# wkentaro/morefusion

Hardware: AMD Instinct MI355X
Metric: objects/sec (32^3 voxelize+3D-CNN+ICC refine) (higher is better)
Workload: dtype f32; 1 GPU; 1 scene(s) x 8 objects per GPU: singleview_3d Model.predict (ResNet18+PSPNet, 32^3 voxelize, occupancy 3D-CNN, heads; B=8) -> ICC joint refine 100 iters (BASELINE configs[1]+configs[2]); random weights, ICC starts from synthetic perturbed-GT poses; ICC(k) on a second HIP stream, event-ordered after network(k), beside network(k+1); objects_per_gpu=8, icc_iters=100, parallelism=scene-sharded x1, pose all_gather, stream_priority=none, backbone_memory_format=contiguous

## Files before the change

include/mfhip.h:

```cpp
#ifndef MFHIP_H_
#define MFHIP_H_

#include <stdint.h>

#ifdef __cplusplus
extern "C" {
#endif

typedef void *mfStream_t;

int mf_version(void);
const char *mf_last_error_string(void);

int mf_average_voxelization_3d_fwd(const float *values, const float *points,
                                   const int32_t *batch_indices, int64_t n, int C,
                                   int B, int X, int Y, int Z, float ox, float oy,
                                   float oz, float pitch, float *matrix,
                                   int32_t *counts, int32_t *head, int32_t *link,
                                   int32_t *nan_flag, mfStream_t stream);
int mf_average_voxelization_3d_bwd(const float *gmatrix, const float *points,
                                   const int32_t *batch_indices,
                                   const int32_t *counts, int64_t n, int C, int B,
                                   int X, int Y, int Z, float ox, float oy, float oz,
                                   float pitch, float *gvalues, mfStream_t stream);

int mf_max_voxelization_3d_fwd(const float *values, const float *points,
                               const int32_t *batch_indices, const float *intensities,
                               int64_t n, int C, int B, int X, int Y, int Z, float ox,
                               float oy, float oz, float pitch, float *matrix,
                               int32_t *indices, uint64_t *key, int32_t *nan_flag,
                               mfStream_t stream);
int mf_max_voxelization_3d_bwd(const float *gmatrix, const int32_t *indices, int64_t n,
                               int C, int B, int X, int Y, int Z, float *gvalues,
                               mfStream_t stream);

int mf_interpolate_voxel_grid_fwd(const float *vox, const float *points,
                                  const int32_t *batch_indices, const int32_t *batch_start,
                                  int64_t n, int B, int C, int X, int Y, int Z, float *values,
                                  int channels_first, mfStream_t stream);
int mf_interpolate_voxel_grid_bwd(const float *gvalues, const float *points,
                                  const int32_t *batch_indices, const int32_t *batch_start,
                                  int64_t n, int B, int C, int X, int Y, int Z, float *gvox,
                                  int channels_first, mfStream_t stream);

int mf_occupancy_grid_3d_fwd(const float *points, int64_t P, float pitch, float ox,
                             float oy, float oz, int X, int Y, int Z, float threshold,
                             float *grid, float *dmin, mfStream_t stream);
int mf_occupancy_grid_3d_bwd(const float *ggrid, const float *points, int64_t P,
                             float pitch, float ox, float oy, float oz, int X, int Y,
                             int Z, float threshold, const float *dmin, float *gpoints,
                             mfStream_t stream);

int mf_truncated_distance_function_fwd(const float *points, int64_t P, float pitch,
                                       float ox, float oy, float oz, int X, int Y, int Z,
                                       float truncation, float *tdf, int32_t *flat,
                                       mfStream_t stream);
int mf_truncated_distance_function_bwd(const float *gtdf, const float *points,
                                       const int32_t *flat, int64_t P, float pitch,
                                       float ox, float oy, float oz, int X, int Y, int Z,
                                       float truncation, float *gpoints,
                                       mfStream_t stream);
int mf_pseudo_occupancy_weights(const float *tdf, const int32_t *flat, const float *sdf,
                                int X, int Y, int Z, int K, float truncation,
                                float sdf_offset, float *grids, float *wsurf, float *win,
                                float *wmax, mfStream_t stream);

int mf_nn(const float *ref, int64_t R, const float *query, int64_t Q, int64_t *out,
          float *out_dist, mfStream_t stream);

int mf_icp_loss_grad(const float *source, int64_t S, const float *target, int64_t T,
                     const float *Rt, float thresh, float *out, mfStream_t stream);

int mf_icp_refine(const float *source, const int32_t *src_off, const float *target,
                  const int32_t *tgt_off, int32_t L, int32_t max_T, float thresh, float *q, float *t,
                  float *adam_m, float *adam_v, int32_t n_iter, int32_t step0, float alpha_q,
                  float alpha_t, float *losses, float *ws, mfStream_t stream);

typedef struct {
  const void *pts4;
  const int32_t *obj_off;
  const int32_t *scene_off;
  const int32_t *obj_scene;
  const float *pitch;
  const float *origin;
  const float *grid_target;
  const float *grid_ne;
  int32_t n_objects;
  int32_t n_scenes;
  int32_t n_points;
  int32_t dim;
  int32_t max_scene_objects;
  float voxel_threshold;
  float sdf_offset;
  int32_t grid_ne_binary;
  int32_t flags;
} mfIccBatch;

int64_t mf_icc_workspace_bytes(const mfIccBatch *batch);

int mf_icc_prepare(const mfIccBatch *batch, void *ws, mfStream_t stream);

int mf_icc_loss_grad(const mfIccBatch *batch, const float *q, const float *t,
                     float *loss, float *gq, float *gt, void *ws, mfStream_t stream);

int mf_icc_refine(const mfIccBatch *batch, float *q, float *t, float *adam_m,
                  float *adam_v, int32_t n_iter, int32_t step0, float alpha_q,
                  float alpha_t, float *losses, float *traj, void *ws,
                  mfStream_t stream);

int mf_icc_iteration_launches(const mfIccBatch *batch);

int mf_icc_plan(const mfIccBatch *batch, int64_t *out, int32_t n);

int mf_icc_launch_stage(const mfIccBatch *batch, const float *q, const float *t, void *ws,
                        int32_t stage, mfStream_t stream);

int mf_icc_debug_stamps(unsigned long long *host_out, int n);

int64_t mf_sparse_conv3d_workspace_bytes(int32_t B, int32_t Cs, int32_t Cout, int32_t D,
                                         int32_t max_rows, int64_t n_points);
int mf_sparse_conv3d_pack_weights(const float *W, int32_t Cout, int32_t Cs, int32_t w_cin,
                                  int32_t c_off, float *Wp, mfStream_t stream);
int mf_sparse_conv3d_k4s2_fwd(const float *x, const int32_t *counts, const float *Wp,
                              const float *dense, const float *bias, float *out, void *ws,
                              int32_t B, int32_t Cs, int32_t Cout, int32_t D, int32_t max_rows,
                              int32_t relu, mfStream_t stream);

int mf_average_distance_fwd(const float *points, const float *T_true, const float *T_pred,
                            const uint8_t *symmetric, int32_t B, int32_t M, int32_t P,
                            float *out, int32_t *nn_idx, mfStream_t stream);
int mf_average_distance_bwd(const float *points, const float *T_true, const float *T_pred,
                            const uint8_t *symmetric, const float *gout, int32_t B, int32_t M,
                            int32_t P, const int32_t *nn_idx, float *gT_pred, mfStream_t stream);

int mf_sparse_conv3d_k4s2_points_fwd(const float *values, const float *points,
                                     const int32_t *batch_indices, int64_t n, float ox, float oy,
                                     float oz, float pitch, const float *Wp, const float *dense,
                                     const float *bias, float *out, void *ws, int32_t B,
                                     int32_t Cs, int32_t Cout, int32_t D, int32_t max_rows,
                                     int32_t relu, mfStream_t stream);

int mf_conv3d_k4s2_pack_weights(const float *W, int32_t Cout, int32_t Cin, int32_t w_cin, int32_t c_off,
                                float *wt, mfStream_t stream);
int32_t mf_conv3d_k4s2_default_split(int32_t B, int32_t Cin, int32_t Cout, int32_t D);
int64_t mf_conv3d_k4s2_workspace_bytes(int32_t B, int32_t Cout, int32_t D, int32_t split);
int mf_conv3d_k4s2_fwd(const float *x, const float *wt, const float *bias, const float *add, float *out,
                       void *ws, int32_t B, int32_t Cin, int32_t Cout, int32_t D, int32_t split,
                       int32_t relu, mfStream_t stream);
int mf_to_channels_last(const float *src, float *dst, int32_t B, int32_t C, int64_t V, mfStream_t stream);

int mf_sparse_conv3d_k4s2_points_cl_fwd(const float *values, int64_t ldv, const float *points,
                                        const int32_t *batch_indices, int64_t n, float ox, float oy,
                                        float oz, float pitch, const float *Wp, const float *dense,
                                        const float *bias, float *out, void *ws, int32_t B, int32_t Cs,
                                        int32_t Cout, int32_t D, int32_t max_rows, int32_t relu,
                                        mfStream_t stream);
int mf_interpolate_voxel_grid_cl_fwd(const float *vox, const float *points, const int32_t *batch_indices,
                                     int64_t n, int B, int C, int X, int Y, int Z, float *out, int64_t ldo,
                                     mfStream_t stream);
int mf_sparse_conv3d_k4s2_points_cl_split_fwd(const float *values, int64_t ldv, const float *points,
                                              const int32_t *batch_indices, int64_t n, float ox, float oy, float oz,
                                              float pitch, const float *Wp, const float *dense, const float *bias,
                                              float *out, void *out_split, void *ws, int32_t B, int32_t Cs,
                                              int32_t Cout, int32_t D, int32_t max_rows, int32_t relu,
                                              mfStream_t stream);
int mf_interpolate_voxel_grid_cl_split_fwd(const float *vox, const float *points, const int32_t *batch_indices,
                                           int64_t n, int B, int C, int X, int Y, int Z, void *outs, int64_t ldos,
                                           int64_t los, mfStream_t stream);
int mf_occupancy_convs_fwd(const float *grid, const float *w1, const float *b1, const float *w2,
                           const float *b2, float *h1, float *h2, int32_t B, int32_t D, mfStream_t stream);

int mf_linear_fwd(const float *A, int64_t a_group_stride, int32_t lda, const float *W, int64_t w_group_stride,
                  int32_t ldw, const float *bias, int64_t b_group_stride, float *out, int64_t o_group_stride,
                  int32_t ldo, int32_t M, int32_t N, int32_t Npad, int32_t K, int32_t groups, int32_t relu,
                  mfStream_t stream);

int mf_cast_rows_bf16(const float *src, int64_t src_ld, void *dst, int64_t dst_ld, int64_t rows, int32_t cols,
                      mfStream_t stream);
int mf_relu_mask_bf16(const void *y, const void *dy, const float *dy32, void *dz, int64_t n, mfStream_t stream);
int mf_linear_bf16(const void *A, int64_t a_group_stride, int32_t lda, const void *W, int64_t w_group_stride,
                   int32_t ldw, const float *bias, int64_t b_group_stride, void *out, int64_t o_group_stride,
                   int32_t ldo, int32_t M, int32_t N, int32_t K, int32_t groups, int32_t relu, int32_t out_f32,
                   int32_t accumulate, mfStream_t stream);
int mf_linear_wgrad_bf16(const void *dY, int64_t y_group_stride, int32_t ldy, const void *A, int64_t a_group_stride,
                         int32_t lda, float *dW, int64_t w_group_stride, int32_t ldc, void *ws, int32_t M, int32_t N,
                         int32_t K, int32_t groups, int32_t split, mfStream_t stream);
int mf_conv3d_k4s2_pack_bf16(const float *W, int32_t Cout, int32_t Cin, int32_t w_cin, int32_t c_off, void *fwd,
                             void *dgrad, mfStream_t stream);
int mf_conv3d_k4s2_bf16_fwd(const void *x, const void *wt, const float *bias, void *out, int32_t B, int32_t Cin,
                            int32_t Cout, int32_t D, int32_t relu, int32_t out_f32, mfStream_t stream);
int mf_conv3d_k4s2_bf16_dgrad(const void *dy, const void *wd, void *dx, int32_t B, int32_t Cin, int32_t Cout,
                              int32_t D, int32_t out_f32, int32_t accumulate, mfStream_t stream);
int64_t mf_conv3d_k4s2_bf16_wgrad_workspace_bytes(int32_t Cin, int32_t Cout, int32_t split);
int32_t mf_conv3d_k4s2_bf16_wgrad_default_split(int32_t B, int32_t Cin, int32_t Cout, int32_t D);
int mf_conv3d_k4s2_bf16_wgrad(const void *dy, const void *x, float *dW, void *ws, int32_t B, int32_t Cin,
                              int32_t Cout, int32_t D, int32_t w_cin, int32_t c_off, int32_t split,
                              mfStream_t stream);

int mf_conv3d_bf16_pack(const float *W, int32_t Cout, int32_t Cin, int32_t w_cin, int32_t c_off, int32_t ks, void *fwd,
                        void *dgrad_k4s2, void *flipT, mfStream_t stream);
int mf_conv3d_bf16_fwd(const void *x, const void *wt, const float *bias, void *out, int32_t B, int32_t Cin,
                       int32_t Cout, int32_t D, int32_t ks, int32_t stride, int32_t pad, int32_t dil, int32_t relu,
                       int32_t out_f32, int32_t ldo, mfStream_t stream);
int64_t mf_conv3d_bf16_fwd_workspace_bytes(int32_t B, int32_t Cin, int32_t Cout, int32_t D, int32_t ks, int32_t stride,
                                           int32_t pad, int32_t dil);
int mf_conv3d_bf16_fwd_ws(const void *x, const void *wt, const float *bias, void *out, void *ws, int64_t ws_bytes,
                          int32_t B, int32_t Cin, int32_t Cout, int32_t D, int32_t ks, int32_t stride, int32_t pad,
                          int32_t dil, int32_t relu, int32_t out_f32, int32_t ldo, mfStream_t stream);
int mf_conv2d_split_pack(const float *W, int32_t Cout, int32_t Cin, int32_t ks, void *wp, mfStream_t stream);
int64_t mf_conv2d_split_workspace_bytes(int32_t B, int32_t Cin, int32_t Cout, int32_t D, int32_t ks, int32_t stride,
                                        int32_t pad, int32_t dil);
int mf_conv2d_split_fwd(const void *xs, const void *wp, const float *bias, const float *res, int32_t ldr,
                        const float *slope, int32_t act, float *out32, int32_t ldo32, void *outs, int32_t ldos,
                        int32_t los, void *ws, int64_t ws_bytes, int32_t B, int32_t Cin, int32_t Cout, int32_t D,
                        int32_t ks, int32_t stride, int32_t pad, int32_t dil, mfStream_t stream);
int mf_conv3d_k4s2_split_pack(const float *W, int32_t Cout, int32_t Cin, int32_t w_cin, int32_t c_off, void *wp,
                              mfStream_t stream);
int64_t mf_conv3d_k4s2_split_workspace_bytes(int32_t B, int32_t Cin, int32_t Cout, int32_t D);
int mf_conv3d_k4s2_split_fwd(const void *xs, const void *wp, const float *bias, int32_t relu, float *out32,
                             int32_t ldo32, void *outs, int32_t ldos, int32_t los, void *ws, int64_t ws_bytes, int32_t B,
                             int32_t Cin, int32_t Cout, int32_t D, mfStream_t stream);
int mf_linear_split_pack(const float *W, int64_t w_gs, int32_t ldw, int32_t N, int32_t K, int32_t Np, int32_t Kp,
                         int32_t groups, void *wp, mfStream_t stream);
int64_t mf_linear_split_workspace_bytes(int64_t M, int32_t N, int32_t Kp);
int mf_linear_split_fwd(const void *As, int32_t lda, const void *wp, const float *bias, int32_t relu, float *out32,
                        int32_t ldo32, void *outs, int32_t ldos, int32_t los, void *ws, int64_t ws_bytes, int32_t M,
                        int32_t N, int32_t Kp, mfStream_t stream);
int64_t mf_conv3d_k3_narrow_bf16_pack_elems(int32_t CI);
int mf_conv3d_k3_narrow_bf16_pack(const float *W, int32_t Cout, int32_t Cin, int32_t w_cin, int32_t c_off,
                                  int32_t transpose, void *wp, mfStream_t stream);
int mf_conv3d_k3_narrow_bf16(const void *x, const void *wp, const float *bias, void *out, int32_t B, int32_t CI,
                             int32_t CO, int32_t D, int32_t dil, int32_t relu, mfStream_t stream);
int64_t mf_conv3d_bf16_wgrad_workspace_bytes(int32_t Cin, int32_t Cout, int32_t ks, int32_t split);
int32_t mf_wgrad_split(int64_t tiles, int64_t ktiles, int64_t slab_bytes);
int32_t mf_linear_wgrad_bf16_default_split(int64_t M, int32_t N, int32_t K, int32_t groups);
int32_t mf_conv3d_bf16_wgrad_default_split(int32_t B, int32_t Cin, int32_t Cout, int32_t Do, int32_t ks);
int mf_conv3d_bf16_wgrad(const void *dy, const void *x, float *dW, void *ws, int32_t B, int32_t Cin, int32_t Cout,
                         int32_t D, int32_t ks, int32_t stride, int32_t pad, int32_t dil, int32_t w_cin, int32_t c_off,
                         int32_t split, mfStream_t stream);

int64_t mf_sparse_conv3_bf16_max_rows(int64_t n_points);
int64_t mf_sparse_conv3_bf16_workspace_bytes(int64_t n_points, int32_t B, int32_t D);
int mf_sparse_conv3_bf16_tables(void *ws, int64_t n_points, int32_t B, int32_t D, int64_t *out7);
int mf_sparse_conv3_bf16_index(const float *points, const int32_t *batch_indices, int64_t n, int32_t B, int32_t D,
                               void *ws, mfStream_t stream);
int mf_sparse_conv3_bf16_pack(const float *W, int32_t Cout, int32_t Cs, int32_t w_cin, int32_t c_off, void *Wp, void *Wq,
                              mfStream_t stream);
int mf_sparse_conv3_bf16_unpack_dw(const float *dWp, int32_t Cout, int32_t Cs, int32_t w_cin, int32_t c_off, float *dW,
                                   mfStream_t stream);
int mf_sparse_conv3_bf16_reduce(const void *C, const float *dense, const float *bias, void *ws, int64_t n_points,
                                int32_t B, int32_t D, int32_t Cout, int32_t relu, void *out, mfStream_t stream);
int mf_sparse_conv3_bf16_gather_dy(const void *dz, void *ws, int64_t n_points, int32_t B, int32_t D, int32_t Cout,
                                   void *dYg, mfStream_t stream);
int mf_linear_bf16_tiles(const void *A, int32_t lda, const void *W, int64_t w_group_stride, int32_t ldw,
                         const int32_t *tile_group, void *out, int32_t ldo, int32_t M, int32_t N, int32_t K,
                         int32_t out_f32, mfStream_t stream);
int mf_linear_wgrad_bf16_ranges(const void *dY, int32_t ldy, const void *A, int32_t lda, float *dW,
                                int64_t w_group_stride, int32_t ldc, const int32_t *m_range, int32_t groups, int32_t N,
                                int32_t K, mfStream_t stream);
int mf_conv3d_k4s2_bf16_pack_cols(const float *W, int32_t Cout, int32_t Cin, int32_t w_cin, int32_t c_off, void *W2,
                                  mfStream_t stream);
int mf_conv3d_k4s2_bf16_col2im(const void *T, int32_t B, int32_t D, int32_t Cin, void *dx, mfStream_t stream);
int mf_average_voxelization_rows_bf16_fwd(const void *values, int64_t ldv, const float *points,
                                          const int32_t *batch_indices, int64_t n, int32_t C, int32_t B, int32_t D,
                                          const int32_t *counts, const int32_t *head, const int32_t *link,
                                          const int32_t *rowmap, void *A, int64_t lda, mfStream_t stream);
int mf_average_voxelization_rows_bf16_bwd(const void *dA, int64_t lda, const float *points,
                                          const int32_t *batch_indices, const int32_t *counts, const int32_t *rowmap,
                                          int64_t n, int32_t C, int32_t B, int32_t D, void *gvalues, int64_t ldg,
                                          mfStream_t stream);

int mf_average_voxelization_cl_bf16_fwd(const void *values, int64_t ldv, const float *points,
                                        const int32_t *batch_indices, int64_t n, int32_t C, int32_t B, int32_t D,
                                        void *x, int64_t ldx, int32_t *counts, int32_t *head, int32_t *link,
                                        mfStream_t stream);
int mf_average_voxelization_cl_bf16_bwd(const void *gx, int64_t ldx, const float *points, const int32_t *batch_indices,
                                        const int32_t *counts, int64_t n, int32_t C, int32_t B, int32_t D,
                                        void *gvalues, int64_t ldg, mfStream_t stream);
int mf_interpolate_voxel_grid_cl_bf16_fwd(const void *vox, const float *points, const int32_t *batch_indices,
                                          int64_t n, int B, int C, int X, int Y, int Z, void *out, int64_t ldo,
                                          mfStream_t stream);
int mf_interpolate_voxel_grid_cl_bf16_bwd(const void *gout, int64_t ldg, const float *points,
                                          const int32_t *batch_indices, const int32_t *batch_start, int64_t n, int B,
                                          int C, int X, int Y, int Z, void *gvox, int32_t out_bf16, mfStream_t stream);

int mf_upsample_bilinear_cl_fwd(const void *x, void *y, int32_t B, int32_t H, int32_t W, int32_t Ho, int32_t Wo,
                                int32_t C, int32_t bf16, mfStream_t stream);
int mf_upsample_bilinear_cl_split_fwd(const float *x, void *y, int32_t B, int32_t H, int32_t W, int32_t Ho, int32_t Wo,
                                      int32_t C, int32_t ldy, int32_t los, mfStream_t stream);
int mf_split_bf16(const float *x, int64_t sb, int64_t sc, int64_t sh, int64_t sw, int32_t B, int32_t C, int32_t H,
                  int32_t W, void *y, int32_t ldy, int32_t los, mfStream_t stream);
int mf_upsample2x_tapsum_fwd(const float *z, const float *bias, const float *slope, int32_t act, float *y32,
                             int32_t ld32, void *ys, int32_t lds, int32_t los, int32_t B, int32_t H, int32_t W, int32_t C,
                             mfStream_t stream);
int mf_maxpool3s2_split_fwd(const float *x, int64_t sb, int64_t sc, int64_t sh, int64_t sw, int32_t B, int32_t C,
                            int32_t H, int32_t W, float *y32, void *ys, mfStream_t stream);
int mf_upsample_bilinear_cl_bwd(const void *gy, void *gx, int32_t B, int32_t H, int32_t W, int32_t Ho, int32_t Wo,
                                int32_t C, int32_t bf16, mfStream_t stream);
int mf_upsample_bilinear_cf_fwd(const void *x, void *y, int64_t BC, int32_t H, int32_t W, int32_t Ho, int32_t Wo,
                                int32_t bf16, mfStream_t stream);
int mf_upsample_bilinear_cf_bwd(const void *gy, void *gx, int64_t BC, int32_t H, int32_t W, int32_t Ho, int32_t Wo,
                                int32_t bf16, mfStream_t stream);
int mf_prelu_fwd(const void *x, const float *slope, void *y, int64_t n, int32_t bf16, mfStream_t stream);
int mf_rgb_normalize(const void *rgb, int32_t u8, const float *mean3, const float *std3, float *out, int64_t npix,
                     mfStream_t stream);
int mf_bn_act_fwd(const void *x, const void *identity, const float *mean, const float *var, const float *weight,
                  const float *bias, float eps, void *y, int64_t n, int32_t C, int64_t HW, int32_t channels_last,
                  int32_t relu, int32_t bf16, mfStream_t stream);
int mf_backbone2d_last_path(void);
int64_t mf_prelu_bwd_workspace_floats(int64_t n);
int mf_prelu_bwd(const void *x, const void *dy, const float *slope, void *dx, float *dslope, float *ws, int64_t n,
                 int32_t bf16, mfStream_t stream);

int mf_gemm_bf16_last_tile(void);

int mf_gemm_bf16_nt_plan(int32_t mode, int64_t M, int32_t N, int32_t K, int32_t groups, int32_t table,
                         int64_t dgrad_rows, int32_t may_split, int32_t have_ws, int32_t *tile, int32_t *S);
int mf_gemm_bf16_tn_plan(int32_t Ni, int32_t Nj, int32_t ldc, int64_t rows, int32_t groups, int32_t ranges,
                         int32_t conv, int32_t split, int32_t *form, int32_t *default_split, int32_t *finish);

int mf_psp_tail_rows_bf16_fwd(const void *u2, const int64_t *pix, int32_t B, int32_t P, int32_t H, int32_t W, void *rows,
                              mfStream_t stream);
int mf_psp_tail_rows_bf16_bwd(const void *grows, const int64_t *pix, int32_t B, int32_t P, int32_t H, int32_t W,
                              float *acc, void *gu2, mfStream_t stream);

int mf_confidence_loss_fwd(const float *add, const float *conf, int32_t B, int32_t P, float lambda, float *loss,
                           int32_t *cnt, mfStream_t stream);
int mf_confidence_loss_bwd(const float *add, const float *conf, const int32_t *cnt, const float *gloss, int32_t B,
                           int32_t P, float lambda, float *dadd, float *dconf, mfStream_t stream);

int mf_pose_epilogue_train_fwd(const float *orot, const float *otrn, const float *ocnf, const int64_t *class_id,
                               const float *pts, const float *origin, const float *pitch, int32_t B, int32_t P,
                               int32_t n_fg, float *rot, float *trans, float *conf, mfStream_t stream);
int mf_pose_epilogue_train_bwd(const float *orot, const float *ocnf, const int64_t *class_id, const float *pitch,
                               const float *grot, const float *gtrans, const float *gconf, int32_t B, int32_t P,
                               int32_t n_fg, float *drot, float *dtrn, float *dcnf, mfStream_t stream);
int mf_transformation_matrix_fwd(const float *q, const float *t, int64_t n, float *T, mfStream_t stream);
int mf_transformation_matrix_bwd(const float *q, const float *gT, int64_t n, float *gq, float *gt, mfStream_t stream);
int mf_point_prep(const float *points_cam, const float *values, const float *origin, const float *pitch,
                  int32_t B, int32_t P, int32_t Cv, float center, float *pts, float *tc4, float *x_rows,
                  int32_t *batch_indices, mfStream_t stream);
int mf_pose_epilogue(const float *heads_out, int64_t ldo, int32_t np4, const int64_t *class_id,
                     const float *pts, const float *origin, const float *pitch, int32_t B, int32_t P, int32_t n_fg,
                     float *rot, float *trans, float *conf, mfStream_t stream);

#define MF_PCDNET_WS_BUFFERS 12
#define MF_PCDNET_MAX_FG 256
int32_t mf_pcdnet_workspace_offsets(int32_t B, int32_t P, int32_t n_fg, int64_t *offsets);
int64_t mf_pcdnet_workspace_bytes(int32_t B, int32_t P, int32_t n_fg);
int mf_pcdnet_stem(const float *x_rows, const float *pcd, const int64_t *pix, const float *center, const float *w_rgb,
                   const float *b_rgb, const float *w_pcd, const float *b_pcd, int32_t B, int32_t P, int32_t HW,
                   float *pts, void *f1, int32_t ld1, void *xs, int32_t ldx, int32_t losx, mfStream_t stream);
int mf_pcdnet_pool(const float *h, int64_t ldh, int32_t B, int32_t P, int32_t C, float *pooled, mfStream_t stream);
int mf_pcdnet_bias_relu_split(const float *y, int64_t ldy, const float *gbias, int32_t B, int32_t P, int32_t N, int32_t G,
                              void *out, int64_t ldo, mfStream_t stream);

int mf_psp_tail_fwd(const float *u2, int64_t sb, int64_t sc, int64_t sy, int64_t sx, const int64_t *pix,
                    const float *w3t, const float *b3, const float *prelu_slope, const float *w1t,
                    const float *b1, int32_t B, int32_t P, int32_t H, int32_t W, float *out, mfStream_t stream);

int mf_pack_points_sdf(const float *points, const float *sdf, int64_t n, void *pts4,
                       mfStream_t stream);

int mf_instance_stats(const int32_t *label, const float *depth, int H, int W,
                      const int32_t *instance_ids, int n_inst, int32_t *stats,
                      mfStream_t stream);
int mf_instance_crops(const uint8_t *rgb, const float *depth, const int32_t *label, int H,
                      int W, double fx, double fy, double cx, double cy,
                      const int32_t *instance_ids, const int32_t *stats, int n_inst, int S,
                      int min_valid, uint8_t *rgb_out, float *pcd_out, uint8_t *keep,
                      mfStream_t stream);

int mf_valid_pixel_order(const float *pcd, int32_t B, int32_t HW, int32_t *order, int32_t *counts,
                         mfStream_t stream);

typedef struct {
  float *logodds;
  uint32_t *bits;
  int32_t lo[3];
  int32_t dim[3];
  double resolution;
  double res_factor;
} mfOccTree;
int mf_occmap_regrid(const mfOccTree *src, const mfOccTree *dst, mfStream_t stream);
int mf_occmap_bounds(const float *pts, const int32_t *label, int64_t n, const int32_t *slots,
                     int32_t n_slots, const mfOccTree *trees, int32_t n_trees, int32_t *bounds,
                     mfStream_t stream);
int mf_occmap_raycast(const float *pts, const int32_t *label, int64_t n, const int32_t *slots,
                      int32_t n_slots, const mfOccTree *trees, float origin_x, float origin_y,
                      float origin_z, int32_t *overflow, mfStream_t stream);
int mf_occmap_count_hits(const float *pts, int64_t n, const mfOccTree *trees, int32_t tree,
                         int32_t *overflow, mfStream_t stream);
int mf_occmap_apply(const mfOccTree *trees, int32_t n_trees, int64_t max_cells, int32_t mode,
                    mfStream_t stream);
int mf_occmap_extract(const mfOccTree *trees, int32_t n_trees, const int32_t *target_tree,
                      const double *pitch, const double *origin, int32_t B, int32_t D0, int32_t D1,
                      int32_t D2, float *grid_target, float *grid_nontarget, float *grid_empty,
                      uint8_t *net_target, uint8_t *net_nte, mfStream_t stream);

int64_t mf_occtrack_workspace_bytes(int32_t H, int32_t W, int32_t n_ref);
int64_t mf_occtrack_stats_elems(int32_t n_ref, int32_t n_det);
int mf_occtrack_transform(const float *pts, const float *T, int64_t n, float *out, mfStream_t stream);
int mf_occtrack_render(const float *pts, const float *K, const float *T, float origin_x, float origin_y,
                       float origin_z, const mfOccTree *trees, const int32_t *slots, int32_t n_slots,
                       int32_t H, int32_t W, void *workspace, int32_t *label_rendered,
                       float *depth_rendered, mfStream_t stream);
int mf_occtrack_overlap(const int32_t *label_rendered, const int32_t *label_detected, int32_t H, int32_t W,
                        const int32_t *ref_ids, int32_t n_ref, const int32_t *det_ids, int32_t n_det,
                        int32_t *stats, mfStream_t stream);
int mf_occtrack_assign(const int32_t *stats, const int32_t *ref_ids, int32_t n_ref, int32_t n_det, int32_t H,
                       int32_t W, int32_t min_mask, int32_t min_bbox, int32_t min_side, double iou_threshold,
                       double coverage_threshold, int32_t *counter, int32_t *remap, int32_t *suspicious_ref,
                       int32_t *suspicious_det, mfStream_t stream);
int mf_occtrack_relabel(const int32_t *label_rendered, const int32_t *label_detected, int32_t H, int32_t W,
                        const int32_t *ref_ids, int32_t n_ref, const int32_t *det_ids, int32_t n_det,
                        const int32_t *remap, const int32_t *suspicious_ref, int32_t *label_tracked,
                        int32_t *label_reference, mfStream_t stream);
int mf_occtrack_clean(const int32_t *label, int32_t H, int32_t W, int32_t min_area, int32_t band,
                      void *workspace, int32_t *label_out, mfStream_t stream);
int mf_occtrack_merge(const int32_t *label_reference, const int32_t *label_tracked, int32_t H, int32_t W,
                      const int32_t *ref_ids, int32_t n_ref, void *workspace, int32_t *label_merged,
                      mfStream_t stream);

#define MF_ICPREG_MAX_CELLS (1 << 24)
int64_t mf_icpreg_workspace_bytes(int64_t total_cells, int64_t total_grid, int64_t n_points);
int mf_icpreg_bounds(const double *pts, const int64_t *off, int32_t n_sets, double voxel_size,
                     double *vmin, int32_t *ext, mfStream_t stream);
int mf_icpreg_prepare(const double *pts, const int64_t *off, int32_t n_sets, double voxel_size,
                      const double *vmin, const int32_t *ext, const int64_t *box_off,
                      int64_t total_cells, const int64_t *grid_off, const int32_t *grid_dim,
                      int64_t total_grid, double cell, int64_t n_points, void *workspace,
                      double *out, int32_t *out_cnt, double *grid_origin, int32_t *grid_start,
                      int32_t *grid_idx, mfStream_t stream);
typedef struct {
  const double *src;
  const int64_t *src_off;
  const int32_t *src_cnt;
  const double *tgt;
  const int64_t *tgt_off;
  const int32_t *tgt_cnt;
  const int64_t *grid_off;
  const int32_t *grid_dim;
  const double *grid_origin;
  const int32_t *grid_start;
  const int32_t *grid_idx;
  const double *transform_init;
  const uint8_t *active;
  double *cur;
  int32_t *corr;
  double *transform;
  double *transformation;
  double *fitness;
  double *inlier_rmse;
  int32_t *n_iter;
  double *hist_transform;
  double *hist_fitness;
  double *hist_rmse;
  double max_corr_dist;
  double cell;
  int32_t n_objects;
  int32_t max_iter;
  int32_t mode;
  int32_t reserved;
} mfIcpRegBatch;
int mf_icpreg_run(const mfIcpRegBatch *batch, mfStream_t stream);

#define MF_MESHSDF_MAX_MESHES 65535
#define MF_MESHSDF_MAX_FACES (1LL << 26)
#define MF_MESHSDF_MAX_GRID_DIM 1024
typedef struct {
  const double *vertices;
  const int64_t *v_off;
  const int32_t *faces;
  const int64_t *f_off;
  double *face_rec;
  const double *points;
  const int64_t *q_off;
  const int32_t *blk_off;
  const double *grid_origin;
  const double *grid_h;
  double *dist;
  int32_t *face;
  double *winding;
  double *sdf;
  uint8_t *occupancy;
  int32_t n_meshes;
  int32_t n_blocks;
  int32_t grid_dim;
  int32_t reserved;
} mfMeshSdfBatch;
int64_t mf_meshsdf_workspace_bytes(int64_t total_faces);
int mf_meshsdf_prepare(const mfMeshSdfBatch *batch, int64_t total_faces, mfStream_t stream);
int mf_meshsdf_query(const mfMeshSdfBatch *batch, mfStream_t stream);

#define MF_RENDER_MAX_ITEMS 65535
#define MF_RENDER_MAX_FACES (1LL << 26)
#define MF_RENDER_MAX_PIXELS (1LL << 28)
#define MF_RENDER_MAX_SIDE 4096
typedef struct {
  const double *vertices;
  const int64_t *v_off;
  const int32_t *faces;
  const int64_t *f_off;
  const int32_t *item_mesh;
  const double *item_T;
  const int32_t *item_target;
  const int32_t *item_id;
  const int64_t *item_rec_off;
  void *workspace;
  float *depth;
  int32_t *instance;
  int32_t *face;
  int32_t *count;
  double fx;
  double fy;
  double cx;
  double cy;
  double near;
  int32_t n_meshes;
  int32_t n_items;
  int32_t n_targets;
  int32_t height;
  int32_t width;
  int32_t reserved;
} mfRenderBatch;
int64_t mf_render_workspace_bytes(int64_t total_records, int64_t n_targets, int64_t height, int64_t width);
int mf_render_setup(const mfRenderBatch *batch, int64_t total_records, mfStream_t stream);
int mf_render_raster(const mfRenderBatch *batch, int64_t total_records, mfStream_t stream);
int mf_render_resolve(const mfRenderBatch *batch, int64_t total_records, mfStream_t stream);
int mf_full_grids(const double *points, const int64_t *p_off, const double *T, const double *pitch,
                  const double *origin, int32_t n_examples, int64_t total_points, int32_t dim,
                  int32_t *target_full, int32_t *nontarget_full, mfStream_t stream);

#define MF_PICK_MAX_OBJECTS 64
int mf_pick_occlusion(const int32_t *instance, const int32_t *item_id, int32_t n_items, int32_t height,
                      int32_t width, int32_t *whole, int32_t *occluded_by, int32_t *bbox, mfStream_t stream);
int mf_pick_normals(const double *points, const int32_t *rect, int32_t n_images, int32_t height, int32_t width,
                    double *normals, mfStream_t stream);
int mf_pick_grasp(const float *depth, const int32_t *instance, const int32_t *item_id, const int32_t *bbox,
                  int32_t n_items, int32_t height, int32_t width, double fx, double fy, double cx, double cy,
                  int32_t *cell, double *translation, double *normal, mfStream_t stream);

int64_t mf_average_distance_f64_workspace_bytes(int32_t n_items, int32_t max_points);
int mf_average_distance_f64(const double *points, const int32_t *cloud_off, const int32_t *item_cloud,
                            const double *T1, const double *T2, int32_t n_clouds, int32_t n_items,
                            int32_t max_points, int32_t translate, double *add, double *add_s, void *workspace,
                            mfStream_t stream);

int64_t mf_augment_workspace_bytes(int32_t n, int32_t S);
int mf_augment_mask(const uint8_t *rgb, const void *pcd, int32_t pcd_is_f64, const double *params,
                    int32_t n, int32_t S, int64_t seed, uint8_t *rgb_out, void *pcd_out,
                    uint8_t *kept_mask, int32_t *stats, uint8_t *keep, int32_t *labels, int32_t *sizes,
                    void *workspace, mfStream_t stream);
int mf_augment_rgb(const uint8_t *rgb, const double *params, int32_t n, int32_t S, uint8_t *rgb_out,
                   void *workspace, mfStream_t stream);
int mf_augment_pcd(const void *pcd, int32_t pcd_is_f64, const double *params, int32_t n, int32_t S,
                   int64_t seed, void *pcd_out, mfStream_t stream);

#define MF_OCCREG_MAX_OBJECTS 65535
#define MF_OCCREG_POINT_TILE 1024
#define MF_OCCREG_LDS_VOXELS 32768
#define MF_OCCREG_MAX_THRESHOLD 64.0f
#define MF_OCCREG_STEPS_PER_LAUNCH 128
typedef struct {
  const float *points;
  const int32_t *pts_off;
  const float *pitch;
  const float *origin;
  const int32_t *dims;
  const float *threshold;
  const float *grid_occ;
  const float *grid_unocc;
  const int32_t *grid_off;
  const uint8_t *active;
  const int32_t *host_pts_off;
  const float *host_pitch;
  const int32_t *host_dims;
  const float *host_threshold;
  int32_t n_objects;
  int32_t n_points_total;
  int32_t max_voxels;
  int32_t reserved;
} mfOccRegBatch;
int64_t mf_occreg_workspace_bytes(int64_t n_objects, int64_t n_points_total, int64_t max_voxels);
int mf_occreg_loss_grad(const mfOccRegBatch *batch, const float *q, const float *t, float *loss, float *gq,
                        float *gt, void *workspace, mfStream_t stream);
int mf_occreg_refine(const mfOccRegBatch *batch, float *q, float *t, float *adam_m, float *adam_v, int32_t n_iter,
                     int32_t step0, float alpha_q, float alpha_t, float *losses, float *traj, void *workspace,
                     mfStream_t stream);

#ifdef __cplusplus
}
#endif
#endif
```

morefusion_amd/_lib.py:

```python
import ctypes
import os

import torch

_HERE = os.path.dirname(os.path.abspath(__file__))
SO_PATH = os.path.join(_HERE, os.path.basename(os.environ.get("MF_LIBMFHIP", "libmfhip.so")))
_lib = None

_p = ctypes.c_void_p
_i = ctypes.c_int32
_i64 = ctypes.c_int64
_f = ctypes.c_float
_d = ctypes.c_double


class IccBatch(ctypes.Structure):

    _fields_ = [
        ("pts4", _p), ("obj_off", _p), ("scene_off", _p), ("obj_scene", _p),
        ("pitch", _p), ("origin", _p), ("grid_target", _p), ("grid_ne", _p),
        ("n_objects", _i), ("n_scenes", _i), ("n_points", _i), ("dim", _i), ("max_scene_objects", _i),
        ("voxel_threshold", _f), ("sdf_offset", _f), ("grid_ne_binary", _i), ("flags", _i),
    ]


class OccTree(ctypes.Structure):

    _fields_ = [
        ("logodds", _p), ("bits", _p), ("lo", _i * 3), ("dim", _i * 3),
        ("resolution", _d), ("res_factor", _d),
    ]


class IcpRegBatch(ctypes.Structure):

    _fields_ = [(n, _p) for n in (
        "src", "src_off", "src_cnt", "tgt", "tgt_off", "tgt_cnt", "grid_off", "grid_dim", "grid_origin", "grid_start",
        "grid_idx", "transform_init", "active", "cur", "corr", "transform", "transformation", "fitness", "inlier_rmse",
        "n_iter", "hist_transform", "hist_fitness", "hist_rmse")] + [
        ("max_corr_dist", _d), ("cell", _d), ("n_objects", _i), ("max_iter", _i), ("mode", _i), ("reserved", _i)]


class MeshSdfBatch(ctypes.Structure):

    _fields_ = [(n, _p) for n in (
        "vertices", "v_off", "faces", "f_off", "face_rec", "points", "q_off", "blk_off", "grid_origin", "grid_h",
        "dist", "face", "winding", "sdf", "occupancy")] + [
        ("n_meshes", _i), ("n_blocks", _i), ("grid_dim", _i), ("reserved", _i)]


class RenderBatch(ctypes.Structure):

    _fields_ = [(n, _p) for n in (
        "vertices", "v_off", "faces", "f_off", "item_mesh", "item_T", "item_target", "item_id", "item_rec_off",
        "workspace", "depth", "instance", "face", "count")] + [
        (n, _d) for n in ("fx", "fy", "cx", "cy", "near")] + [
        (n, _i) for n in ("n_meshes", "n_items", "n_targets", "height", "width", "reserved")]


class OccRegBatch(ctypes.Structure):

    _fields_ = [(n, _p) for n in (
        "points", "pts_off", "pitch", "origin", "dims", "threshold", "grid_occ", "grid_unocc", "grid_off", "active",
        "host_pts_off", "host_pitch", "host_dims", "host_threshold")] + [
        (n, _i) for n in ("n_objects", "n_points_total", "max_voxels", "reserved")]


_SIGNATURES = {
    "mf_version": ([], _i),
    "mf_last_error_string": ([], ctypes.c_char_p),
    "mf_average_voxelization_3d_fwd": ([_p, _p, _p, _i64, _i, _i, _i, _i, _i, _f, _f, _f, _f, _p, _p, _p, _p, _p, _p], _i),
    "mf_average_voxelization_3d_bwd": ([_p, _p, _p, _p, _i64, _i, _i, _i, _i, _i, _f, _f, _f, _f, _p, _p], _i),
    "mf_max_voxelization_3d_fwd": ([_p, _p, _p, _p, _i64, _i, _i, _i, _i, _i, _f, _f, _f, _f, _p, _p, _p, _p, _p], _i),
    "mf_max_voxelization_3d_bwd": ([_p, _p, _i64, _i, _i, _i, _i, _i, _p, _p], _i),
    "mf_interpolate_voxel_grid_fwd": ([_p, _p, _p, _p, _i64, _i, _i, _i, _i, _i, _p, _i, _p], _i),
    "mf_interpolate_voxel_grid_bwd": ([_p, _p, _p, _p, _i64, _i, _i, _i, _i, _i, _p, _i, _p], _i),
    "mf_occupancy_grid_3d_fwd": ([_p, _i64, _f, _f, _f, _f, _i, _i, _i, _f, _p, _p, _p], _i),
    "mf_occupancy_grid_3d_bwd": ([_p, _p, _i64, _f, _f, _f, _f, _i, _i, _i, _f, _p, _p, _p], _i),
    "mf_truncated_distance_function_fwd": ([_p, _i64, _f, _f, _f, _f, _i, _i, _i, _f, _p, _p, _p], _i),
    "mf_truncated_distance_function_bwd": ([_p, _p, _p, _i64, _f, _f, _f, _f, _i, _i, _i, _f, _p, _p], _i),
    "mf_pseudo_occupancy_weights": ([_p, _p, _p, _i, _i, _i, _i, _f, _f, _p, _p, _p, _p, _p], _i),
    "mf_nn": ([_p, _i64, _p, _i64, _p, _p, _p], _i),
    "mf_icp_loss_grad": ([_p, _i64, _p, _i64, _p, _f, _p, _p], _i),
    "mf_icp_refine": ([_p, _p, _p, _p, _i, _i, _f, _p, _p, _p, _p, _i, _i, _f, _f, _p, _p, _p], _i),
    "mf_icc_workspace_bytes": ([ctypes.POINTER(IccBatch)], _i64),
    "mf_icc_iteration_launches": ([ctypes.POINTER(IccBatch)], _i),
    "mf_icc_plan": ([ctypes.POINTER(IccBatch), _p, _i], _i),
    "mf_icc_launch_stage": ([ctypes.POINTER(IccBatch), _p, _p, _p, _i, _p], _i),
    "mf_icc_prepare": ([ctypes.POINTER(IccBatch), _p, _p], _i),
    "mf_icc_loss_grad": ([ctypes.POINTER(IccBatch), _p, _p, _p, _p, _p, _p, _p], _i),
    "mf_icc_refine": ([ctypes.POINTER(IccBatch), _p, _p, _p, _p, _i, _i, _f, _f, _p, _p, _p, _p], _i),
    "mf_icc_debug_stamps": ([_p, _i], _i),
    "mf_sparse_conv3d_workspace_bytes": ([_i] * 5 + [_i64], _i64),
    "mf_sparse_conv3d_k4s2_points_fwd": ([_p, _p, _p, _i64, _f, _f, _f, _f, _p, _p, _p, _p, _p] + [_i] * 6 + [_p], _i),
    "mf_sparse_conv3d_pack_weights": ([_p, _i, _i, _i, _i, _p, _p], _i),
    "mf_sparse_conv3d_k4s2_fwd": ([_p, _p, _p, _p, _p, _p, _p] + [_i] * 6 + [_p], _i),
    "mf_pack_points_sdf": ([_p, _p, _i64, _p, _p], _i),
    "mf_average_distance_fwd": ([_p, _p, _p, _p, _i, _i, _i, _p, _p, _p], _i),
    "mf_average_distance_bwd": ([_p, _p, _p, _p, _p, _i, _i, _i, _p, _p, _p], _i),
    "mf_conv3d_k4s2_pack_weights": ([_p, _i, _i, _i, _i, _p, _p], _i),
    "mf_conv3d_k4s2_default_split": ([_i] * 4, _i),
    "mf_conv3d_k4s2_workspace_bytes": ([_i] * 4, _i64),
    "mf_conv3d_k4s2_fwd": ([_p, _p, _p, _p, _p, _p] + [_i] * 6 + [_p], _i),
    "mf_to_channels_last": ([_p, _p, _i, _i, _i64, _p], _i),
    "mf_sparse_conv3d_k4s2_points_cl_fwd": ([_p, _i64, _p, _p, _i64, _f, _f, _f, _f, _p, _p, _p, _p, _p] + [_i] * 6 + [_p], _i),
    "mf_interpolate_voxel_grid_cl_fwd": ([_p, _p, _p, _i64, _i, _i, _i, _i, _i, _p, _i64, _p], _i),
    "mf_occupancy_convs_fwd": ([_p] * 7 + [_i] * 2 + [_p], _i),
    "mf_linear_fwd": ([_p, _i64, _i, _p, _i64, _i, _p, _i64, _p, _i64] + [_i] * 7 + [_p], _i),
    "mf_cast_rows_bf16": ([_p, _i64, _p, _i64, _i64, _i, _p], _i),
    "mf_relu_mask_bf16": ([_p, _p, _p, _p, _i64, _p], _i),
    "mf_linear_bf16": ([_p, _i64, _i, _p, _i64, _i, _p, _i64, _p, _i64] + [_i] * 8 + [_p], _i),
    "mf_linear_wgrad_bf16": ([_p, _i64, _i, _p, _i64, _i, _p, _i64, _i, _p] + [_i] * 5 + [_p], _i),
    "mf_conv3d_k4s2_pack_bf16": ([_p] + [_i] * 4 + [_p, _p, _p], _i),
    "mf_conv3d_k4s2_bf16_fwd": ([_p, _p, _p, _p] + [_i] * 6 + [_p], _i),
    "mf_conv3d_k4s2_bf16_dgrad": ([_p, _p, _p] + [_i] * 6 + [_p], _i),
    "mf_conv3d_k4s2_bf16_wgrad_workspace_bytes": ([_i] * 3, _i64),
    "mf_conv3d_k4s2_bf16_wgrad_default_split": ([_i] * 4, _i),
    "mf_conv3d_k4s2_bf16_wgrad": ([_p, _p, _p, _p] + [_i] * 7 + [_p], _i),
    "mf_conv3d_bf16_pack": ([_p] + [_i] * 5 + [_p, _p, _p, _p], _i),
    "mf_conv3d_bf16_fwd": ([_p, _p, _p, _p] + [_i] * 11 + [_p], _i),
    "mf_conv3d_bf16_fwd_workspace_bytes": ([_i] * 8, _i64),
    "mf_conv3d_bf16_fwd_ws": ([_p, _p, _p, _p, _p, _i64] + [_i] * 11 + [_p], _i),
    "mf_conv2d_split_pack": ([_p] + [_i] * 3 + [_p, _p], _i),
    "mf_conv2d_split_workspace_bytes": ([_i] * 8, _i64),
    "mf_conv2d_split_fwd": ([_p, _p, _p, _p, _i, _p, _i, _p, _i, _p, _i, _i, _p, _i64] + [_i] * 8 + [_p], _i),
    "mf_conv3d_k4s2_split_pack": ([_p] + [_i] * 4 + [_p, _p], _i),
    "mf_conv3d_k4s2_split_workspace_bytes": ([_i] * 4, _i64),
    "mf_conv3d_k4s2_split_fwd": ([_p, _p, _p, _i, _p, _i, _p, _i, _i, _p, _i64] + [_i] * 4 + [_p], _i),
    "mf_linear_split_pack": ([_p, _i64] + [_i] * 6 + [_p, _p], _i),
    "mf_linear_split_workspace_bytes": ([_i64, _i, _i], _i64),
    "mf_linear_split_fwd": ([_p, _i, _p, _p, _i, _p, _i, _p, _i, _i, _p, _i64] + [_i] * 3 + [_p], _i),
    "mf_sparse_conv3d_k4s2_points_cl_split_fwd": ([_p, _i64, _p, _p, _i64, _f, _f, _f, _f, _p, _p, _p, _p, _p, _p] + [_i] * 6 + [_p], _i),
    "mf_interpolate_voxel_grid_cl_split_fwd": ([_p, _p, _p, _i64, _i, _i, _i, _i, _i, _p, _i64, _i64, _p], _i),
    "mf_conv3d_k3_narrow_bf16_pack_elems": ([_i], _i64),
    "mf_conv3d_k3_narrow_bf16_pack": ([_p] + [_i] * 5 + [_p, _p], _i),
    "mf_conv3d_k3_narrow_bf16": ([_p, _p, _p, _p] + [_i] * 6 + [_p], _i),
    "mf_conv3d_bf16_wgrad_workspace_bytes": ([_i] * 4, _i64),
    "mf_wgrad_split": ([_i64, _i64, _i64], _i),
    "mf_linear_wgrad_bf16_default_split": ([_i64, _i, _i, _i], _i),
    "mf_conv3d_bf16_wgrad_default_split": ([_i] * 5, _i),
    "mf_conv3d_bf16_wgrad": ([_p, _p, _p, _p] + [_i] * 11 + [_p], _i),
    "mf_sparse_conv3_bf16_max_rows": ([_i64], _i64),
    "mf_sparse_conv3_bf16_workspace_bytes": ([_i64, _i, _i], _i64),
    "mf_sparse_conv3_bf16_tables": ([_p, _i64, _i, _i, _p], _i),
    "mf_sparse_conv3_bf16_index": ([_p, _p, _i64, _i, _i, _p, _p], _i),
    "mf_sparse_conv3_bf16_pack": ([_p, _i, _i, _i, _i, _p, _p, _p], _i),
    "mf_sparse_conv3_bf16_unpack_dw": ([_p, _i, _i, _i, _i, _p, _p], _i),
    "mf_sparse_conv3_bf16_reduce": ([_p, _p, _p, _p, _i64, _i, _i, _i, _i, _p, _p], _i),
    "mf_sparse_conv3_bf16_gather_dy": ([_p, _p, _i64, _i, _i, _i, _p, _p], _i),
    "mf_linear_bf16_tiles": ([_p, _i, _p, _i64, _i, _p, _p, _i, _i, _i, _i, _i, _p], _i),
    "mf_linear_wgrad_bf16_ranges": ([_p, _i, _p, _i, _p, _i64, _i, _p, _i, _i, _i, _p], _i),
    "mf_conv3d_k4s2_bf16_pack_cols": ([_p, _i, _i, _i, _i, _p, _p], _i),
    "mf_conv3d_k4s2_bf16_col2im": ([_p, _i, _i, _i, _p, _p], _i),
    "mf_average_voxelization_rows_bf16_fwd": ([_p, _i64, _p, _p, _i64, _i, _i, _i, _p, _p, _p, _p, _p, _i64, _p], _i),
    "mf_average_voxelization_rows_bf16_bwd": ([_p, _i64, _p, _p, _p, _p, _i64, _i, _i, _i, _p, _i64, _p], _i),
    "mf_average_voxelization_cl_bf16_fwd": ([_p, _i64, _p, _p, _i64, _i, _i, _i, _p, _i64, _p, _p, _p, _p], _i),
    "mf_average_voxelization_cl_bf16_bwd": ([_p, _i64, _p, _p, _p, _i64, _i, _i, _i, _p, _i64, _p], _i),
    "mf_interpolate_voxel_grid_cl_bf16_fwd": ([_p, _p, _p, _i64, _i, _i, _i, _i, _i, _p, _i64, _p], _i),
    "mf_interpolate_voxel_grid_cl_bf16_bwd": ([_p, _i64, _p, _p, _p, _i64, _i, _i, _i, _i, _i, _p, _i, _p], _i),
    "mf_upsample_bilinear_cl_fwd": ([_p, _p] + [_i] * 7 + [_p], _i),
    "mf_upsample_bilinear_cl_split_fwd": ([_p, _p] + [_i] * 8 + [_p], _i),
    "mf_upsample2x_tapsum_fwd": ([_p, _p, _p, _i, _p, _i, _p] + [_i] * 6 + [_p], _i),
    "mf_split_bf16": ([_p, _i64, _i64, _i64, _i64] + [_i] * 4 + [_p, _i, _i, _p], _i),
    "mf_maxpool3s2_split_fwd": ([_p, _i64, _i64, _i64, _i64] + [_i] * 4 + [_p, _p, _p], _i),
    "mf_upsample_bilinear_cl_bwd": ([_p, _p] + [_i] * 7 + [_p], _i),
    "mf_upsample_bilinear_cf_fwd": ([_p, _p, _i64] + [_i] * 5 + [_p], _i),
    "mf_upsample_bilinear_cf_bwd": ([_p, _p, _i64] + [_i] * 5 + [_p], _i),
    "mf_prelu_fwd": ([_p, _p, _p, _i64, _i, _p], _i),
    "mf_rgb_normalize": ([_p, _i, _p, _p, _p, _i64, _p], _i),
    "mf_bn_act_fwd": ([_p, _p, _p, _p, _p, _p, _f, _p, _i64, _i, _i64, _i, _i, _i, _p], _i),
    "mf_backbone2d_last_path": ([], _i),
    "mf_prelu_bwd_workspace_floats": ([_i64], _i64),
    "mf_prelu_bwd": ([_p, _p, _p, _p, _p, _p, _i64, _i, _p], _i),
    "mf_gemm_bf16_last_tile": ([], _i),
    "mf_gemm_bf16_nt_plan": ([_i, _i64, _i, _i, _i, _i, _i64, _i, _i, _p, _p], _i),
    "mf_gemm_bf16_tn_plan": ([_i, _i, _i, _i64, _i, _i, _i, _i, _p, _p, _p], _i),
    "mf_psp_tail_rows_bf16_fwd": ([_p, _p, _i, _i, _i, _i, _p, _p], _i),
    "mf_psp_tail_rows_bf16_bwd": ([_p, _p, _i, _i, _i, _i, _p, _p, _p], _i),
    "mf_confidence_loss_fwd": ([_p, _p, _i, _i, _f, _p, _p, _p], _i),
    "mf_confidence_loss_bwd": ([_p, _p, _p, _p, _i, _i, _f, _p, _p, _p], _i),
    "mf_pose_epilogue_train_fwd": ([_p, _p, _p, _p, _p, _p, _p, _i, _i, _i, _p, _p, _p, _p], _i),
    "mf_pose_epilogue_train_bwd": ([_p, _p, _p, _p, _p, _p, _p, _i, _i, _i, _p, _p, _p, _p], _i),
    "mf_transformation_matrix_fwd": ([_p, _p, _i64, _p, _p], _i),
    "mf_transformation_matrix_bwd": ([_p, _p, _i64, _p, _p, _p], _i),
    "mf_point_prep": ([_p, _p, _p, _p, _i, _i, _i, _f, _p, _p, _p, _p, _p], _i),
    "mf_pose_epilogue": ([_p, _i64, _i, _p, _p, _p, _p, _i, _i, _i, _p, _p, _p, _p], _i),
    "mf_psp_tail_fwd": ([_p, _i64, _i64, _i64, _i64, _p, _p, _p, _p, _p, _p] + [_i] * 4 + [_p, _p], _i),
    "mf_valid_pixel_order": ([_p, _i, _i, _p, _p, _p], _i),
    "mf_instance_stats": ([_p, _p, _i, _i, _p, _i, _p, _p], _i),
    "mf_instance_crops": ([_p, _p, _p, _i, _i, _d, _d, _d, _d, _p, _p, _i, _i, _i, _p, _p, _p, _p], _i),
    "mf_occmap_regrid": ([ctypes.POINTER(OccTree), ctypes.POINTER(OccTree), _p], _i),
    "mf_occmap_bounds": ([_p, _p, _i64, _p, _i, _p, _i, _p, _p], _i),
    "mf_occmap_raycast": ([_p, _p, _i64, _p, _i, _p, _f, _f, _f, _p, _p], _i),
    "mf_occmap_count_hits": ([_p, _i64, _p, _i, _p, _p], _i),
    "mf_occmap_apply": ([_p, _i, _i64, _i, _p], _i),
    "mf_occmap_extract": ([_p, _i, _p, _p, _p] + [_i] * 4 + [_p] * 6, _i),
    "mf_occtrack_workspace_bytes": ([_i] * 3, _i64),
    "mf_occtrack_stats_elems": ([_i, _i], _i64),
    "mf_occtrack_transform": ([_p, _p, _i64, _p, _p], _i),
    "mf_occtrack_render": ([_p, _p, _p, _f, _f, _f, _p, _p, _i, _i, _i, _p, _p, _p, _p], _i),
    "mf_occtrack_overlap": ([_p, _p, _i, _i, _p, _i, _p, _i, _p, _p], _i),
    "mf_occtrack_assign": ([_p, _p] + [_i] * 7 + [_d, _d] + [_p] * 5, _i),
    "mf_occtrack_relabel": ([_p, _p, _i, _i, _p, _i, _p, _i] + [_p] * 5, _i),
    "mf_occtrack_clean": ([_p] + [_i] * 4 + [_p, _p, _p], _i),
    "mf_occtrack_merge": ([_p, _p, _i, _i, _p, _i, _p, _p, _p], _i),
    "mf_icpreg_workspace_bytes": ([_i64, _i64, _i64], _i64),
    "mf_icpreg_bounds": ([_p, _p, _i, _d, _p, _p, _p], _i),
    "mf_icpreg_prepare": ([_p, _p, _i, _d, _p, _p, _p, _i64, _p, _p, _i64, _d, _i64] + [_p] * 7, _i),
    "mf_icpreg_run": ([ctypes.POINTER(IcpRegBatch), _p], _i),
    "mf_meshsdf_workspace_bytes": ([_i64], _i64),
    "mf_meshsdf_prepare": ([ctypes.POINTER(MeshSdfBatch), _i64, _p], _i),
    "mf_meshsdf_query": ([ctypes.POINTER(MeshSdfBatch), _p], _i),
    "mf_render_workspace_bytes": ([_i64] * 4, _i64),
    "mf_render_setup": ([_p, _i64, _p], _i),
    "mf_render_raster": ([_p, _i64, _p], _i),
    "mf_render_resolve": ([_p, _i64, _p], _i),
    "mf_full_grids": ([_p] * 5 + [_i, _i64, _i, _p, _p, _p], _i),
    "mf_pick_occlusion": ([_p, _p, _i, _i, _i, _p, _p, _p, _p], _i),
    "mf_pick_normals": ([_p, _p, _i, _i, _i, _p, _p], _i),
    "mf_pick_grasp": ([_p, _p, _p, _p, _i, _i, _i, _d, _d, _d, _d, _p, _p, _p, _p], _i),
    "mf_average_distance_f64_workspace_bytes": ([_i, _i], _i64),
    "mf_average_distance_f64": ([_p] * 5 + [_i] * 4 + [_p] * 4, _i),
    "mf_augment_workspace_bytes": ([_i, _i], _i64),
    "mf_augment_mask": ([_p, _p, _i, _p, _i, _i, _i64] + [_p] * 9, _i),
    "mf_augment_rgb": ([_p, _p, _i, _i, _p, _p, _p], _i),
    "mf_augment_pcd": ([_p, _i, _p, _i, _i, _i64, _p, _p], _i),
    "mf_pcdnet_workspace_offsets": ([_i, _i, _i, _p], _i),
    "mf_pcdnet_workspace_bytes": ([_i, _i, _i], _i64),
    "mf_pcdnet_stem": ([_p] * 8 + [_i] * 3 + [_p, _p, _i, _p, _i, _i, _p], _i),
    "mf_pcdnet_pool": ([_p, _i64, _i, _i, _i, _p, _p], _i),
    "mf_pcdnet_bias_relu_split": ([_p, _i64, _p, _i, _i, _i, _i, _p, _i64, _p], _i),
    "mf_occreg_workspace_bytes": ([_i64, _i64, _i64], _i64),
    "mf_occreg_loss_grad": ([_p] * 8, _i),
    "mf_occreg_refine": ([_p] * 5 + [_i, _i, _f, _f] + [_p] * 4, _i),
}

EXPORTED_SYMBOLS = tuple(_SIGNATURES)


def bind(handle, partial=False):
    for name, (argtypes, restype) in _SIGNATURES.items():
        fn = getattr(handle, name, None) if partial else getattr(handle, name)
        if fn is not None:
            fn.argtypes, fn.restype = argtypes, restype
    return handle


def lib():
    global _lib
    if _lib is None:
        if not os.path.exists(SO_PATH):
            raise RuntimeError(
                f"{SO_PATH} is missing: the HIP extension is not built. Run "
                "`python -c 'import __graft_entry__ as g; g.build()'` (or `make -C "
                "morefusion_amd/csrc`). morefusion_amd has no CPU fallback."
            )
        handle = bind(ctypes.CDLL(SO_PATH))
        _lib = handle
    return _lib


def check(code, what):
    if code != 0:
        msg = lib().mf_last_error_string().decode()
        raise RuntimeError(f"{what} failed ({code}): {msg}")


def stream_ptr():
    return torch.cuda.current_stream().cuda_stream


def require_gpu(*tensors):
    cur = None
    for t in tensors:
        if not isinstance(t, torch.Tensor):
            raise TypeError(f"expected torch.Tensor, got {type(t)}")
        if not t.is_cuda:
            raise RuntimeError(
                "morefusion_amd voxel/refinement ops run on the MI355X only: got a "
                f"{t.device} tensor (there is no CPU fallback; move inputs to 'cuda')."
            )
        if cur is None:
            cur = torch.cuda.current_device()
        if t.device.index != cur:
            raise RuntimeError(
                f"tensor on {t.device} but the current device is cuda:{cur}: run the op under "
                f"`with torch.cuda.device({t.device.index}):` (kernels launch on the current device's stream)")


def ptr(t):
    return None if t is None else t.data_ptr()


def f32c(t):
    return t.detach().to(torch.float32).contiguous()


def i32c(t):
    return t.detach().to(torch.int32).contiguous()


def as_float3(origin):
    if isinstance(origin, torch.Tensor):
        origin = origin.detach().cpu().tolist()
    o = [float(x) for x in origin]
    if len(o) != 3:
        raise ValueError("origin must have 3 elements")
    return o
```

morefusion_amd/contrib/singleview_3d/models/volumetric_cl.py:

```python
import torch
import torch.nn.functional as F

from .... import _lib
from .sparse_conv import SparseVoxelConv3d


F_COLS, F_LD = 984, 992

SPLIT_MIN_BATCH = {"conv4": 4, "heads1": 4}


class ChannelsLastVolumetric:

    split_bf16 = True

    def __init__(self, model):
        self.m = model
        self._packs = {}
        self._buf = {}
        self._sparse = SparseVoxelConv3d(model.conv3)
        self.mfma_linear = True

    def _pack(self, name, tensors, build):
        key = tuple((t.data_ptr(), t._version) for t in tensors)
        hit = self._packs.get(name)
        if hit is None or hit[0] != key:
            hit = (key, build())
            self._packs[name] = hit
        return hit[1]

    def _conv_pack(self, name, conv, cin, c_off):
        def build():
            w = conv.weight.detach().float().contiguous()
            cout, w_cin = w.shape[0], w.shape[1]
            wt = torch.empty((cout, 64, cin), dtype=torch.float32, device=w.device)
            _lib.check(_lib.lib().mf_conv3d_k4s2_pack_weights(w.data_ptr(), cout, cin, w_cin, c_off, wt.data_ptr(),
                                                              _lib.stream_ptr()), "mf_conv3d_k4s2_pack_weights")
            bias = conv.bias.detach().float().contiguous() if conv.bias is not None else None
            return wt, bias
        return self._pack(name, [conv.weight] + ([conv.bias] if conv.bias is not None else []), build)

    def _occ_pack(self):
        m = self.m

        def build():
            out = []
            for conv in (m.conv1_occ, m.conv2_occ):
                w = conv.weight.detach().float()
                out.append(w.permute(2, 3, 4, 1, 0).contiguous().reshape(27, w.shape[1], w.shape[0]))
                out.append(conv.bias.detach().float().contiguous())
            return out
        return self._pack("occ", [m.conv1_occ.weight, m.conv1_occ.bias, m.conv2_occ.weight, m.conv2_occ.bias], build)

    def _linear_pack(self, name, conv):
        return self._pack(name, [conv.weight, conv.bias],
                          lambda: (conv.weight.detach().squeeze(-1).contiguous(), conv.bias.detach()))

    def _scratch(self, name, shape, device, dtype=torch.float32, zero=False):
        key = (name, tuple(shape), str(device), dtype)
        t = self._buf.get(key)
        if t is None:
            t = (torch.zeros if zero else torch.empty)(shape, dtype=dtype, device=device)
            self._buf[key] = t
        return t

    def conv_k4s2(self, name, conv, x_cl, B, D, cin, c_off=0, add=None, relu=True, bias=True, split=None):
        L = _lib.lib()
        wt, b = self._conv_pack(name, conv, cin, c_off)
        cout = wt.shape[0]
        if split is None:
            split = L.mf_conv3d_k4s2_default_split(B, cin, cout, D)
        nbytes = L.mf_conv3d_k4s2_workspace_bytes(B, cout, D, split)
        ws = self._scratch(name + "_ws", (max(nbytes, 16),), x_cl.device, torch.uint8)
        out = torch.empty((B, (D // 2) ** 3, cout), dtype=torch.float32, device=x_cl.device)
        _lib.check(L.mf_conv3d_k4s2_fwd(x_cl.data_ptr(), wt.data_ptr(), _lib.ptr(b if bias else None), _lib.ptr(add),
                                        out.data_ptr(), ws.data_ptr(), B, cin, cout, D, int(split), int(relu),
                                        _lib.stream_ptr()), "mf_conv3d_k4s2_fwd")
        return out

    def _split_path(self, layer, B):
        return (self.split_bf16 and self.mfma_linear and not torch.is_autocast_enabled()
                and not torch.is_grad_enabled() and B >= SPLIT_MIN_BATCH[layer])

    def conv_k4s2_split(self, name, conv, xs_cl, B, D, cin, c_off=0, relu=True, bias=True, out_split=None):
        L = _lib.lib()

        def build():
            w = conv.weight.detach().float().contiguous()
            wp = torch.empty((w.shape[0], 64, 3 * cin), dtype=torch.bfloat16, device=w.device)
            _lib.check(L.mf_conv3d_k4s2_split_pack(w.data_ptr(), w.shape[0], cin, w.shape[1], c_off, wp.data_ptr(),
                                                   _lib.stream_ptr()), "mf_conv3d_k4s2_split_pack")
            return wp, (conv.bias.detach().float().contiguous() if conv.bias is not None else None)
        wp, b = self._pack(name + "_split", [conv.weight] + ([conv.bias] if conv.bias is not None else []), build)
        cout = wp.shape[0]
        nbytes = L.mf_conv3d_k4s2_split_workspace_bytes(B, cin, cout, D)
        ws = self._scratch(name + "_split_ws", (max(nbytes, 16),), xs_cl.device, torch.uint8)
        out = torch.empty((B, (D // 2) ** 3, cout), dtype=torch.float32, device=xs_cl.device)
        _lib.check(L.mf_conv3d_k4s2_split_fwd(xs_cl.data_ptr(), wp.data_ptr(), _lib.ptr(b if bias else None), int(relu),
                                              out.data_ptr(), cout, _lib.ptr(out_split), 2 * cout, cout, ws.data_ptr(),
                                              nbytes, B, cin, cout, D, _lib.stream_ptr()), "mf_conv3d_k4s2_split_fwd")
        return out

    def sample_split(self, vox_cl, D, pts, batch_indices, fs_block, ldos, los):
        B, _, C = vox_cl.shape
        _lib.check(_lib.lib().mf_interpolate_voxel_grid_cl_split_fwd(
            vox_cl.data_ptr(), pts.data_ptr(), batch_indices.data_ptr(), pts.shape[0], B, C, D, D, D,
            fs_block.data_ptr(), ldos, los, _lib.stream_ptr()), "mf_interpolate_voxel_grid_cl_split_fwd")

    def _split_cols(self, feat, c0, c1, fs):
        n = feat.shape[0]
        _lib.check(_lib.lib().mf_split_bf16(feat[:, c0:].data_ptr(), 0, 1, 0, feat.stride(0), 1, c1 - c0, 1, n,
                                            fs[:, c0:].data_ptr(), 2 * F_LD, F_LD, _lib.stream_ptr()), "mf_split_bf16")

    def heads1_split(self, fs, h1):
        m, L = self.m, _lib.lib()
        names = ("rot", "trans", "conf")

        def build():
            w = torch.cat([getattr(m, f"conv1_{k}").weight.detach().float().squeeze(-1) for k in names]).contiguous()
            wp = torch.empty((w.shape[0], 3 * F_LD), dtype=torch.bfloat16, device=w.device)
            _lib.check(L.mf_linear_split_pack(w.data_ptr(), 0, w.shape[1], w.shape[0], w.shape[1], w.shape[0], F_LD, 1,
                                              wp.data_ptr(), _lib.stream_ptr()), "mf_linear_split_pack")
            return wp, torch.cat([getattr(m, f"conv1_{k}").bias.detach().float() for k in names]).contiguous()
        wp, b = self._pack("gemm_heads1_split", [t for k in names for t in (getattr(m, f"conv1_{k}").weight,
                                                                             getattr(m, f"conv1_{k}").bias)], build)
        n, N = fs.shape[0], wp.shape[0]
        nbytes = L.mf_linear_split_workspace_bytes(n, N, F_LD)
        ws = self._scratch("heads1_split_ws", (max(nbytes, 16),), fs.device, torch.uint8)
        _lib.check(L.mf_linear_split_fwd(fs.data_ptr(), 2 * F_LD, wp.data_ptr(), b.data_ptr(), 1, h1.data_ptr(),
                                         h1.stride(0), None, 0, 0, ws.data_ptr(), nbytes, n, N, F_LD,
                                         _lib.stream_ptr()), "mf_linear_split_fwd")

    def occupancy(self, grid):
        B, D = grid.shape[0], grid.shape[1]
        g = _lib.f32c(grid)
        w1, b1, w2, b2 = self._occ_pack()
        h1 = self._scratch("occ_h1", (B, D ** 3, 8), g.device)
        h2 = torch.empty((B, D ** 3, 16), dtype=torch.float32, device=g.device)
        _lib.check(_lib.lib().mf_occupancy_convs_fwd(g.data_ptr(), w1.data_ptr(), b1.data_ptr(), w2.data_ptr(),
                                                     b2.data_ptr(), h1.data_ptr(), h2.data_ptr(), B, D,
                                                     _lib.stream_ptr()), "mf_occupancy_convs_fwd")
        return h2

    def sample(self, vox_cl, D, pts, batch_indices, out_block, ldo):
        B, _, C = vox_cl.shape
        _lib.check(_lib.lib().mf_interpolate_voxel_grid_cl_fwd(
            vox_cl.data_ptr(), pts.data_ptr(), batch_indices.data_ptr(), pts.shape[0], B, C, D, D, D,
            out_block.data_ptr(), ldo, _lib.stream_ptr()), "mf_interpolate_voxel_grid_cl_fwd")

    def prep(self, values, points_cam, pitch, origin):
        B, _, P = points_cam.shape
        n, dev = B * P, values.device
        _lib.require_gpu(values, points_cam, pitch, origin)
        pts = torch.empty((n, 3), dtype=torch.float32, device=dev)
        tc4 = torch.empty((n, 4), dtype=torch.float32, device=dev)
        if values.ndim == 2:
            x_rows, Cv = _lib.f32c(values), 0
        else:
            Cv = values.shape[1]
            x_rows = torch.empty((n, Cv), dtype=torch.float32, device=dev)
        bi = torch.empty((n,), dtype=torch.int32, device=dev)
        _lib.check(_lib.lib().mf_point_prep(
            _lib.f32c(points_cam).data_ptr(), _lib.f32c(values).data_ptr(), _lib.f32c(origin).data_ptr(),
            _lib.f32c(pitch).data_ptr(), B, P, Cv, self.m._voxel_dim / 2.0 - 0.5, pts.data_ptr(), tc4.data_ptr(),
            x_rows.data_ptr(), bi.data_ptr(), _lib.stream_ptr()), "mf_point_prep")
        return pts, tc4, x_rows, bi

    def features(self, values, points_cam, pitch, origin, grid_nontarget_empty):
        m = self.m
        B, _, P = points_cam.shape
        n, D = B * P, m._voxel_dim
        dev = values.device
        pts, tc4, x_rgb, batch_indices = self.prep(values, points_cam, pitch, origin)
        to_center = tc4[:, :3]
        feat = torch.empty((n, F_LD), dtype=torch.float32, device=dev)
        feat[:, F_COLS:].zero_()
        split4, split1 = self._split_path("conv4", B), self._split_path("heads1", B)
        fs = self._scratch("feat_split", (n, 2 * F_LD), dev, torch.bfloat16, zero=True) if split1 else None

        if self.mfma_linear and not torch.is_autocast_enabled():
            self._linear("conv1_rgb", [m.conv1_rgb], x_rgb, 32, feat[:, 0:64], F_LD, relu=True)
            self._linear("conv1_pcd", [m.conv1_pcd], tc4, 4, feat[:, 64:72], F_LD, relu=True, k_pad=4)
            self._linear("conv2_rgb", [m.conv2_rgb], feat[:, 0:64], F_LD, feat[:, 72:200], F_LD, relu=True)
            self._linear("conv2_pcd", [m.conv2_pcd], feat[:, 64:72], F_LD, feat[:, 200:216], F_LD, relu=True)
        else:
            w, b = self._linear_pack("conv1_rgb", m.conv1_rgb)
            h_rgb = F.relu(F.linear(x_rgb, w, b))
            w, b = self._linear_pack("conv1_pcd", m.conv1_pcd)
            h_pcd = F.relu(F.linear(to_center.to(x_rgb.dtype), w, b))
            feat[:, 0:64] = h_rgb
            feat[:, 64:72] = h_pcd
            w, b = self._linear_pack("conv2_rgb", m.conv2_rgb)
            feat[:, 72:200] = F.relu(F.linear(h_rgb, w, b))
            w, b = self._linear_pack("conv2_pcd", m.conv2_pcd)
            feat[:, 200:216] = F.relu(F.linear(h_pcd, w, b))

        dense = None
        if m._with_occupancy:
            h_occ = self.occupancy(grid_nontarget_empty)
            dense = self.conv_k4s2("conv3_occ", m.conv3, h_occ, B, D, cin=16, c_off=144, relu=False, bias=False)
        h3s = self._scratch("h3_split", (B, (D // 2) ** 3, 2 * m.conv3.out_channels), dev, torch.bfloat16) if split4 else None
        h3 = self._sparse.from_points_cl(feat[:, 72:216], F_LD, pts, batch_indices, B, dense, D, out_split=h3s)
        pts2 = pts * 0.5
        if split4:
            h4 = self.conv_k4s2_split("conv4", m.conv4, h3s, B, D // 2, cin=256)
        else:
            h4 = self.conv_k4s2("conv4", m.conv4, h3, B, D // 2, cin=256)
        if split1:
            self._split_cols(feat, 0, 216, fs)
            self.sample_split(h3, D // 2, pts2, batch_indices, fs[:, 216:], 2 * F_LD, F_LD)
            self.sample_split(h4, D // 4, pts2 * 0.5, batch_indices, fs[:, 472:], 2 * F_LD, F_LD)
            feat._mf_split = fs
        else:
            self.sample(h3, D // 2, pts2, batch_indices, feat[:, 216:472], F_LD)
            self.sample(h4, D // 4, pts2 * 0.5, batch_indices, feat[:, 472:984], F_LD)
        return feat, pts

    def _gemm_pack(self, name, convs, k_pad=None):
        def build():
            ws, bs = [], []
            for c in convs:
                w = c.weight.detach().float().squeeze(-1)
                N, K = w.shape
                Kp = k_pad or K
                Np = -(-N // 128) * 128
                wp = torch.zeros((Np, Kp), dtype=torch.float32, device=w.device)
                wp[:N, :K] = w
                ws.append(wp)
                bs.append(c.bias.detach().float())
            return torch.stack(ws).contiguous(), torch.stack(bs).contiguous()
        return self._pack("gemm_" + name, [t for c in convs for t in (c.weight, c.bias)], build)

    def _linear(self, name, convs, a, lda, out, ldo, relu, k_pad=None, a_gs=0, o_gs=0):
        w, b = self._gemm_pack(name, convs, k_pad)
        G, Np, K = w.shape
        N = b.shape[1]
        _lib.check(_lib.lib().mf_linear_fwd(a.data_ptr(), a_gs, lda, w.data_ptr(), Np * K, K, b.data_ptr(), N,
                                            out.data_ptr(), o_gs, ldo, a.shape[0], N, Np, K, G, int(relu),
                                            _lib.stream_ptr()), "mf_linear_fwd")

    def heads(self, feat, B, P, raw=False):
        m = self.m
        nf = m._n_fg_class
        names = ("rot", "trans", "conf")
        if self.mfma_linear and not torch.is_autocast_enabled() and feat.dtype == torch.float32:
            n, dev = feat.shape[0], feat.device
            def build1():
                w = torch.cat([getattr(m, f"conv1_{k}").weight.detach().float().squeeze(-1) for k in names])
                wp = torch.zeros((w.shape[0], F_LD), dtype=torch.float32, device=w.device)
                wp[:, :F_COLS] = w
                b = torch.cat([getattr(m, f"conv1_{k}").bias.detach().float() for k in names])
                return wp.contiguous()[None], b.contiguous()[None]
            w1, b1 = self._pack("gemm_heads1", [t for k in names for t in (getattr(m, f"conv1_{k}").weight,
                                                                            getattr(m, f"conv1_{k}").bias)], build1)
            h1 = self._scratch("heads_h1", (n, 1920), dev)
            h2 = self._scratch("heads_h2", (n, 768), dev)
            h3 = self._scratch("heads_h3", (n, 384), dev)
            np4 = -(-(nf * 4) // 128) * 128
            o = torch.empty((n, 3 * np4), dtype=torch.float32, device=dev)
            L = _lib.lib()
            assert feat.stride(0) == F_LD
            fs = getattr(feat, "_mf_split", None)
            if fs is None and self._split_path("heads1", B):
                fs = self._scratch("feat_split", (n, 2 * F_LD), dev, torch.bfloat16, zero=True)
                self._split_cols(feat, 0, F_COLS, fs)
            if fs is not None:
                self.heads1_split(fs, h1)
            else:
                _lib.check(L.mf_linear_fwd(feat.data_ptr(), 0, F_LD, w1.data_ptr(), 0, F_LD, b1.data_ptr(), 0,
                                           h1.data_ptr(), 0, 1920, n, 1920, 1920, F_LD, 1, 1, _lib.stream_ptr()),
                           "mf_linear_fwd")
            self._linear("heads2", [getattr(m, f"conv2_{k}") for k in names], h1, 1920, h2, 768, True, a_gs=640, o_gs=256)
            self._linear("heads3", [getattr(m, f"conv3_{k}") for k in names], h2, 768, h3, 384, True, a_gs=256, o_gs=128)
            w4, b4 = self._pack("gemm_heads4", [t for k in names for t in (getattr(m, f"conv4_{k}").weight,
                                                                           getattr(m, f"conv4_{k}").bias)],
                                lambda: self._pad_heads4(names, nf, np4))
            _lib.check(L.mf_linear_fwd(h3.data_ptr(), 128, 384, w4.data_ptr(), np4 * 128, 128, b4.data_ptr(), np4,
                                       o.data_ptr(), np4, 3 * np4, n, np4, np4, 128, 3, 0, _lib.stream_ptr()),
                       "mf_linear_fwd")
            if raw:
                return o, np4
            rot = o[:, 0:nf * 4].reshape(B, P, nf, 4)
            trans = o[:, np4:np4 + nf * 3].reshape(B, P, nf, 3)
            conf = torch.sigmoid(o[:, 2 * np4:2 * np4 + nf]).reshape(B, P, nf)
            return rot, trans, conf
        if raw:
            return None, 0
        outs = {}
        for name in names:
            x = feat[:, :F_COLS]
            for i in (1, 2, 3):
                w, b = self._linear_pack(f"conv{i}_{name}", getattr(m, f"conv{i}_{name}"))
                x = F.relu(F.linear(x, w, b))
            w, b = self._linear_pack(f"conv4_{name}", getattr(m, f"conv4_{name}"))
            outs[name] = F.linear(x, w, b).float()
        return (outs["rot"].reshape(B, P, nf, 4), outs["trans"].reshape(B, P, nf, 3),
                torch.sigmoid(outs["conf"]).reshape(B, P, nf))

    def _pad_heads4(self, names, nf, np4):
        m = self.m
        w = torch.zeros((3, np4, 128), dtype=torch.float32, device=m.conv4_rot.weight.device)
        b = torch.zeros((3, np4), dtype=torch.float32, device=w.device)
        for g, k in enumerate(names):
            c = getattr(m, f"conv4_{k}")
            w[g, :c.out_channels] = c.weight.detach().float().squeeze(-1)
            b[g, :c.out_channels] = c.bias.detach().float()
        return w.contiguous(), b.contiguous()

    def pose(self, class_id, values, points_cam, pitch, origin, grid_nontarget_empty):
        B, _, P = points_cam.shape
        feat, pts = self.features(values, points_cam, pitch, origin, grid_nontarget_empty)
        o, np4 = self.heads(feat, B, P, raw=True)
        if o is not None:
            dev = values.device
            rot = torch.empty((B, P, 4), dtype=torch.float32, device=dev)
            trans = torch.empty((B, P, 3), dtype=torch.float32, device=dev)
            conf = torch.empty((B, P), dtype=torch.float32, device=dev)
            cid = class_id.to(device=dev, dtype=torch.int64).contiguous()
            _lib.check(_lib.lib().mf_pose_epilogue(
                o.data_ptr(), o.stride(0), np4, cid.data_ptr(), pts.data_ptr(), _lib.f32c(origin).data_ptr(),
                _lib.f32c(pitch).data_ptr(), B, P, self.m._n_fg_class, rot.data_ptr(), trans.data_ptr(), conf.data_ptr(),
                _lib.stream_ptr()), "mf_pose_epilogue")
            return rot, trans, conf
        cls_rot, cls_trans, cls_conf = self.heads(feat, B, P)
        fg = (class_id - 1).long()
        ar = torch.arange(B, device=values.device)
        rot = cls_rot[ar, :, fg]
        rot = rot / (rot.norm(dim=2, keepdim=True) + 1e-5)
        pts_b = pts.reshape(B, P, 3)
        points_back = pts_b * pitch[:, None, None] + origin[:, None, :]
        trans = points_back + cls_trans[ar, :, fg] * pitch[:, None, None]
        conf = cls_conf[ar, :, fg]
        return rot, trans, conf
```

morefusion_amd/csrc/conv3d.hip:

```cpp
#include "mf_common.h"

namespace {

typedef float f32x16 __attribute__((ext_vector_type(16)));

constexpr int kBM = 128, kBN = 128, kBK = 32;
constexpr int kPitch = kBK + 4;
constexpr int kTileFloats = (kBM + kBN) * kPitch;
constexpr int kConvLds = 2 * kTileFloats * (int)sizeof(float);

struct ConvArgs {
  const float *x;
  const float *wt;
  const float *bias;
  const float *add;
  float *out;
  int B, D, Cin, cin_log2, Cout, S, relu;
};

__device__ __forceinline__ float4 load_a(const float *__restrict__ x, int base, int mask, int tapoff, int tapbits) {
  const bool ok = (mask & tapbits) == tapbits;
  const float4 r = *reinterpret_cast<const float4 *>(x + (ok ? base + tapoff : 0));
  return ok ? r : make_float4(0.0f, 0.0f, 0.0f, 0.0f);
}

__global__ __launch_bounds__(256, 2) void k_conv3d_k4s2_mfma(ConvArgs a) {
  MF_DYN_LDS(float, s_mem);
  const int Do = a.D / 2, Vo = Do * Do * Do;
  const int M = a.B * Vo, N = a.Cout, K = 64 * a.Cin;
  const int tiles_m = (M + kBM - 1) / kBM, tiles_n = N / kBN;
  const int G = gridDim.x;
  int L = blockIdx.x;
  if ((G & 7) == 0) L = (blockIdx.x & 7) * (G >> 3) + (blockIdx.x >> 3);
  const int split = L / (tiles_m * tiles_n);
  const int rem = L - split * (tiles_m * tiles_n);
  const int m0 = (rem % tiles_m) * kBM, n0 = (rem / tiles_m) * kBN;
  const int T = (K / kBK) / a.S;
  const int kt0 = split * T;

  const int tid = threadIdx.x, wave = tid >> 6, lane = tid & 63;
  const int wm = wave & 1, wn = wave >> 1;
  const int lrow = lane & 31, lhalf = lane >> 5;
  const int chunk = tid & 7, r0 = tid >> 3;

  int base[4], mask[4];
#pragma unroll
  for (int i = 0; i < 4; ++i) {
    const int m = m0 + r0 + 32 * i;
    const bool row_ok = m < M;
    const int mm = row_ok ? m : 0;
    const int b = mm / Vo, o = mm - b * Vo;
    const int ox = o / (Do * Do), oy = (o / Do) % Do, oz = o % Do;
    const int x0 = 2 * ox - 1, y0 = 2 * oy - 1, z0 = 2 * oz - 1;
    base[i] = (((b * a.D + x0) * a.D + y0) * a.D + z0) * a.Cin;
    int mk = row_ok ? 1 << 12 : 0;
#pragma unroll
    for (int k = 0; k < 4; ++k) {
      mk |= ((unsigned)(x0 + k) < (unsigned)a.D ? 1 : 0) << k;
      mk |= ((unsigned)(y0 + k) < (unsigned)a.D ? 1 : 0) << (4 + k);
      mk |= ((unsigned)(z0 + k) < (unsigned)a.D ? 1 : 0) << (8 + k);
    }
    mask[i] = mk;
  }
  const float *wrow[4];
#pragma unroll
  for (int i = 0; i < 4; ++i) wrow[i] = a.wt + (n0 + r0 + 32 * i) * K + 4 * chunk;

  f32x16 acc[2][2];
#pragma unroll
  for (int i = 0; i < 2; ++i)
#pragma unroll
    for (int j = 0; j < 2; ++j)
#pragma unroll
      for (int e = 0; e < 16; ++e) acc[i][j][e] = 0.0f;

#define MF_CONV_FETCH(kt_)                                                                        \
  {                                                                                               \
    const int kt__ = (kt_);                                                                       \
    const int kglob = kt__ * kBK + 4 * chunk;                                                     \
    const int tap = kglob >> a.cin_log2, kx = tap >> 4, ky = (tap >> 2) & 3, kz = tap & 3;        \
    const int tapoff = ((kx * a.D + ky) * a.D + kz) * a.Cin + (kglob & (a.Cin - 1));              \
    const int tapbits = (1 << kx) | (16 << ky) | (256 << kz) | (1 << 12);                         \
    ra0 = load_a(a.x, base[0], mask[0], tapoff, tapbits);                                         \
    ra1 = load_a(a.x, base[1], mask[1], tapoff, tapbits);                                         \
    ra2 = load_a(a.x, base[2], mask[2], tapoff, tapbits);                                         \
    ra3 = load_a(a.x, base[3], mask[3], tapoff, tapbits);                                         \
    rb0 = *reinterpret_cast<const float4 *>(wrow[0] + kt__ * kBK);                       \
    rb1 = *reinterpret_cast<const float4 *>(wrow[1] + kt__ * kBK);                       \
    rb2 = *reinterpret_cast<const float4 *>(wrow[2] + kt__ * kBK);                       \
    rb3 = *reinterpret_cast<const float4 *>(wrow[3] + kt__ * kBK);                       \
  }
#define MF_CONV_STASH(buf_)                                                                       \
  {                                                                                               \
    float *As_ = s_mem + (buf_) * kTileFloats + r0 * kPitch + 4 * chunk;                          \
    float *Bs_ = As_ + kBM * kPitch;                                                              \
    *reinterpret_cast<float4 *>(As_) = ra0;                                                       \
    *reinterpret_cast<float4 *>(As_ + 32 * kPitch) = ra1;                                         \
    *reinterpret_cast<float4 *>(As_ + 64 * kPitch) = ra2;                                         \
    *reinterpret_cast<float4 *>(As_ + 96 * kPitch) = ra3;                                         \
    *reinterpret_cast<float4 *>(Bs_) = rb0;                                                       \
    *reinterpret_cast<float4 *>(Bs_ + 32 * kPitch) = rb1;                                         \
    *reinterpret_cast<float4 *>(Bs_ + 64 * kPitch) = rb2;                                         \
    *reinterpret_cast<float4 *>(Bs_ + 96 * kPitch) = rb3;                                         \
  }
  float4 ra0, ra1, ra2, ra3, rb0, rb1, rb2, rb3;
  MF_CONV_FETCH(kt0);
  MF_CONV_STASH(0);
  __syncthreads();
  for (int t = 0; t < T; ++t) {
    MF_CONV_FETCH(kt0 + (t + 1 < T ? t + 1 : t));
    asm volatile("" ::: "memory");
    __builtin_amdgcn_sched_barrier(0);
    const float *As = s_mem + (t & 1) * kTileFloats + (wm * 64 + lrow) * kPitch + 4 * lhalf;
    const float *Bs = s_mem + (t & 1) * kTileFloats + (kBM + wn * 64 + lrow) * kPitch + 4 * lhalf;
#pragma unroll
    for (int kk = 0; kk < 4; ++kk) {
      const float4 a0 = *reinterpret_cast<const float4 *>(As + 8 * kk);
      const float4 a1 = *reinterpret_cast<const float4 *>(As + 32 * kPitch + 8 * kk);
      const float4 b0 = *reinterpret_cast<const float4 *>(Bs + 8 * kk);
      const float4 b1 = *reinterpret_cast<const float4 *>(Bs + 32 * kPitch + 8 * kk);
#define MF_CONV_STEP(c_)                                                                          \
      acc[0][0] = __builtin_amdgcn_mfma_f32_32x32x2f32(a0.c_, b0.c_, acc[0][0], 0, 0, 0);         \
      acc[0][1] = __builtin_amdgcn_mfma_f32_32x32x2f32(a0.c_, b1.c_, acc[0][1], 0, 0, 0);         \
      acc[1][0] = __builtin_amdgcn_mfma_f32_32x32x2f32(a1.c_, b0.c_, acc[1][0], 0, 0, 0);         \
      acc[1][1] = __builtin_amdgcn_mfma_f32_32x32x2f32(a1.c_, b1.c_, acc[1][1], 0, 0, 0);
      MF_CONV_STEP(x)
      MF_CONV_STEP(y)
      MF_CONV_STEP(z)
      MF_CONV_STEP(w)
#undef MF_CONV_STEP
    }
    MF_CONV_STASH((t + 1) & 1);
    __syncthreads();
  }
#undef MF_CONV_FETCH
#undef MF_CONV_STASH

  float *dst = a.out + (a.S > 1 ? (int64_t)split * M * N : 0);
#pragma unroll
  for (int mi = 0; mi < 2; ++mi)
#pragma unroll
    for (int ni = 0; ni < 2; ++ni) {
      const int n = n0 + wn * 64 + ni * 32 + lrow;
      const float bn = (a.S == 1 && a.bias) ? a.bias[n] : 0.0f;
#pragma unroll
      for (int e = 0; e < 16; ++e) {
        const int m = m0 + wm * 64 + mi * 32 + (e & 3) + 8 * (e >> 2) + 4 * lhalf;
        if (m >= M) continue;
        float v = acc[mi][ni][e];
        if (a.S == 1) {
          v += bn;
          if (a.add) v += a.add[(int64_t)m * N + n];
          if (a.relu) v = v > 0.0f ? v : 0.0f;
        }
        dst[(int64_t)m * N + n] = v;
      }
    }
}

__global__ __launch_bounds__(256) void k_conv_finish(const float *__restrict__ slabs, const float *__restrict__ bias,
                                                     const float *__restrict__ add, float *__restrict__ out,
                                                     int64_t MN, int N, int S, int relu) {
  const int64_t i4 = (int64_t)blockIdx.x * blockDim.x + threadIdx.x;
  if (i4 * 4 >= MN) return;
  const float4 *s4 = reinterpret_cast<const float4 *>(slabs);
  float4 v = s4[i4];
  for (int s = 1; s < S; ++s) {
    const float4 w = s4[(int64_t)s * (MN / 4) + i4];
    v.x += w.x; v.y += w.y; v.z += w.z; v.w += w.w;
  }
  const int n = (int)((i4 * 4) % N);
  if (bias) {
    const float4 b = *reinterpret_cast<const float4 *>(bias + n);
    v.x += b.x; v.y += b.y; v.z += b.z; v.w += b.w;
  }
  if (add) {
    const float4 w = reinterpret_cast<const float4 *>(add)[i4];
    v.x += w.x; v.y += w.y; v.z += w.z; v.w += w.w;
  }
  if (relu) {
    v.x = v.x > 0.0f ? v.x : 0.0f; v.y = v.y > 0.0f ? v.y : 0.0f;
    v.z = v.z > 0.0f ? v.z : 0.0f; v.w = v.w > 0.0f ? v.w : 0.0f;
  }
  reinterpret_cast<float4 *>(out)[i4] = v;
}

__global__ void k_conv_pack(const float *__restrict__ W, int Cout, int Cin, int w_cin, int c_off,
                            float *__restrict__ wt) {
  const int64_t i = (int64_t)blockIdx.x * blockDim.x + threadIdx.x;
  const int64_t total = (int64_t)Cout * 64 * Cin;
  if (i >= total) return;
  const int ci = (int)(i % Cin), tap = (int)((i / Cin) % 64), co = (int)(i / ((int64_t)64 * Cin));
  wt[i] = W[((int64_t)co * w_cin + c_off + ci) * 64 + tap];
}

__global__ __launch_bounds__(256) void k_to_channels_last(const float *__restrict__ src, float *__restrict__ dst,
                                                          int C, int V) {
  __shared__ float tile[32][33];
  const int b = blockIdx.z, v0 = blockIdx.x * 32, c0 = blockIdx.y * 32;
  const int tx = threadIdx.x & 31, ty = threadIdx.x >> 5;
  for (int j = ty; j < 32; j += 8)
    if (c0 + j < C && v0 + tx < V) tile[j][tx] = src[((int64_t)b * C + c0 + j) * V + v0 + tx];
  __syncthreads();
  for (int j = ty; j < 32; j += 8)
    if (v0 + j < V && c0 + tx < C) dst[((int64_t)b * V + v0 + j) * C + c0 + tx] = tile[tx][j];
}

template <int CI, int CO, int DIL>
__global__ __launch_bounds__(256) void k_occ_conv3(const float *__restrict__ x, const float *__restrict__ w,
                                                   const float *__restrict__ bias, float *__restrict__ out,
                                                   int B, int D) {
  const int64_t total = (int64_t)B * D * D * D;
  const int64_t i = (int64_t)blockIdx.x * blockDim.x + threadIdx.x;
  if (i >= total) return;
  const int iz = (int)(i % D), iy = (int)((i / D) % D), ix = (int)((i / ((int64_t)D * D)) % D);
  const int64_t b = i / ((int64_t)D * D * D);
  float acc[CO];
#pragma unroll
  for (int co = 0; co < CO; ++co) acc[co] = bias[co];
#pragma unroll 1
  for (int kx = 0; kx < 3; ++kx) {
    const int jx = ix + (kx - 1) * DIL;
#pragma unroll 1
    for (int ky = 0; ky < 3; ++ky) {
      const int jy = iy + (ky - 1) * DIL;
#pragma unroll
      for (int kz = 0; kz < 3; ++kz) {
        const int jz = iz + (kz - 1) * DIL;
        const bool ok = (unsigned)jx < (unsigned)D && (unsigned)jy < (unsigned)D && (unsigned)jz < (unsigned)D;
        const float *src = x + (ok ? (((b * D + jx) * D + jy) * D + jz) * CI : 0);
        float in[CI];
        if (CI % 4 == 0) {
#pragma unroll
          for (int q = 0; q < CI / 4; ++q) {
            const float4 v = reinterpret_cast<const float4 *>(src)[q];
            in[4 * q] = v.x; in[4 * q + 1] = v.y; in[4 * q + 2] = v.z; in[4 * q + 3] = v.w;
          }
        } else {
#pragma unroll
          for (int ci = 0; ci < CI; ++ci) in[ci] = src[ci];
        }
        const float *wt = w + ((kx * 3 + ky) * 3 + kz) * CI * CO;
#pragma unroll
        for (int ci = 0; ci < CI; ++ci) {
          const float v = ok ? in[ci] : 0.0f;
#pragma unroll
          for (int co = 0; co < CO; ++co) acc[co] = fmaf(v, wt[ci * CO + co], acc[co]);
        }
      }
    }
  }
  float *dst = out + i * CO;
#pragma unroll
  for (int q = 0; q < CO / 4; ++q)
    reinterpret_cast<float4 *>(dst)[q] =
        make_float4(fmaxf(acc[4 * q], 0.0f), fmaxf(acc[4 * q + 1], 0.0f), fmaxf(acc[4 * q + 2], 0.0f),
                    fmaxf(acc[4 * q + 3], 0.0f));
}

int ilog2(int x) {
  int l = 0;
  while ((1 << l) < x) ++l;
  return l;
}

}

extern "C" int mf_conv3d_k4s2_pack_weights(const float *W, int32_t Cout, int32_t Cin, int32_t w_cin,
                                           int32_t c_off, float *wt, mfStream_t stream_) {
  hipStream_t stream = (hipStream_t)stream_;
  const int64_t total = (int64_t)Cout * 64 * Cin;
  hipLaunchKernelGGL(k_conv_pack, dim3((unsigned)((total + 255) / 256)), dim3(256), 0, stream, W, Cout, Cin,
                     w_cin, c_off, wt);
  return mf::check_launch("mf_conv3d_k4s2_pack_weights");
}

extern "C" int32_t mf_conv3d_k4s2_default_split(int32_t B, int32_t Cin, int32_t Cout, int32_t D) {
  const int Do = D / 2;
  const int64_t M = (int64_t)B * Do * Do * Do;
  const int64_t tiles = ((M + kBM - 1) / kBM) * (Cout / kBN);
  const int max_split = 2 * Cin >= 64 ? 64 : 2 * Cin;
  int S = 1;
  while (tiles * S < 512 && S * 2 <= max_split && (2 * Cin) / (S * 2) >= 8) S *= 2;
  return S;
}

extern "C" int64_t mf_conv3d_k4s2_workspace_bytes(int32_t B, int32_t Cout, int32_t D, int32_t split) {
  const int Do = D / 2;
  return split > 1 ? (int64_t)split * B * Do * Do * Do * Cout * 4 : 0;
}

extern "C" int mf_conv3d_k4s2_fwd(const float *x, const float *wt, const float *bias, const float *add,
                                  float *out, void *ws, int32_t B, int32_t Cin, int32_t Cout, int32_t D,
                                  int32_t split, int32_t relu, mfStream_t stream_) {
  hipStream_t stream = (hipStream_t)stream_;
  if (B <= 0) return 0;
  const int lg = ilog2(Cin);
  if ((1 << lg) != Cin || Cin < 4 || Cout % kBN || D % 2 || D < 2 || split < 1 || (2 * Cin) % split ||
      (split > 1 && !ws) || (int64_t)B * D * D * D * Cin >= (1ll << 31) || (int64_t)Cout * 64 * Cin >= (1ll << 31)) {
    mf::set_last_error(hipErrorInvalidValue,
                       "conv3d_k4s2: need Cin a power of two >= 4, Cout % 128 == 0, even D, split | 2 Cin, "
                       "input and weights < 2^31 elements");
    return -(int)hipErrorInvalidValue;
  }
  if (int e = mf::allow_big_lds((const void *)k_conv3d_k4s2_mfma, kConvLds)) return e;
  const int Do = D / 2;
  const int64_t M = (int64_t)B * Do * Do * Do;
  ConvArgs a;
  a.x = x; a.wt = wt; a.bias = bias; a.add = add;
  a.out = split > 1 ? (float *)ws : out;
  a.B = B; a.D = D; a.Cin = Cin; a.cin_log2 = lg; a.Cout = Cout; a.S = split; a.relu = relu;
  const int64_t grid = ((M + kBM - 1) / kBM) * (Cout / kBN) * split;
  hipLaunchKernelGGL(k_conv3d_k4s2_mfma, dim3((unsigned)grid), dim3(256), kConvLds, stream, a);
  if (split > 1) {
    const int64_t MN = M * Cout;
    hipLaunchKernelGGL(k_conv_finish, dim3((unsigned)((MN / 4 + 255) / 256)), dim3(256), 0, stream,
                       (const float *)ws, bias, add, out, MN, Cout, split, relu);
  }
  return mf::check_launch("mf_conv3d_k4s2_fwd");
}

extern "C" int mf_to_channels_last(const float *src, float *dst, int32_t B, int32_t C, int64_t V,
                                   mfStream_t stream_) {
  hipStream_t stream = (hipStream_t)stream_;
  if (B <= 0 || C <= 0 || V <= 0) return 0;
  hipLaunchKernelGGL(k_to_channels_last, dim3((unsigned)((V + 31) / 32), (unsigned)((C + 31) / 32), (unsigned)B),
                     dim3(256), 0, stream, src, dst, C, (int)V);
  return mf::check_launch("mf_to_channels_last");
}

extern "C" int mf_occupancy_convs_fwd(const float *grid, const float *w1, const float *b1, const float *w2,
                                      const float *b2, float *h1, float *h2, int32_t B, int32_t D,
                                      mfStream_t stream_) {
  hipStream_t stream = (hipStream_t)stream_;
  if (B <= 0) return 0;
  const int64_t total = (int64_t)B * D * D * D;
  if (total * 16 >= (1ll << 31)) {
    mf::set_last_error(hipErrorInvalidValue, "occupancy_convs: B * D^3 * 16 must stay below 2^31");
    return -(int)hipErrorInvalidValue;
  }
  const unsigned nb = (unsigned)((total + 255) / 256);
  hipLaunchKernelGGL((k_occ_conv3<1, 8, 1>), dim3(nb), dim3(256), 0, stream, grid, w1, b1, h1, B, D);
  hipLaunchKernelGGL((k_occ_conv3<8, 16, 2>), dim3(nb), dim3(256), 0, stream, (const float *)h1, w2, b2, h2, B, D);
  return mf::check_launch("mf_occupancy_convs_fwd");
}
```

morefusion_amd/csrc/gemm_bf16.hip:

```cpp
#include <cstdlib>

#include "mf_common.h"

#include "gemm_bf16_nt.h"
#include "gemm_bf16_tn.h"
#include "gemm_bf16_aux.h"
#include "gemm_bf16_narrow.h"

namespace {

struct Knobs { int nt_big, nt_splitk, tn_pp, nt_half_max, pp_dbg; };
Knobs read_knobs() {
  auto num = [](const char *name, int unset) { const char *e = getenv(name); return e ? atoi(e) : unset; };
  Knobs k = {num("MF_NT_BIG", -1), num("MF_NT_SPLITK", 0), num("MF_TN_PP", 1), num("MF_NT_HALF_MAX", 255), 0};
#ifdef MF_PP_ABLATE
  k.pp_dbg = num("MF_PP_DBG", 0);
#endif
  return k;
}

constexpr int64_t kAnyWs = INT64_MAX;
struct NtShape { int mode; int64_t M; int N, K, groups; bool table; int64_t dgrad_rows; bool may_split; int64_t ws_bytes; };
struct NtPlan { int tile, S, dbg; };

NtPlan nt_plan(const NtShape &p, const Knobs &k) {
  const int64_t full = ((p.M + 127) / 128) * ((p.N + kBN - 1) / kBN) * p.groups;
  const int64_t big = ((p.M + kBigM - 1) / kBigM) * ((p.N + kBigN - 1) / kBigN) * p.groups;
  const bool dgrad = p.mode == kConvDgrad, can_big = !p.table && !(dgrad && (p.dgrad_rows & (kBigM - 1)));
  int S = 1;
  if (p.may_split && p.ws_bytes > 0 && can_big && p.N >= 192 && p.N % 8 == 0 && k.nt_big != 0) {
    const int T = (p.K + kBK - 1) / kBK;
    if (k.nt_splitk > 0) S = k.nt_splitk <= T ? k.nt_splitk : 1;
    else if (big >= 16 && big < 160)
      for (S = (int)(256 / big); S > 1 && T / S < 16;) --S;
    if (S > 1 && p.ws_bytes < S * p.M * p.N * 4) S = 1;
  }
  bool use_big = (big >= 224 && p.N >= 160 && can_big) || S > 1;
  if (k.nt_big == 2)
    use_big = can_big;
  else if (k.nt_big >= 0)
    use_big = use_big && k.nt_big == 1;
  if (use_big) return {kBigM, S, k.pp_dbg};
  const bool half = full <= k.nt_half_max && !dgrad;
  return {half ? 64 : 128, S, 0};
}

int64_t nt_workspace_bytes(int mode, int64_t M, int N, int K) {
  const NtPlan p = nt_plan({mode, M, N, K, 1, false, 0, true, kAnyWs}, read_knobs());
  return p.S > 1 ? p.S * M * N * 4 : 0;
}

int wgrad_split_model(int64_t tiles, int64_t ktiles, int64_t slab_bytes, int slots) {
  if (tiles <= 0 || ktiles <= 0) return 1;
  const double per_slab = slab_bytes / 3.0e6 > 0.05 ? slab_bytes / 3.0e6 : 0.05;
  int best = 1;
  double best_cost = 1e30;
  for (int S = 1; S <= 512; ++S) {
    if (S > 1 && ktiles / S < 8) break;
    const int64_t rounds = (tiles * S + slots - 1) / slots;
    const double cost = (double)rounds * (double)((ktiles + S - 1) / S + 8) + (S > 1 ? S * per_slab : 0.0);
    if (cost < best_cost) { best_cost = cost; best = S; }
  }
  return best;
}

struct TnShape { int Ni, Nj, ldc; int64_t ktiles; int groups; bool ranges, conv; int split; };
enum { kFinishNone = 0, kFinishPlain = 1, kFinishDeep = 2, kFinishConv = 3 };
struct TnPlan { bool pp; int split, finish; };

TnPlan tn_plan(const TnShape &p, const Knobs &k) {
  const int64_t tiles_pp = (int64_t)((p.Ni + 255) / 256) * ((p.Nj + 255) / 256) * p.groups;
  bool pp = k.tn_pp != 0 && k.nt_big != 0 && !p.ranges;
  if (pp && k.nt_big != 2)
    pp = p.Ni >= 192 && p.Nj >= 192 && p.ktiles >= 48 * (tiles_pp >= 256 ? 1 : (256 + tiles_pp - 1) / tiles_pp);
  const int64_t tiles = (int64_t)((p.Ni + 127) / 128) * ((p.Nj + 127) / 128) * p.groups, slab_bytes = 4ll * p.Ni * p.Nj * p.groups;
  const int split = p.split > 0 ? p.split : pp ? wgrad_split_model(tiles_pp, 2 * p.ktiles, slab_bytes, 256)
                                               : wgrad_split_model(tiles, p.ktiles, slab_bytes, 512);
  const int64_t per_slab = (int64_t)p.Ni * p.ldc * p.groups;
  int finish = split >= 32 && per_slab <= (1 << 16) ? kFinishDeep : kFinishPlain;
  if (p.conv && per_slab >= (1 << 20)) finish = kFinishConv;
  if (!p.conv && split == 1) finish = kFinishNone;
  return {pp, split, finish};
}

int g_nt_last_tile = 0;

template <int MODE, int MI>
int launch_nt_tile(const NtArgs &a, hipStream_t stream) {
  if (int e = mf::allow_big_lds((const void *)k_gemm_nt_bf16<MODE, MI>, nt_lds<MI>())) return e;
  const int64_t grid = (int64_t)((a.M + 64 * MI - 1) / (64 * MI)) * ((a.N + kBN - 1) / kBN) * a.groups;
  hipLaunchKernelGGL((k_gemm_nt_bf16<MODE, MI>), dim3((unsigned)grid), dim3(256), nt_lds<MI>(), stream, a);
  return 0;
}
template <int MODE>
int launch_nt(const NtArgs &a, const NtPlan &p, hipStream_t stream, const char *what) {
  g_nt_last_tile = p.tile;
  if (p.tile == kBigM) {
    const int64_t big = (int64_t)((a.M + kBigM - 1) / kBigM) * ((a.N + kBigN - 1) / kBigN) * a.groups;
    if (int e = mf::allow_big_lds((const void *)k_gemm_nt_bf16_pp<MODE>, nt_pp_lds())) return e;
    hipLaunchKernelGGL((k_gemm_nt_bf16_pp<MODE>), dim3((unsigned)(big * a.S)), dim3(512), nt_pp_lds(), stream, a);
    const dim3 finish((unsigned)(((int64_t)a.M * (a.N / 8) + 255) / 256));
    if (a.S > 1 && nt_split(MODE))
      hipLaunchKernelGGL(k_splitk_finish_conv2, finish, dim3(256), 0, stream, a);
    else if (a.S > 1)
      hipLaunchKernelGGL(k_splitk_finish, finish, dim3(256), 0, stream, (const float *)a.slab, a.bias, a.out,
                         (int64_t)a.M, a.N, a.S, a.ldo, a.relu, a.out_f32);
  } else if (int e = p.tile == 64 ? launch_nt_tile<MODE, 1>(a, stream) : launch_nt_tile<MODE, 2>(a, stream))
    return e;
  return mf::check_launch(what);
}

template <bool CONV>
int launch_tn(const TnArgs &a, const TnPlan &p, hipStream_t stream) {
  if (p.pp) {
    if (int e = mf::allow_big_lds((const void *)k_gemm_tn_bf16_pp<CONV>, 5 * kPpOp)) return e;
    const int64_t grid = (int64_t)((a.Ni + 255) / 256) * ((a.Nj + 255) / 256) * a.groups * a.S;
    hipLaunchKernelGGL(k_gemm_tn_bf16_pp<CONV>, dim3((unsigned)grid), dim3(512), 5 * kPpOp, stream, a);
    return 0;
  }
  if (int e = mf::allow_big_lds((const void *)k_gemm_tn_bf16<CONV>, kTnLds)) return e;
  const int64_t grid = (int64_t)((a.Ni + 127) / 128) * ((a.Nj + 127) / 128) * a.groups * a.S;
  hipLaunchKernelGGL(k_gemm_tn_bf16<CONV>, dim3((unsigned)grid), dim3(256), kTnLds, stream, a);
  return 0;
}

void launch_wgrad_finish(int finish, const TnArgs &a, float *dW, int w_cin, int keep, hipStream_t stream) {
  const int taps = a.conv ? a.ks * a.ks * a.ks : 0, cin = a.conv ? a.Cin : 0;
  const int64_t per_group = (int64_t)a.Ni * a.ldc, per_slab = per_group * a.groups;
  const int64_t pitch = a.conv ? (int64_t)w_cin * taps : a.ldc;
  if (finish == kFinishConv)
    hipLaunchKernelGGL(k_wgrad_finish_conv, dim3((keep + kPackTile - 1) / kPackTile, a.Ni), dim3(256), 0, stream,
                       (const float *)a.out, dW, per_slab, a.S, a.Cin, taps, w_cin, keep);
  else if (finish == kFinishDeep)
    hipLaunchKernelGGL(k_wgrad_finish_deep, dim3((unsigned)((per_slab + 3) / 4)), dim3(256), 0, stream,
                       (const float *)a.out, dW, per_slab, a.Nj, a.ldc, a.S, cin, a.c_gs, per_group, pitch, taps, keep);
  else if (finish == kFinishPlain)
    hipLaunchKernelGGL(k_wgrad_finish, dim3((unsigned)((per_slab + 255) / 256)), dim3(256), 0, stream,
                       (const float *)a.out, dW, per_slab, a.Nj, a.ldc, a.S, cin, a.c_gs, per_group, pitch, taps, keep);
}

constexpr int64_t kMaxBf16Elems = 1ll << 30;
int bad(const char *msg) {
  mf::set_last_error(hipErrorInvalidValue, msg);
  return -(int)hipErrorInvalidValue;
}

int ilog2_exact(int x) {
  int l = 0;
  while ((1 << l) < x) ++l;
  return (1 << l) == x ? l : -1;
}

struct Geom { int Do, olog, taps; };
int conv_geom(int B, int Cin, int Cout, int D, int ks, int stride, int pad, int dil, Geom *g) {
  const int span = dil * (ks - 1) + 1;
  if ((ks != 3 && ks != 4) || (stride != 1 && stride != 2) || dil < 1 || pad < 0 || D + 2 * pad < span)
    return bad("conv3d (bf16): kernel 3 or 4, stride 1 or 2");
  g->Do = (D + 2 * pad - span) / stride + 1;
  g->olog = ilog2_exact(g->Do);
  g->taps = ks * ks * ks;
  if (g->olog < 1 || Cin % 8 || Cout % 8 || (int64_t)B * D * D * D * Cin >= kMaxBf16Elems ||
      (int64_t)B * g->Do * g->Do * g->Do * Cout >= kMaxBf16Elems || (int64_t)Cout * g->taps * Cin >= kMaxBf16Elems)
    return bad("conv3d (bf16): output size a power of two, Cin % 8 == 0, Cout % 8 == 0, tensors < 2^30 elements (2^31 bytes)");
  return 0;
}

int conv2_geom(int B, int Cin, int Cout, int D, int ks, int stride, int pad, int dil, Geom *g) {
  const int span = dil * (ks - 1) + 1;
  if ((ks != 1 && ks != 3) || (stride != 1 && stride != 2) || dil < 1 || dil > 4 || pad < 0 || D + 2 * pad < span)
    return bad("conv2d_split: kernel 1 or 3, stride 1 or 2, dilation 1 .. 4");
  g->Do = (D + 2 * pad - span) / stride + 1;
  g->olog = ilog2_exact(g->Do);
  g->taps = ks * ks;
  if (g->olog < 0 || Cin % 8 || Cout % 8 || (int64_t)B * D * D * 2 * Cin >= kMaxBf16Elems ||
      (int64_t)B * g->Do * g->Do >= (1ll << 31) || (int64_t)Cout * g->taps * 3 * Cin >= kMaxBf16Elems)
    return bad("conv2d_split: output side a power of two, Cin % 8 == 0, Cout % 8 == 0, operands < 2^30 elements");
  return 0;
}

int split_out_check(const char *what, const float *bias, float *out32, int ldo32, void *outs, int ldos, int los, int N,
                    const float *res = nullptr, int ldr = 0) {
  if ((!out32 && !outs) || N % 8 || (out32 && (ldo32 < N || ldo32 % 8)) ||
      (outs && (ldos < N || ldos % 8 || los < N || los % 8 || ldos < los + N)) || (res && (ldr < N || ldr % 8)))
    return bad(what);
  if (((uintptr_t)bias | (uintptr_t)out32 | (uintptr_t)outs | (uintptr_t)res) & 15) return bad(what);
  return 0;
}

NtArgs nt_operands(const void *A, int lda, int64_t a_gs, const void *W, int ldw, int64_t w_gs, const float *bias,
                   int64_t b_gs, int64_t M, int N, int K, int groups, const int32_t *tile_group = nullptr) {
  NtArgs a = {};
  a.A = (const uint16_t *)A; a.W = (const uint16_t *)W; a.bias = bias;
  a.a_gs = a_gs; a.w_gs = w_gs; a.b_gs = b_gs;
  a.M = (int)M; a.N = N; a.K = K; a.lda = lda; a.ldw = ldw; a.groups = groups;
  a.tile_group = tile_group;
  return a;
}
void nt_conv_geom(NtArgs &a, int B, int D, const Geom &g, int Cin, int Cout, int ks, int stride, int pad, int dil) {
  a.B = B; a.D = D; a.Do = g.Do; a.olog = g.olog; a.Cin = Cin; a.Cout = Cout;
  a.ks = ks; a.stride = stride; a.pad = pad; a.dil = dil;
}
void nt_plain_out(NtArgs &a, void *out, int64_t o_gs, int ldo, int relu, int out_f32, int accumulate, const NtPlan &p,
                  void *ws = nullptr) {
  a.out = out; a.o_gs = o_gs; a.ldo = ldo; a.relu = relu; a.out_f32 = out_f32; a.accumulate = accumulate;
  a.S = p.S; a.slab = p.S > 1 ? (float *)ws : nullptr; a.dbg = p.dbg;
}
template <int MODE>
int launch_nt_split(NtArgs a, int xc, int act, float *out32, int ldo32, void *outs, int ldos, int los, void *ws,
                    int64_t ws_bytes, mfStream_t stream, const char *what, const float *res = nullptr, int ldr = 0,
                    const float *slope = nullptr) {
  const NtPlan p = nt_plan({MODE, a.M, a.N, a.K, 1, false, 0, true, ws ? ws_bytes : 0}, read_knobs());
  a.xc = xc; a.act = act; a.ldo32 = ldo32; a.ldos = ldos; a.los = los; a.out32 = out32; a.outs = (uint16_t *)outs;
  a.res = res; a.ldr = ldr; a.slope = slope;
  a.S = p.S; a.slab = p.S > 1 ? (float *)ws : nullptr; a.dbg = p.dbg;
  return launch_nt<MODE>(a, p, (hipStream_t)stream, what);
}

}

extern "C" int mf_gemm_bf16_nt_plan(int32_t mode, int64_t M, int32_t N, int32_t K, int32_t groups, int32_t table,
                                    int64_t dgrad_rows, int32_t may_split, int32_t have_ws, int32_t *tile, int32_t *S) {
  if (mode < kRows || mode > kRowsS || M <= 0 || N <= 0 || K <= 0 || groups <= 0 || !tile || !S)
    return bad("gemm_bf16_nt_plan: a mode 0 .. 5, a problem, somewhere to answer");
  const NtShape s = {mode, M, N, K, groups, table != 0, dgrad_rows, may_split != 0, have_ws ? kAnyWs : 0};
  const NtPlan p = nt_plan(s, read_knobs());
  *tile = p.tile; *S = p.S;
  return 0;
}

extern "C" int mf_gemm_bf16_tn_plan(int32_t Ni, int32_t Nj, int32_t ldc, int64_t rows, int32_t groups, int32_t ranges,
                                    int32_t conv, int32_t split, int32_t *form, int32_t *default_split, int32_t *finish) {
  if (Ni <= 0 || Nj <= 0 || ldc < Nj || rows < 0 || groups <= 0 || !form || !default_split || !finish)
    return bad("gemm_bf16_tn_plan: a problem with ldc >= Nj, somewhere to answer");
  const Knobs k = read_knobs();
  TnShape s = {Ni, Nj, ldc, (rows + 63) / 64, groups, ranges != 0, conv != 0, 0};
  *default_split = s.split = tn_plan(s, k).split;
  if (split > 0) s.split = split;
  const TnPlan p = tn_plan(s, k);
  *form = p.pp ? 256 : 128; *finish = p.finish;
  return 0;
}

extern "C" int mf_gemm_bf16_last_tile(void) { return g_nt_last_tile; }

extern "C" int mf_cast_rows_bf16(const float *src, int64_t src_ld, void *dst, int64_t dst_ld, int64_t rows,
                                 int32_t cols, mfStream_t stream_) {
  hipStream_t stream = (hipStream_t)stream_;
  if (rows <= 0) return 0;
  if (dst_ld % 8 || cols > dst_ld || src_ld < cols || ((uintptr_t)dst & 15)) return bad("cast_rows_bf16: dst_ld % 8 == 0, cols <= dst_ld");
  const int64_t n = rows * (dst_ld / 8);
  hipLaunchKernelGGL(k_cast_rows_bf16, dim3((unsigned)((n + 255) / 256)), dim3(256), 0, stream, src, src_ld,
                     (uint16_t *)dst, dst_ld, rows, cols);
  return mf::check_launch("mf_cast_rows_bf16");
}

extern "C" int mf_relu_mask_bf16(const void *y, const void *dy, const float *dy32, void *dz, int64_t n,
                                 mfStream_t stream_) {
  hipStream_t stream = (hipStream_t)stream_;
  if (n <= 0) return 0;
  if (n % 8 || (!dy == !dy32)) return bad("relu_mask_bf16: n % 8 == 0 and exactly one of dy / dy32");
  hipLaunchKernelGGL(k_relu_mask_bf16, dim3((unsigned)((n / 8 + 255) / 256)), dim3(256), 0, stream,
                     (const uint16_t *)y, (const uint16_t *)dy, dy32, (uint16_t *)dz, n / 8);
  return mf::check_launch("mf_relu_mask_bf16");
}

extern "C" int mf_linear_bf16(const void *A, int64_t a_gs, int32_t lda, const void *W, int64_t w_gs, int32_t ldw,
                              const float *bias, int64_t b_gs, void *out, int64_t o_gs, int32_t ldo, int32_t M,
                              int32_t N, int32_t K, int32_t groups, int32_t relu, int32_t out_f32,
                              int32_t accumulate, mfStream_t stream_) {
  if (M <= 0 || N <= 0 || groups <= 0) return 0;
  if (K <= 0 || K % 8 || lda % 8 || ldw % 8 || a_gs % 8 || w_gs % 8 || lda < K || ldw < K || ldo < N ||
      (((uintptr_t)A | (uintptr_t)W) & 15) || (accumulate && !out_f32))
    return bad("linear_bf16: K, lda, ldw, group strides % 8 == 0, 16-byte aligned A / W, accumulate needs fp32 out");
  if ((int64_t)M * lda >= kMaxBf16Elems || (int64_t)N * ldw >= kMaxBf16Elems)
    return bad("linear_bf16: an operand of one group spans >= 2^31 bytes (32-bit byte offsets: split the rows)");
  NtArgs a = nt_operands(A, lda, a_gs, W, ldw, w_gs, bias, b_gs, M, N, K, groups);
  const NtPlan p = nt_plan({kRows, M, N, K, groups, false, 0, false, 0}, read_knobs());
  nt_plain_out(a, out, o_gs, ldo, relu, out_f32, accumulate, p);
  return launch_nt<kRows>(a, p, (hipStream_t)stream_, "mf_linear_bf16");
}

extern "C" int mf_linear_wgrad_bf16(const void *dY, int64_t y_gs, int32_t ldy, const void *A, int64_t a_gs, int32_t lda,
                                    float *dW, int64_t w_gs, int32_t ldc, void *ws, int32_t M, int32_t N, int32_t K,
                                    int32_t groups, int32_t split, mfStream_t stream_) {
  hipStream_t stream = (hipStream_t)stream_;
  if (M <= 0 || N <= 0 || K <= 0 || groups <= 0) return 0;
  if (N % 8 || K % 8 || ldy % 8 || lda % 8 || y_gs % 8 || a_gs % 8 || split < 1 || (split > 1 && !ws) || ldc < K ||
      (((uintptr_t)dY | (uintptr_t)A) & 15))
    return bad("linear_wgrad_bf16: N, K, ldy, lda, group strides % 8 == 0, 16-byte aligned operands");
  if ((int64_t)M * ldy >= kMaxBf16Elems || (int64_t)M * lda >= kMaxBf16Elems)
    return bad("linear_wgrad_bf16: an operand of one group spans >= 2^31 bytes (32-bit byte offsets: split the rows)");
  TnArgs a = {};
  a.P = (const uint16_t *)dY; a.Q = (const uint16_t *)A; a.out = split > 1 ? (float *)ws : dW;
  a.p_gs = y_gs; a.q_gs = a_gs; a.c_gs = w_gs;
  a.M = M; a.Ni = N; a.Nj = K; a.ldp = ldy; a.ldq = lda; a.ldc = ldc; a.groups = groups; a.S = split;
  const TnPlan p = tn_plan({N, K, ldc, ((int64_t)M + 63) / 64, groups, false, false, split}, read_knobs());
  if (int e = launch_tn<false>(a, p, stream)) return e;
  launch_wgrad_finish(p.finish, a, dW, 0, 0, stream);
  return mf::check_launch("mf_linear_wgrad_bf16");
}

extern "C" int mf_linear_bf16_tiles(const void *A, int32_t lda, const void *W, int64_t w_gs, int32_t ldw,
                                    const int32_t *tile_group, void *out, int32_t ldo, int32_t M, int32_t N, int32_t K,
                                    int32_t out_f32, mfStream_t stream_) {
  if (M <= 0 || N <= 0) return 0;
  if (K <= 0 || K % 8 || lda % 8 || ldw % 8 || w_gs % 8 || lda < K || ldw < K || ldo < N || M % 128 || !tile_group ||
      (((uintptr_t)A | (uintptr_t)W) & 15))
    return bad("linear_bf16_tiles: K, lda, ldw, w_gs % 8 == 0, M % 128 == 0, 16-byte aligned A / W, a group table");
  if ((int64_t)M * lda >= kMaxBf16Elems || (int64_t)N * ldw >= kMaxBf16Elems)
    return bad("linear_bf16_tiles: an operand spans >= 2^31 bytes");
  NtArgs a = nt_operands(A, lda, 0, W, ldw, w_gs, nullptr, 0, M, N, K, 1, tile_group);
  const NtPlan p = nt_plan({kRows, M, N, K, 1, true, 0, false, 0}, read_knobs());
  nt_plain_out(a, out, 0, ldo, 0, out_f32, 0, p);
  return launch_nt<kRows>(a, p, (hipStream_t)stream_, "mf_linear_bf16_tiles");
}

extern "C" int mf_linear_wgrad_bf16_ranges(const void *dY, int32_t ldy, const void *A, int32_t lda, float *dW,
                                           int64_t w_gs, int32_t ldc, const int32_t *m_range, int32_t groups, int32_t N,
                                           int32_t K, mfStream_t stream_) {
  if (N <= 0 || K <= 0 || groups <= 0) return 0;
  if (N % 8 || K % 8 || ldy % 8 || lda % 8 || ldc < K || !m_range || (((uintptr_t)dY | (uintptr_t)A) & 15))
    return bad("linear_wgrad_bf16_ranges: N, K, ldy, lda % 8 == 0, 16-byte aligned operands, a range table");
  TnArgs a = {};
  a.P = (const uint16_t *)dY; a.Q = (const uint16_t *)A; a.out = dW;
  a.c_gs = w_gs;
  a.M = 0; a.Ni = N; a.Nj = K; a.ldp = ldy; a.ldq = lda; a.ldc = ldc; a.groups = groups; a.S = 1;
  a.m_range = m_range;
  if (int e = launch_tn<false>(a, tn_plan({N, K, ldc, 0, groups, true, false, 1}, read_knobs()), (hipStream_t)stream_))
    return e;
  return mf::check_launch("mf_linear_wgrad_bf16_ranges");
}

extern "C" int64_t mf_conv3d_bf16_fwd_workspace_bytes(int32_t B, int32_t Cin, int32_t Cout, int32_t D, int32_t ks,
                                                      int32_t stride, int32_t pad, int32_t dil) {
  Geom g;
  if (B <= 0 || conv_geom(B, Cin, Cout, D, ks, stride, pad, dil, &g)) return 0;
  return nt_workspace_bytes(kConvFwd, (int64_t)B * g.Do * g.Do * g.Do, Cout, g.taps * Cin);
}

extern "C" int mf_conv3d_bf16_pack(const float *W, int32_t Cout, int32_t Cin, int32_t w_cin, int32_t c_off, int32_t ks,
                                   void *fwd, void *dgrad_k4s2, void *flipT, mfStream_t stream_) {
  hipStream_t stream = (hipStream_t)stream_;
  if ((ks != 3 && ks != 4) || (dgrad_k4s2 && ks != 4)) return bad("conv3d_bf16_pack: kernel 3 or 4 (parity-class dgrad: 4)");
  const int taps = ks * ks * ks;
  if (fwd)
    hipLaunchKernelGGL(k_conv_pack_fwd_tile, dim3((Cin + kPackTile - 1) / kPackTile, Cout), dim3(256), 0, stream, W, Cin,
                       w_cin, c_off, taps, (uint16_t *)fwd);
  if (dgrad_k4s2 || flipT)
    hipLaunchKernelGGL(k_conv_pack_cof_tile, dim3((Cout + kPackTile - 1) / kPackTile, Cin), dim3(256), 0, stream, W,
                       Cout, Cin, w_cin, c_off, ks, (uint16_t *)dgrad_k4s2, (uint16_t *)flipT);
  return mf::check_launch("mf_conv3d_bf16_pack");
}

extern "C" int mf_conv3d_bf16_fwd_ws(const void *x, const void *wt, const float *bias, void *out, void *ws,
                                     int64_t ws_bytes, int32_t B, int32_t Cin, int32_t Cout, int32_t D, int32_t ks,
                                     int32_t stride, int32_t pad, int32_t dil, int32_t relu, int32_t out_f32,
                                     int32_t ldo, mfStream_t stream_) {
  if (B <= 0) return 0;
  Geom g;
  if (int e = conv_geom(B, Cin, Cout, D, ks, stride, pad, dil, &g)) return e;
  if (ldo < Cout) return bad("conv3d_bf16_fwd / _ws: ldo >= Cout");
  const int64_t M = (int64_t)B * g.Do * g.Do * g.Do;
  const NtPlan p = nt_plan({kConvFwd, M, Cout, g.taps * Cin, 1, false, 0, true, ws ? kAnyWs : 0}, read_knobs());
  if (p.S > 1 && (ws_bytes < p.S * M * Cout * 4 || ((uintptr_t)ws & 15))) return bad("conv3d_bf16_fwd_ws: workspace too small / unaligned");
  NtArgs a = nt_operands(x, 0, 0, wt, g.taps * Cin, 0, bias, 0, M, Cout, g.taps * Cin, 1);
  nt_conv_geom(a, B, D, g, Cin, Cout, ks, stride, pad, dil);
  nt_plain_out(a, out, 0, ldo, relu, out_f32, 0, p, ws);
  return launch_nt<kConvFwd>(a, p, (hipStream_t)stream_, "mf_conv3d_bf16_fwd");
}

extern "C" int mf_conv3d_bf16_fwd(const void *x, const void *wt, const float *bias, void *out, int32_t B, int32_t Cin,
                                  int32_t Cout, int32_t D, int32_t ks, int32_t stride, int32_t pad, int32_t dil,
                                  int32_t relu, int32_t out_f32, int32_t ldo, mfStream_t stream) {
  return mf_conv3d_bf16_fwd_ws(x, wt, bias, out, nullptr, 0, B, Cin, Cout, D, ks, stride, pad, dil, relu, out_f32, ldo, stream);
}

extern "C" int mf_conv3d_k4s2_bf16_dgrad(const void *dy, const void *wd, void *dx, int32_t B, int32_t Cin,
                                         int32_t Cout, int32_t D, int32_t out_f32, int32_t accumulate,
                                         mfStream_t stream_) {
  if (B <= 0) return 0;
  Geom g;
  if (int e = conv_geom(B, Cin, Cout, D, 4, 2, 1, 1, &g)) return e;
  const int64_t Do3 = (int64_t)g.Do * g.Do * g.Do, M = (int64_t)B * D * D * D;
  if (Do3 % 128 || (accumulate && !out_f32)) return bad("conv3d_k4s2 dgrad: (D/2)^3 % 128 == 0; accumulate needs fp32");
  NtArgs a = nt_operands(dy, 0, 0, wd, 8 * Cout, 0, nullptr, 0, M, Cin, 8 * Cout, 1);
  nt_conv_geom(a, B, D, g, Cin, Cout, 4, 2, 1, 1);
  const NtPlan p = nt_plan({kConvDgrad, M, Cin, 8 * Cout, 1, false, Do3, false, 0}, read_knobs());
  nt_plain_out(a, dx, 0, Cin, 0, out_f32, accumulate, p);
  return launch_nt<kConvDgrad>(a, p, (hipStream_t)stream_, "mf_conv3d_k4s2_bf16_dgrad");
}

extern "C" int64_t mf_conv3d_bf16_wgrad_workspace_bytes(int32_t Cin, int32_t Cout, int32_t ks, int32_t split) {
  return (int64_t)(split > 1 ? split : 1) * Cout * ks * ks * ks * Cin * 4;
}

extern "C" int32_t mf_wgrad_split(int64_t tiles, int64_t ktiles, int64_t slab_bytes) {
  return wgrad_split_model(tiles, ktiles, slab_bytes, 512);
}

extern "C" int32_t mf_linear_wgrad_bf16_default_split(int64_t M, int32_t N, int32_t K, int32_t groups) {
  return tn_plan({N, K, K, (M + 63) / 64, groups, false, false, 0}, read_knobs()).split;
}

extern "C" int32_t mf_conv3d_bf16_wgrad_default_split(int32_t B, int32_t Cin, int32_t Cout, int32_t Do, int32_t ks) {
  const int Nj = ks * ks * ks * Cin;
  return tn_plan({Cout, Nj, Nj, ((int64_t)B * Do * Do * Do + 63) / 64, 1, false, true, 0}, read_knobs()).split;
}

extern "C" int mf_conv3d_bf16_wgrad(const void *dy, const void *x, float *dW, void *ws, int32_t B, int32_t Cin,
                                    int32_t Cout, int32_t D, int32_t ks, int32_t stride, int32_t pad, int32_t dil,
                                    int32_t w_cin, int32_t c_off, int32_t split, mfStream_t stream_) {
  hipStream_t stream = (hipStream_t)stream_;
  if (B <= 0) return 0;
  Geom g;
  if (int e = conv_geom(B, Cin, Cout, D, ks, stride, pad, dil, &g)) return e;
  if (split < 1 || !ws) return bad("conv3d wgrad: workspace required");
  if (g.olog < 2) return bad("conv3d wgrad: output size >= 4 per axis");
  TnArgs a = {};
  a.P = (const uint16_t *)dy; a.Q = (const uint16_t *)x; a.out = (float *)ws;
  a.M = B * g.Do * g.Do * g.Do; a.Ni = Cout; a.Nj = g.taps * Cin; a.ldp = Cout; a.ldc = g.taps * Cin; a.groups = 1;
  a.S = split;
  a.conv = 1; a.B = B; a.D = D; a.Do = g.Do; a.olog = g.olog; a.Cin = Cin;
  a.ks = ks; a.stride = stride; a.pad = pad; a.dil = dil;
  const TnPlan p = tn_plan({a.Ni, a.Nj, a.ldc, ((int64_t)a.M + 63) / 64, 1, false, true, split}, read_knobs());
  if (int e = launch_tn<true>(a, p, stream)) return e;
  const int keep = w_cin - c_off < Cin ? w_cin - c_off : Cin;
  if (keep > 0) launch_wgrad_finish(p.finish, a, dW + (int64_t)c_off * g.taps, w_cin, keep, stream);
  return mf::check_launch("mf_conv3d_bf16_wgrad");
}

extern "C" int64_t mf_conv3d_k3_narrow_bf16_pack_elems(int32_t CI) { return (int64_t)32 * ((27 * CI + 15) / 16) * 16; }

extern "C" int mf_conv3d_k3_narrow_bf16_pack(const float *W, int32_t Cout, int32_t Cin, int32_t w_cin, int32_t c_off,
                                             int32_t transpose, void *wp, mfStream_t stream_) {
  hipStream_t stream = (hipStream_t)stream_;
  const int CI = transpose ? Cout : Cin, NO = transpose ? Cin : Cout;
  if ((CI != 8 && CI != 16) || NO < 1 || NO > 16 || (NO & 3)) return bad("conv3d_k3_narrow pack: read channels 8 or 16, written channels 4 .. 16 (% 4)");
  const int Kp = ((27 * CI + 15) / 16) * 16;
  hipLaunchKernelGGL(k_conv_k3_narrow_pack, dim3((32 * Kp + 255) / 256), dim3(256), 0, stream, W, Cout, Cin, w_cin, c_off,
                     transpose, CI, Kp, (uint16_t *)wp);
  return mf::check_launch("mf_conv3d_k3_narrow_bf16_pack");
}

extern "C" int mf_conv3d_k3_narrow_bf16(const void *x, const void *wp, const float *bias, void *out, int32_t B,
                                        int32_t CI, int32_t CO, int32_t D, int32_t dil, int32_t relu,
                                        mfStream_t stream_) {
  hipStream_t stream = (hipStream_t)stream_;
  if (B <= 0) return 0;
  const int dlog = ilog2_exact(D);
  if ((CI != 8 && CI != 16) || CO < 1 || CO > 16 || (CO & 3) || dlog < 1 || dil < 1 ||
      (int64_t)B * D * D * D * 16 >= kMaxBf16Elems || (((uintptr_t)x | (uintptr_t)wp | (uintptr_t)out) & 15))
    return bad("conv3d_k3_narrow: read channels 8 or 16, written channels 4 .. 16 (% 4), D a power of two, 16-byte aligned");
  const int64_t tiles = ((int64_t)B * D * D * D + 31) / 32;
  int tpw = 1;
  while (tpw < 8 && tiles / (4 * tpw * 2) >= 2048) tpw *= 2;
  const unsigned blocks = (unsigned)((tiles + 4 * tpw - 1) / (4 * tpw));
  if (CI == 8)
    hipLaunchKernelGGL((k_conv_k3_narrow_bf16<8, 14>), dim3(blocks), dim3(256), 0, stream, (const uint16_t *)x,
                       (const uint16_t *)wp, bias, (uint16_t *)out, B, D, dlog, CO, dil, relu, tpw);
  else
    hipLaunchKernelGGL((k_conv_k3_narrow_bf16<16, 27>), dim3(blocks), dim3(256), 0, stream, (const uint16_t *)x,
                       (const uint16_t *)wp, bias, (uint16_t *)out, B, D, dlog, CO, dil, relu, tpw);
  return mf::check_launch("mf_conv3d_k3_narrow_bf16");
}

extern "C" int mf_conv3d_k4s2_pack_bf16(const float *W, int32_t Cout, int32_t Cin, int32_t w_cin, int32_t c_off,
                                        void *fwd, void *dgrad, mfStream_t stream) {
  return mf_conv3d_bf16_pack(W, Cout, Cin, w_cin, c_off, 4, fwd, dgrad, nullptr, stream);
}
extern "C" int mf_conv3d_k4s2_bf16_fwd(const void *x, const void *wt, const float *bias, void *out, int32_t B,
                                       int32_t Cin, int32_t Cout, int32_t D, int32_t relu, int32_t out_f32,
                                       mfStream_t stream) {
  return mf_conv3d_bf16_fwd(x, wt, bias, out, B, Cin, Cout, D, 4, 2, 1, 1, relu, out_f32, Cout, stream);
}
extern "C" int64_t mf_conv3d_k4s2_bf16_wgrad_workspace_bytes(int32_t Cin, int32_t Cout, int32_t split) {
  return mf_conv3d_bf16_wgrad_workspace_bytes(Cin, Cout, 4, split);
}
extern "C" int32_t mf_conv3d_k4s2_bf16_wgrad_default_split(int32_t B, int32_t Cin, int32_t Cout, int32_t D) {
  return mf_conv3d_bf16_wgrad_default_split(B, Cin, Cout, D / 2, 4);
}
extern "C" int mf_conv3d_k4s2_bf16_wgrad(const void *dy, const void *x, float *dW, void *ws, int32_t B, int32_t Cin,
                                         int32_t Cout, int32_t D, int32_t w_cin, int32_t c_off, int32_t split,
                                         mfStream_t stream) {
  return mf_conv3d_bf16_wgrad(dy, x, dW, ws, B, Cin, Cout, D, 4, 2, 1, 1, w_cin, c_off, split, stream);
}

extern "C" int mf_conv2d_split_pack(const float *W, int32_t Cout, int32_t Cin, int32_t ks, void *wp, mfStream_t stream_) {
  hipStream_t stream = (hipStream_t)stream_;
  if (Cout <= 0 || Cin <= 0) return 0;
  if ((ks != 1 && ks != 3) || ((uintptr_t)wp & 15)) return bad("conv2d_split_pack: kernel 1 or 3, aligned output");
  const int64_t n = (int64_t)Cout * ks * ks * 3 * Cin;
  hipLaunchKernelGGL(k_conv2_pack_split, dim3((unsigned)((n + 255) / 256)), dim3(256), 0, stream, W, Cout, Cin, Cin, 0,
                     ks * ks, (uint16_t *)wp);
  return mf::check_launch("mf_conv2d_split_pack");
}

extern "C" int64_t mf_conv2d_split_workspace_bytes(int32_t B, int32_t Cin, int32_t Cout, int32_t D, int32_t ks,
                                                   int32_t stride, int32_t pad, int32_t dil) {
  Geom g;
  if (B <= 0 || conv2_geom(B, Cin, Cout, D, ks, stride, pad, dil, &g)) return 0;
  return nt_workspace_bytes(kConv2Fwd, (int64_t)B * g.Do * g.Do, Cout, g.taps * 3 * Cin);
}

extern "C" int mf_conv2d_split_fwd(const void *xs, const void *wp, const float *bias, const float *res, int32_t ldr,
                                   const float *slope, int32_t act, float *out32, int32_t ldo32, void *outs, int32_t ldos,
                                   int32_t los, void *ws, int64_t ws_bytes, int32_t B, int32_t Cin, int32_t Cout,
                                   int32_t D, int32_t ks, int32_t stride, int32_t pad, int32_t dil, mfStream_t stream_) {
  if (B <= 0) return 0;
  Geom g;
  if (int e = conv2_geom(B, Cin, Cout, D, ks, stride, pad, dil, &g)) return e;
  if (act < 0 || act > 2 || (act == 2 && !slope)) return bad("conv2d_split_fwd: act 0 / 1 / 2 (PReLU needs its slope)");
  if (int e = split_out_check("conv2d_split_fwd: an output; output / residual pitches >= Cout, multiples of 8; lo plane inside the row; 16-byte aligned",
                              bias, out32, ldo32, outs, ldos, los, Cout, res, ldr))
    return e;
  if (((uintptr_t)xs | (uintptr_t)wp | (uintptr_t)ws) & 15) return bad("conv2d_split_fwd: 16-byte aligned operands");
  const int64_t M = (int64_t)B * g.Do * g.Do;
  const int K = g.taps * 3 * Cin;
  NtArgs a = nt_operands(xs, 0, 0, wp, K, 0, bias, 0, M, Cout, K, 1);
  nt_conv_geom(a, B, D, g, 3 * Cin, Cout, ks, stride, pad, dil);
  return launch_nt_split<kConv2Fwd>(a, 2 * Cin, act, out32, ldo32, outs, ldos, los, ws, ws_bytes, stream_,
                                    "mf_conv2d_split_fwd", res, ldr, slope);
}

extern "C" int mf_conv3d_k4s2_split_pack(const float *W, int32_t Cout, int32_t Cin, int32_t w_cin, int32_t c_off,
                                         void *wp, mfStream_t stream_) {
  hipStream_t stream = (hipStream_t)stream_;
  if (Cout <= 0 || Cin <= 0) return 0;
  if (c_off < 0 || c_off + Cin > w_cin || ((uintptr_t)wp & 15)) return bad("conv3d_k4s2_split_pack: channel range, aligned output");
  const int64_t n = (int64_t)Cout * 64 * 3 * Cin;
  hipLaunchKernelGGL(k_conv2_pack_split, dim3((unsigned)((n + 255) / 256)), dim3(256), 0, stream, W, Cout, Cin, w_cin,
                     c_off, 64, (uint16_t *)wp);
  return mf::check_launch("mf_conv3d_k4s2_split_pack");
}

extern "C" int64_t mf_conv3d_k4s2_split_workspace_bytes(int32_t B, int32_t Cin, int32_t Cout, int32_t D) {
  Geom g;
  if (B <= 0 || conv_geom(B, 2 * Cin, Cout, D, 4, 2, 1, 1, &g)) return 0;
  return nt_workspace_bytes(kConvFwdS, (int64_t)B * g.Do * g.Do * g.Do, Cout, 64 * 3 * Cin);
}

extern "C" int mf_conv3d_k4s2_split_fwd(const void *xs, const void *wp, const float *bias, int32_t relu, float *out32,
                                        int32_t ldo32, void *outs, int32_t ldos, int32_t los, void *ws, int64_t ws_bytes,
                                        int32_t B, int32_t Cin, int32_t Cout, int32_t D, mfStream_t stream_) {
  if (B <= 0) return 0;
  Geom g;
  if (int e = conv_geom(B, 2 * Cin, Cout, D, 4, 2, 1, 1, &g)) return e;
  if (Cin % 8 || (int64_t)Cout * 64 * 3 * Cin >= kMaxBf16Elems) return bad("conv3d_k4s2_split_fwd: Cin % 8 == 0, weights < 2^30 elements");
  if (int e = split_out_check("conv3d_k4s2_split_fwd: an output; pitches >= Cout, multiples of 8; lo plane inside the row; 16-byte aligned",
                              bias, out32, ldo32, outs, ldos, los, Cout))
    return e;
  if (((uintptr_t)xs | (uintptr_t)wp | (uintptr_t)ws) & 15) return bad("conv3d_k4s2_split_fwd: 16-byte aligned operands");
  const int64_t M = (int64_t)B * g.Do * g.Do * g.Do;
  const int K = 64 * 3 * Cin;
  NtArgs a = nt_operands(xs, 0, 0, wp, K, 0, bias, 0, M, Cout, K, 1);
  nt_conv_geom(a, B, D, g, 3 * Cin, Cout, 4, 2, 1, 1);
  return launch_nt_split<kConvFwdS>(a, 2 * Cin, relu ? 1 : 0, out32, ldo32, outs, ldos, los, ws, ws_bytes, stream_,
                                    "mf_conv3d_k4s2_split_fwd");
}

extern "C" int mf_linear_split_pack(const float *W, int64_t w_gs, int32_t ldw, int32_t N, int32_t K, int32_t Np,
                                    int32_t Kp, int32_t groups, void *wp, mfStream_t stream_) {
  hipStream_t stream = (hipStream_t)stream_;
  if (N <= 0 || K <= 0 || groups <= 0) return 0;
  if (Np < N || Kp < K || Kp % 8 || ldw < K || ((uintptr_t)wp & 15))
    return bad("linear_split_pack: Np >= N, Kp >= K, Kp % 8 == 0, ldw >= K, aligned output");
  const int64_t n = (int64_t)groups * Np * 3 * Kp;
  hipLaunchKernelGGL(k_rows_pack_split, dim3((unsigned)((n + 255) / 256)), dim3(256), 0, stream, W, w_gs, ldw, N, K, Np,
                     Kp, groups, (uint16_t *)wp);
  return mf::check_launch("mf_linear_split_pack");
}

extern "C" int64_t mf_linear_split_workspace_bytes(int64_t M, int32_t N, int32_t Kp) {
  if (M <= 0 || N <= 0 || Kp <= 0 || N % 8) return 0;
  return nt_workspace_bytes(kRowsS, M, N, 3 * Kp);
}

extern "C" int mf_linear_split_fwd(const void *As, int32_t lda, const void *wp, const float *bias, int32_t relu,
                                   float *out32, int32_t ldo32, void *outs, int32_t ldos, int32_t los, void *ws,
                                   int64_t ws_bytes, int32_t M, int32_t N, int32_t Kp, mfStream_t stream_) {
  if (M <= 0 || N <= 0) return 0;
  if (Kp <= 0 || Kp % 8 || lda % 8 || lda < 2 * Kp || (((uintptr_t)As | (uintptr_t)wp | (uintptr_t)ws) & 15))
    return bad("linear_split_fwd: Kp, lda % 8 == 0, lda >= 2 Kp, 16-byte aligned operands");
  if ((int64_t)M * lda >= kMaxBf16Elems || (int64_t)N * 3 * Kp >= kMaxBf16Elems)
    return bad("linear_split_fwd: an operand spans >= 2^31 bytes");
  if (int e = split_out_check("linear_split_fwd: an output; N % 8 == 0; pitches >= N, multiples of 8; lo plane inside the row; 16-byte aligned",
                              bias, out32, ldo32, outs, ldos, los, N))
    return e;
  const NtArgs a = nt_operands(As, lda, 0, wp, 3 * Kp, 0, bias, 0, M, N, 3 * Kp, 1);
  return launch_nt_split<kRowsS>(a, 2 * Kp, relu ? 1 : 0, out32, ldo32, outs, ldos, los, ws, ws_bytes, stream_,
                                 "mf_linear_split_fwd");
}
```

morefusion_amd/csrc/gemm_bf16_nt.h:

```cpp
#pragma once
#include "mf_common.h"

namespace {

using mf::mf_f32x16;

constexpr int kBN = 128, kBK = 64;
constexpr int kPitch = 144;
template <int MI> constexpr int nt_buf_bytes() { return (64 * MI + kBN) * kPitch; }
template <int MI> constexpr int nt_lds() {
  return 2 * nt_buf_bytes<MI>() > 64 * MI * (kBN + 4) * 4 ? 2 * nt_buf_bytes<MI>() : 64 * MI * (kBN + 4) * 4;
}

enum { kRows = 0, kConvFwd = 1, kConvDgrad = 2, kConv2Fwd = 3, kConvFwdS = 4, kRowsS = 5 };
constexpr bool nt_conv3(int mode) { return mode == kConvFwd || mode == kConvFwdS; }
constexpr bool nt_rows(int mode) { return mode == kRows || mode == kRowsS; }
constexpr bool nt_split(int mode) { return mode == kConv2Fwd || mode == kConvFwdS || mode == kRowsS; }

struct NtArgs {
  const uint16_t *A;
  const uint16_t *W;
  const float *bias;
  void *out;
  int64_t a_gs, w_gs, b_gs, o_gs;
  int M, N, K, lda, ldw, ldo, groups;
  int relu, out_f32, accumulate;
  const int32_t *tile_group;
  int B, D, Do, olog, Cin, Cout, ks, stride, pad, dil;
  int S;
  float *slab;
  int xc, act, ldr, ldo32, ldos, los;
  const float *res, *slope;
  float *out32;
  uint16_t *outs;
  int dbg;
};

__device__ __forceinline__ void conv2_store8(const NtArgs &a, int64_t m, int n, float *v) {
  if (a.bias) {
    const float4 b0 = *reinterpret_cast<const float4 *>(a.bias + n), b1 = *reinterpret_cast<const float4 *>(a.bias + n + 4);
    v[0] += b0.x; v[1] += b0.y; v[2] += b0.z; v[3] += b0.w; v[4] += b1.x; v[5] += b1.y; v[6] += b1.z; v[7] += b1.w;
  }
  if (a.res) {
    const float *r = a.res + m * a.ldr + n;
    const float4 r0 = *reinterpret_cast<const float4 *>(r), r1 = *reinterpret_cast<const float4 *>(r + 4);
    v[0] += r0.x; v[1] += r0.y; v[2] += r0.z; v[3] += r0.w; v[4] += r1.x; v[5] += r1.y; v[6] += r1.z; v[7] += r1.w;
  }
  if (a.act) {
    const float s = a.act == 2 ? *a.slope : 0.0f;
#pragma unroll
    for (int j = 0; j < 8; ++j) v[j] = v[j] > 0.0f ? v[j] : s * v[j];
  }
  if (a.out32) {
    float4 *o = reinterpret_cast<float4 *>(a.out32 + m * a.ldo32 + n);
    o[0] = make_float4(v[0], v[1], v[2], v[3]);
    o[1] = make_float4(v[4], v[5], v[6], v[7]);
  }
  if (a.outs) {
    uint32_t h[8], l[8];
#pragma unroll
    for (int j = 0; j < 8; ++j) {
      h[j] = mf::bf16_bits(v[j]);
      l[j] = mf::bf16_bits(v[j] - mf::bf16_lo(h[j]));
    }
    uint16_t *o = a.outs + m * a.ldos + n;
    *reinterpret_cast<uint4 *>(o) = make_uint4(h[0] | h[1] << 16, h[2] | h[3] << 16, h[4] | h[5] << 16, h[6] | h[7] << 16);
    *reinterpret_cast<uint4 *>(o + a.los) =
        make_uint4(l[0] | l[1] << 16, l[2] | l[3] << 16, l[4] | l[5] << 16, l[6] | l[7] << 16);
  }
}

template <int MODE, int MI>
__global__ __launch_bounds__(256, 2) void k_gemm_nt_bf16(NtArgs a) {
  MF_DYN_LDS(unsigned char, s_raw);
  constexpr int kBM = 64 * MI, kBuf = nt_buf_bytes<MI>();
  const int tiles_m = (a.M + kBM - 1) / kBM, tiles_n = (a.N + kBN - 1) / kBN;
  const int per_group = tiles_m * tiles_n;
  const int G = gridDim.x;
  int L = blockIdx.x;
  if ((G & 7) == 0) L = (blockIdx.x & 7) * (G >> 3) + (blockIdx.x >> 3);
  const int grp = L / per_group;
  const int rem = L - grp * per_group;
  const int m0 = (rem / tiles_n) * kBM, n0 = (rem % tiles_n) * kBN;
  const int T = (a.K + kBK - 1) / kBK;

  const int tid = threadIdx.x, wave = tid >> 6, lane = tid & 63;
  const int wm = wave & 1, wn = wave >> 1;
  const int lrow = lane & 31, lhalf = lane >> 5;
  const int chunk = tid & 7, r0 = tid >> 3;

  const int Do = a.Do, dol = a.olog;
  const uint16_t *A = a.A + grp * a.a_gs;
  const uint16_t *W = a.W + grp * a.w_gs;
  if (MODE == kRows && a.tile_group) {
    const int g = a.tile_group[m0 >> 6];
    if (g < 0) return;
    W += (int64_t)g * a.w_gs;
  }
  int cls = 0;
  if (MODE == kConvDgrad) {
    cls = (m0 >> (3 * dol)) & 7;
    W += (int64_t)cls * a.N * a.ldw;
  }
  int base[2 * MI], mask[2 * MI];
#pragma unroll
  for (int i = 0; i < 2 * MI; ++i) {
    const int m = m0 + r0 + 32 * i;
    const bool row_ok = m < a.M;
    const int mm = row_ok ? m : 0;
    int mk = row_ok ? 1 << 12 : 0;
    if (nt_rows(MODE)) {
      base[i] = mm * a.lda;
    } else if (MODE == kConv2Fwd) {
      const int b = mm >> (2 * dol), o = mm & ((1 << (2 * dol)) - 1);
      const int y0 = a.stride * (o >> dol) - a.pad, x0 = a.stride * (o & (Do - 1)) - a.pad;
      base[i] = ((b * a.D + y0) * a.D + x0) * a.xc;
#pragma unroll
      for (int k = 0; k < 4; ++k) {
        mk |= ((unsigned)(y0 + a.dil * k) < (unsigned)a.D ? 1 : 0) << k;
        mk |= ((unsigned)(x0 + a.dil * k) < (unsigned)a.D ? 1 : 0) << (4 + k);
      }
    } else if (nt_conv3(MODE)) {
      const int b = mm >> (3 * dol), o = mm & ((1 << (3 * dol)) - 1);
      const int ox = o >> (2 * dol), oy = (o >> dol) & (Do - 1), oz = o & (Do - 1);
      const int x0 = a.stride * ox - a.pad, y0 = a.stride * oy - a.pad, z0 = a.stride * oz - a.pad;
      base[i] = (((b * a.D + x0) * a.D + y0) * a.D + z0) * (MODE == kConvFwdS ? a.xc : a.Cin);
#pragma unroll
      for (int k = 0; k < 4; ++k) {
        mk |= ((unsigned)(x0 + a.dil * k) < (unsigned)a.D ? 1 : 0) << k;
        mk |= ((unsigned)(y0 + a.dil * k) < (unsigned)a.D ? 1 : 0) << (4 + k);
        mk |= ((unsigned)(z0 + a.dil * k) < (unsigned)a.D ? 1 : 0) << (8 + k);
      }
    } else {
      const int h = mm & ((1 << (3 * dol)) - 1), b = mm >> (3 * dol + 3);
      const int hx = h >> (2 * dol), hy = (h >> dol) & (Do - 1), hz = h & (Do - 1);
      const int ux = hx + (cls & 1), uy = hy + ((cls >> 1) & 1), uz = hz + ((cls >> 2) & 1);
      base[i] = (((b * Do + ux) * Do + uy) * Do + uz) * a.Cout;
#pragma unroll
      for (int s = 0; s < 2; ++s) {
        mk |= ((unsigned)(ux - s) < (unsigned)Do ? 1 : 0) << s;
        mk |= ((unsigned)(uy - s) < (unsigned)Do ? 1 : 0) << (4 + s);
        mk |= ((unsigned)(uz - s) < (unsigned)Do ? 1 : 0) << (8 + s);
      }
    }
    mask[i] = mk;
  }
  uint32_t wrow[4];
#pragma unroll
  for (int i = 0; i < 4; ++i) {
    const int n = n0 + r0 + 32 * i;
    wrow[i] = 2u * (uint32_t)((int64_t)(n < a.N ? n : 0) * a.ldw);
  }

  mf_f32x16 acc[MI][2];
#pragma unroll
  for (int i = 0; i < MI; ++i)
#pragma unroll
    for (int j = 0; j < 2; ++j)
#pragma unroll
      for (int e = 0; e < 16; ++e) acc[i][j][e] = 0.0f;

  uint4 ra0P, ra1P, ra2P = make_uint4(0u, 0u, 0u, 0u), ra3P = ra2P, rb0P, rb1P, rb2P, rb3P;
  int kg = 8 * chunk, tc = 0, tx = 0, ty = 0, tz = 0;
  if (nt_conv3(MODE)) {
    const int tap = kg / a.Cin;
    tc = kg - tap * a.Cin;
    const int kxy = tap / a.ks;
    tz = tap - kxy * a.ks; tx = kxy / a.ks; ty = kxy - tx * a.ks;
  } else if (MODE == kConv2Fwd) {
    const int tap = kg / a.Cin;
    tc = kg - tap * a.Cin;
    tx = tap / a.ks; ty = tap - tx * a.ks;
  } else if (MODE == kConvDgrad) {
    tx = kg / a.Cout;
    tc = kg - tx * a.Cout;
  }
  const mf::BufRsrc Ars = mf::make_rsrc(A), Wrs = mf::make_rsrc(W);
#define MF_NT_LOAD_A(S, i_, reg_)                                                                     \
  reg_ = mf::buf_load16(Ars, (mask[i_] & bits_) == bits_ ? 2u * (uint32_t)(base[i_] + off_) : mf::kBufMasked);
#define MF_NT_LOAD_B(S, i_, reg_) reg_ = mf::buf_load16(Wrs, wrow[i_] + kofs_);
#define MF_NT_FETCH(S)                                                                                \
  {                                                                                                   \
    const bool kin_ = kg + 8 <= a.K;                                                                  \
    const uint32_t kofs_ = kin_ ? 2u * (uint32_t)kg : 0u;                                             \
    int off_ = MODE == kRowsS && kg >= a.xc ? kg - a.xc : kg, bits_ = 1 << 12;                        \
    if (nt_conv3(MODE)) {                                                                             \
      off_ = ((tx * a.D + ty) * a.D + tz) * a.dil * (MODE == kConvFwdS ? a.xc : a.Cin) +              \
             (MODE == kConvFwdS && tc >= a.xc ? tc - a.xc : tc);                                      \
      bits_ = tx < a.ks ? (1 << tx) | (16 << ty) | (256 << tz) | (1 << 12) : 1 << 13;                 \
    } else if (MODE == kConv2Fwd) {                                                                   \
      off_ = (tx * a.D + ty) * a.dil * a.xc + (tc >= a.xc ? tc - a.xc : tc);                          \
      bits_ = tx < a.ks ? (1 << tx) | (16 << ty) | (1 << 12) : 1 << 13;                               \
    } else if (MODE == kConvDgrad) {                                                                  \
      const int sx = tx & 1, sy = (tx >> 1) & 1, sz = tx >> 2;                                        \
      off_ = tc - ((sx * Do + sy) * Do + sz) * a.Cout;                                                \
      bits_ = (1 << sx) | (16 << sy) | (256 << sz) | (1 << 12);                                       \
    }                                                                                                 \
    if (!kin_) bits_ = 1 << 13;                                              \
    MF_NT_LOAD_A(S, 0, ra0##S) MF_NT_LOAD_A(S, 1, ra1##S)                                             \
    if constexpr (MI == 2) { MF_NT_LOAD_A(S, 2 * MI - 2, ra2##S) MF_NT_LOAD_A(S, 2 * MI - 1, ra3##S) } \
    MF_NT_LOAD_B(S, 0, rb0##S) MF_NT_LOAD_B(S, 1, rb1##S) MF_NT_LOAD_B(S, 2, rb2##S) MF_NT_LOAD_B(S, 3, rb3##S) \
    kg += kBK;                                                                                        \
    if (nt_conv3(MODE)) {                                                                             \
      tc += kBK;                                                                                      \
      while (tc >= a.Cin) {                                                                           \
        tc -= a.Cin;                                                                                  \
        if (++tz == a.ks) { tz = 0; if (++ty == a.ks) { ty = 0; ++tx; } }                             \
      }                                                                                               \
    } else if (MODE == kConv2Fwd) {                                                                   \
      tc += kBK;                                                                                      \
      while (tc >= a.Cin) {                                                                           \
        tc -= a.Cin;                                                                                  \
        if (++ty == a.ks) { ty = 0; ++tx; }                                                           \
      }                                                                                               \
    } else if (MODE == kConvDgrad) {                                                                  \
      tc += kBK;                                                                                      \
      while (tc >= a.Cout) { tc -= a.Cout; ++tx; }                                                    \
    }                                                                                                 \
  }
#define MF_NT_STASH(S, buf_)                                                                          \
  {                                                                                                   \
    MF_HOLD(ra0##S); MF_HOLD(ra1##S); MF_HOLD(rb0##S); MF_HOLD(rb1##S); MF_HOLD(rb2##S); MF_HOLD(rb3##S); \
    if constexpr (MI == 2) { MF_HOLD(ra2##S); MF_HOLD(ra3##S); }                                      \
    unsigned char *As_ = s_raw + (buf_) * kBuf + r0 * kPitch + 16 * chunk;                            \
    unsigned char *Bs_ = As_ + kBM * kPitch;                                                          \
    *reinterpret_cast<uint4 *>(As_) = ra0##S; *reinterpret_cast<uint4 *>(As_ + 32 * kPitch) = ra1##S; \
    if constexpr (MI == 2) {                                                                          \
      *reinterpret_cast<uint4 *>(As_ + 64 * kPitch) = ra2##S; *reinterpret_cast<uint4 *>(As_ + 96 * kPitch) = ra3##S; \
    }                                                                                                 \
    *reinterpret_cast<uint4 *>(Bs_) = rb0##S; *reinterpret_cast<uint4 *>(Bs_ + 32 * kPitch) = rb1##S; \
    *reinterpret_cast<uint4 *>(Bs_ + 64 * kPitch) = rb2##S; *reinterpret_cast<uint4 *>(Bs_ + 96 * kPitch) = rb3##S; \
  }
#ifndef MF_NT_PIPE
#define MF_NT_PIPE 1
#endif
#define MF_NT_FRAGS(set_, s_, NJ_)                                                                    \
  {                                                                                                   \
    fa[set_][0] = *reinterpret_cast<const uint4 *>(As + 32 * (s_));                                   \
    if constexpr (MI == 2) fa[set_][1] = *reinterpret_cast<const uint4 *>(As + 32 * kPitch + 32 * (s_)); \
    fb[set_][0] = *reinterpret_cast<const uint4 *>(Bs + 32 * (s_));                                   \
    if constexpr (NJ_ == 2) fb[set_][1] = *reinterpret_cast<const uint4 *>(Bs + 32 * kPitch + 32 * (s_)); \
  }
#define MF_NT_COMPUTE(buf_, NJ_)                                                                      \
  {                                                                                                   \
    asm volatile("" ::: "memory");                                                                    \
    __builtin_amdgcn_sched_barrier(0);                                                                \
    const unsigned char *As = s_raw + (buf_) * kBuf + (wm * 32 * MI + lrow) * kPitch + 16 * lhalf;    \
    const unsigned char *Bs = s_raw + (buf_) * kBuf + (kBM + wn * 64 + lrow) * kPitch + 16 * lhalf;   \
    if constexpr (MF_NT_PIPE) {                                                                       \
      uint4 fa[2][2], fb[2][2];                                                                       \
      MF_NT_FRAGS(0, 0, NJ_)                                                                          \
      __builtin_amdgcn_sched_group_barrier(0x100, MI + NJ_, 0);                                       \
      _Pragma("unroll") for (int s = 0; s < 4; ++s) {                                                 \
        const int c = s & 1;                                                                          \
        if (s < 3) MF_NT_FRAGS(c ^ 1, s + 1, NJ_)                                                     \
        _Pragma("unroll") for (int mi = 0; mi < MI; ++mi) {                                           \
          acc[mi][0] = mf::mfma_bf16_32x32x16(fa[c][mi], fb[c][0], acc[mi][0]);                       \
          if constexpr (NJ_ == 2) acc[mi][1] = mf::mfma_bf16_32x32x16(fa[c][mi], fb[c][1], acc[mi][1]); \
        }                                                                                             \
        if (s < 3) __builtin_amdgcn_sched_group_barrier(0x100, MI + NJ_, 0);                          \
        __builtin_amdgcn_sched_group_barrier(0x008, MI * NJ_, 0);                                     \
      }                                                                                               \
    } else {                                                                                          \
      _Pragma("unroll") for (int s = 0; s < 4; ++s) {                                                 \
        const uint4 a0 = *reinterpret_cast<const uint4 *>(As + 32 * s);                               \
        const uint4 b0 = *reinterpret_cast<const uint4 *>(Bs + 32 * s);                               \
        acc[0][0] = mf::mfma_bf16_32x32x16(a0, b0, acc[0][0]);                                        \
        if constexpr (NJ_ == 2) {                                                                     \
          const uint4 b1 = *reinterpret_cast<const uint4 *>(Bs + 32 * kPitch + 32 * s);               \
          acc[0][1] = mf::mfma_bf16_32x32x16(a0, b1, acc[0][1]);                                      \
          if constexpr (MI == 2) {                                                                    \
            const uint4 a1 = *reinterpret_cast<const uint4 *>(As + 32 * kPitch + 32 * s);             \
            acc[MI - 1][0] = mf::mfma_bf16_32x32x16(a1, b0, acc[MI - 1][0]);                          \
            acc[MI - 1][1] = mf::mfma_bf16_32x32x16(a1, b1, acc[MI - 1][1]);                          \
          }                                                                                           \
        } else if constexpr (MI == 2) {                                                               \
          const uint4 a1 = *reinterpret_cast<const uint4 *>(As + 32 * kPitch + 32 * s);               \
          acc[MI - 1][0] = mf::mfma_bf16_32x32x16(a1, b0, acc[MI - 1][0]);                            \
        }                                                                                             \
      }                                                                                               \
    }                                                                                                 \
    __builtin_amdgcn_sched_barrier(0);                                                                \
  }
  const int ncols = a.N - (n0 + wn * 64);
  MF_NT_FETCH(P);
  MF_NT_STASH(P, 0);
  __syncthreads();
  for (int t = 0; t < T; ++t) {
    MF_NT_FETCH(P);
    if (ncols > 32) MF_NT_COMPUTE(t & 1, 2) else if (ncols > 0) MF_NT_COMPUTE(t & 1, 1)
    MF_NT_STASH(P, (t + 1) & 1);
    __syncthreads();
  }
#undef MF_NT_FRAGS
#undef MF_NT_COMPUTE
#undef MF_NT_STASH
#undef MF_NT_FETCH
#undef MF_NT_LOAD_B
#undef MF_NT_LOAD_A

  constexpr int kEp = kBN + 4;
  float *s_out = reinterpret_cast<float *>(s_raw);
  const float *bias = a.bias && !nt_split(MODE) ? a.bias + grp * a.b_gs : nullptr;
#pragma unroll
  for (int mi = 0; mi < MI; ++mi)
#pragma unroll
    for (int ni = 0; ni < 2; ++ni) {
      const int nl = wn * 64 + ni * 32 + lrow;
      const float bn = (bias && n0 + nl < a.N) ? bias[n0 + nl] : 0.0f;
#pragma unroll
      for (int e = 0; e < 16; ++e) {
        const int ml = wm * 32 * MI + mi * 32 + (e & 3) + 8 * (e >> 2) + 4 * lhalf;
        float v = acc[mi][ni][e] + bn;
        if (a.relu && !nt_split(MODE)) v = v > 0.0f ? v : 0.0f;
        s_out[ml * kEp + nl] = v;
      }
    }
  __syncthreads();
  for (int i = tid; i < kBM * (kBN / 8); i += 256) {
    const int ml = i / (kBN / 8), c8 = i - ml * (kBN / 8);
    const int m = m0 + ml, n = n0 + 8 * c8;
    if (m >= a.M || n >= a.N) continue;
    int64_t orow = m;
    if (MODE == kConvDgrad) {
      const int h = m & ((1 << (3 * dol)) - 1), p = (m >> (3 * dol)) & 7, b = m >> (3 * dol + 3);
      const int x = 2 * (h >> (2 * dol)) + (p & 1), y = 2 * ((h >> dol) & (Do - 1)) + ((p >> 1) & 1),
                z = 2 * (h & (Do - 1)) + (p >> 2);
      orow = (((int64_t)b * a.D + x) * a.D + y) * a.D + z;
    }
    const float4 v0 = *reinterpret_cast<const float4 *>(s_out + ml * kEp + 8 * c8);
    const float4 v1 = *reinterpret_cast<const float4 *>(s_out + ml * kEp + 8 * c8 + 4);
    float v[8] = {v0.x, v0.y, v0.z, v0.w, v1.x, v1.y, v1.z, v1.w};
    if (nt_split(MODE)) {
      conv2_store8(a, m, n, v);
      continue;
    }
    const int nv = a.N - n < 8 ? a.N - n : 8;
    if (a.out_f32) {
      float *o = reinterpret_cast<float *>(a.out) + grp * a.o_gs + orow * a.ldo + n;
      if (nv == 8 && (a.ldo & 3) == 0 && ((uintptr_t)o & 15) == 0) {
        float4 *o4 = reinterpret_cast<float4 *>(o);
        if (a.accumulate) {
          const float4 p0 = o4[0], p1 = o4[1];
          v[0] += p0.x; v[1] += p0.y; v[2] += p0.z; v[3] += p0.w;
          v[4] += p1.x; v[5] += p1.y; v[6] += p1.z; v[7] += p1.w;
        }
        o4[0] = make_float4(v[0], v[1], v[2], v[3]);
        o4[1] = make_float4(v[4], v[5], v[6], v[7]);
      } else {
        for (int j = 0; j < nv; ++j) o[j] = a.accumulate ? o[j] + v[j] : v[j];
      }
    } else {
      uint16_t *o = reinterpret_cast<uint16_t *>(a.out) + grp * a.o_gs + orow * a.ldo + n;
      if (nv == 8 && (a.ldo & 7) == 0 && ((uintptr_t)o & 15) == 0) {
        *reinterpret_cast<uint4 *>(o) = make_uint4(mf::pack_bf16x2(v[0], v[1]), mf::pack_bf16x2(v[2], v[3]),
                                                   mf::pack_bf16x2(v[4], v[5]), mf::pack_bf16x2(v[6], v[7]));
      } else {
        for (int j = 0; j < nv; ++j) o[j] = (uint16_t)mf::bf16_bits(v[j]);
      }
    }
  }
}

constexpr int kBigM = 256, kBigN = 256;

constexpr int kPpOp = 256 * 128;
constexpr int kPpW0 = 3 * kPpOp;
constexpr int nt_pp_lds() { return 5 * kPpOp; }

template <int MODE>
__global__ __launch_bounds__(512, 2) void k_gemm_nt_bf16_pp(NtArgs a) {
  MF_DYN_LDS(unsigned char, s_raw);
  constexpr int kBM = kBigM, kBNb = kBigN;
  const int tiles_m = (a.M + kBM - 1) / kBM, tiles_n = (a.N + kBNb - 1) / kBNb;
  const int per_group = tiles_m * tiles_n;
  const int G = gridDim.x;
  int L = blockIdx.x;
  if ((G & 7) == 0) L = (blockIdx.x & 7) * (G >> 3) + (blockIdx.x >> 3);
  const int split = L / (per_group * a.groups);
  L -= split * per_group * a.groups;
  const int grp = L / per_group;
  const int rem = L - grp * per_group;
  const int m0 = (rem / tiles_n) * kBM, n0 = (rem % tiles_n) * kBNb;
  const int Tall = (a.K + kBK - 1) / kBK, Tper = (Tall + a.S - 1) / a.S;
  const int t0 = split * Tper;
  const int T = max(0, min(Tall, t0 + Tper) - t0);

  const int tid = threadIdx.x, lane = tid & 63;
  const int wave = mf::wave_uniform(tid >> 6);
  const int wm = wave >> 2, wn = wave & 3;
  const int lrow = lane & 31, lhalf = lane >> 5;
  const int r0 = tid >> 3;
  const int chunk = (tid & 7) ^ ((r0 >> 1) & 7);

  const int Do = a.Do, dol = a.olog;
  const uint16_t *A = a.A + grp * a.a_gs;
  const uint16_t *W = a.W + grp * a.w_gs;
  int cls = 0;
  if (MODE == kConvDgrad) {
    cls = (m0 >> (3 * dol)) & 7;
    W += (int64_t)cls * a.N * a.ldw;
  }
  int base[4], mask[4];
#pragma unroll
  for (int i = 0; i < 4; ++i) {
    const int m = m0 + r0 + 64 * i;
    const bool row_ok = m < a.M;
    const int mm = row_ok ? m : 0;
    int mk = row_ok ? 1 << 12 : 0;
    if (nt_rows(MODE)) {
      base[i] = mm * a.lda;
    } else if (MODE == kConv2Fwd) {
      const int b = mm >> (2 * dol), o = mm & ((1 << (2 * dol)) - 1);
      const int y0 = a.stride * (o >> dol) - a.pad, x0 = a.stride * (o & (Do - 1)) - a.pad;
      base[i] = ((b * a.D + y0) * a.D + x0) * a.xc;
#pragma unroll
      for (int k = 0; k < 4; ++k) {
        mk |= ((unsigned)(y0 + a.dil * k) < (unsigned)a.D ? 1 : 0) << k;
        mk |= ((unsigned)(x0 + a.dil * k) < (unsigned)a.D ? 1 : 0) << (4 + k);
      }
    } else if (nt_conv3(MODE)) {
      const int b = mm >> (3 * dol), o = mm & ((1 << (3 * dol)) - 1);
      const int ox = o >> (2 * dol), oy = (o >> dol) & (Do - 1), oz = o & (Do - 1);
      const int x0 = a.stride * ox - a.pad, y0 = a.stride * oy - a.pad, z0 = a.stride * oz - a.pad;
      base[i] = (((b * a.D + x0) * a.D + y0) * a.D + z0) * (MODE == kConvFwdS ? a.xc : a.Cin);
#pragma unroll
      for (int k = 0; k < 4; ++k) {
        mk |= ((unsigned)(x0 + a.dil * k) < (unsigned)a.D ? 1 : 0) << k;
        mk |= ((unsigned)(y0 + a.dil * k) < (unsigned)a.D ? 1 : 0) << (4 + k);
        mk |= ((unsigned)(z0 + a.dil * k) < (unsigned)a.D ? 1 : 0) << (8 + k);
      }
    } else {
      const int h = mm & ((1 << (3 * dol)) - 1), b = mm >> (3 * dol + 3);
      const int hx = h >> (2 * dol), hy = (h >> dol) & (Do - 1), hz = h & (Do - 1);
      const int ux = hx + (cls & 1), uy = hy + ((cls >> 1) & 1), uz = hz + ((cls >> 2) & 1);
      base[i] = (((b * Do + ux) * Do + uy) * Do + uz) * a.Cout;
#pragma unroll
      for (int s = 0; s < 2; ++s) {
        mk |= ((unsigned)(ux - s) < (unsigned)Do ? 1 : 0) << s;
        mk |= ((unsigned)(uy - s) < (unsigned)Do ? 1 : 0) << (4 + s);
        mk |= ((unsigned)(uz - s) < (unsigned)Do ? 1 : 0) << (8 + s);
      }
    }
    mask[i] = mk;
  }
  uint32_t wrow[4];
#pragma unroll
  for (int i = 0; i < 4; ++i) {
    const int n = n0 + r0 + 64 * i;
    wrow[i] = 2u * (uint32_t)((int64_t)(n < a.N ? n : 0) * a.ldw);
  }

  mf_f32x16 acc[4][2];
#pragma unroll
  for (int i = 0; i < 4; ++i)
#pragma unroll
    for (int j = 0; j < 2; ++j)
#pragma unroll
      for (int e = 0; e < 16; ++e) acc[i][j][e] = 0.0f;

  int kg = 8 * chunk + kBK * t0, tc = 0, tx = 0, ty = 0, tz = 0, kgw = kg;
  if (nt_conv3(MODE)) {
    const int tap = kg / a.Cin;
    tc = kg - tap * a.Cin;
    const int kxy = tap / a.ks;
    tz = tap - kxy * a.ks; tx = kxy / a.ks; ty = kxy - tx * a.ks;
  } else if (MODE == kConv2Fwd) {
    const int tap = kg / a.Cin;
    tc = kg - tap * a.Cin;
    tx = tap / a.ks; ty = tap - tx * a.ks;
  } else if (MODE == kConvDgrad) {
    tx = kg / a.Cout;
    tc = kg - tx * a.Cout;
  }
  const mf::BufRsrc Ars = mf::make_rsrc(A), Wrs = mf::make_rsrc(W);
  unsigned char *const dma0 = s_raw + 8 * wave * 128;
#define MF_PP_REQ_A(sa_, i0_, i1_)                                                                    \
  {                                                                                                   \
    const bool kin_ = kg + 8 <= a.K;                                                                  \
    int off_ = MODE == kRowsS && kg >= a.xc ? kg - a.xc : kg, bits_ = 1 << 12;                        \
    if (nt_conv3(MODE)) {                                                                             \
      off_ = ((tx * a.D + ty) * a.D + tz) * a.dil * (MODE == kConvFwdS ? a.xc : a.Cin) +              \
             (MODE == kConvFwdS && tc >= a.xc ? tc - a.xc : tc);                                      \
      bits_ = tx < a.ks ? (1 << tx) | (16 << ty) | (256 << tz) | (1 << 12) : 1 << 13;                 \
    } else if (MODE == kConv2Fwd) {                                                                   \
      off_ = (tx * a.D + ty) * a.dil * a.xc + (tc >= a.xc ? tc - a.xc : tc);                          \
      bits_ = tx < a.ks ? (1 << tx) | (16 << ty) | (1 << 12) : 1 << 13;                               \
    } else if (MODE == kConvDgrad) {                                                                  \
      const int sx = tx & 1, sy = (tx >> 1) & 1, sz = tx >> 2;                                        \
      off_ = tc - ((sx * Do + sy) * Do + sz) * a.Cout;                                                \
      bits_ = (1 << sx) | (16 << sy) | (256 << sz) | (1 << 12);                                       \
    }                                                                                                 \
    if (!kin_) bits_ = 1 << 13;                                              \
    _Pragma("unroll") for (int i = (i0_); i < (i1_); ++i)                                             \
      mf::glds16(Ars, (mask[i] & bits_) == bits_ ? 2u * (uint32_t)(base[i] + off_) : mf::kBufMasked,  \
                 dma0 + (sa_) * kPpOp + i * 64 * 128);                                                \
    if ((i1_) == 4) {                                                                                 \
      kg += kBK;                                                                                      \
      if (nt_conv3(MODE)) {                                                                           \
        tc += kBK;                                                                                    \
        while (tc >= a.Cin) {                                                                         \
          tc -= a.Cin;                                                                                \
          if (++tz == a.ks) { tz = 0; if (++ty == a.ks) { ty = 0; ++tx; } }                           \
        }                                                                                             \
      } else if (MODE == kConv2Fwd) {                                                                 \
        tc += kBK;                                                                                    \
        while (tc >= a.Cin) {                                                                         \
          tc -= a.Cin;                                                                                \
          if (++ty == a.ks) { ty = 0; ++tx; }                                                         \
        }                                                                                             \
      } else if (MODE == kConvDgrad) {                                                                \
        tc += kBK;                                                                                    \
        while (tc >= a.Cout) { tc -= a.Cout; ++tx; }                                                  \
      }                                                                                               \
    }                                                                                                 \
  }
#define MF_PP_REQ_W(sw_, i0_, i1_)                                                                    \
  {                                                                                                   \
    const uint32_t kofs_ = kgw + 8 <= a.K ? 2u * (uint32_t)kgw : 0u;                                  \
    _Pragma("unroll") for (int i = (i0_); i < (i1_); ++i)                                             \
      mf::glds16(Wrs, wrow[i] + kofs_, dma0 + kPpW0 + (sw_) * kPpOp + i * 64 * 128);                  \
    if ((i1_) == 4) kgw += kBK;                                                                       \
  }
  const int gh = (lrow >> 2) & 3, c0 = ((lhalf ^ (lrow >> 1)) & 1) << 4;
  const mf::lds_addr_t fragA = mf::lds_addr(s_raw) + (128 * wm + lrow) * 128 + c0;
  const mf::lds_addr_t fragW = mf::lds_addr(s_raw) + kPpW0 + (64 * wn + lrow) * 128 + c0;
  const int ncols = a.N - (n0 + wn * 64);
  uint4 fa[2][4], fb[2][2];
#define MF_PP_READS(NJ_, kk_, sa_, sw_, s_, r0_, r1_)                                                  \
  if ((NJ_) > 0) {                                                                                    \
    const mf::lds_addr_t va_ = fragA + (sa_) * kPpOp + (((s_) ^ gh) << 5);                            \
    const mf::lds_addr_t vb_ = fragW + (sw_) * kPpOp + (((s_) ^ gh) << 5);                            \
    if ((r0_) <= 0 && 0 < (r1_)) fa[kk_][0] = mf::lds_read16_async<0>(va_);                           \
    if ((r0_) <= 1 && 1 < (r1_)) fb[kk_][0] = mf::lds_read16_async<0>(vb_);                           \
    if ((r0_) <= 2 && 2 < (r1_)) fa[kk_][1] = mf::lds_read16_async<4096>(va_);                        \
    if ((r0_) <= 3 && 3 < (r1_) && (NJ_) > 1) fb[kk_][1] = mf::lds_read16_async<4096>(vb_);           \
    if ((r0_) <= 4 && 4 < (r1_)) fa[kk_][2] = mf::lds_read16_async<8192>(va_);                        \
    if ((r0_) <= 5 && 5 < (r1_)) fa[kk_][3] = mf::lds_read16_async<12288>(va_);                       \
  }
#define MF_PP_PHASE(NJ_, p_, REQ_, WAIT_)                                                             \
  {                                                                                                   \
    MF_PP_READS(NJ_, 0, sa, sw, 2 * (p_), 0, 6)                                                       \
    MF_PP_READS(NJ_, 1, sa, sw, 2 * (p_) + 1, 0, 6)                                                   \
    REQ_(0, 4)                                                                                        \
    WAIT_                                                                                             \
    mf::wait_lds_reads();                                                                             \
    if ((NJ_) > 0) {                                                                                  \
      _Pragma("unroll") for (int kk = 0; kk < 2; ++kk) {                                              \
        _Pragma("unroll") for (int mi = 0; mi < 4; ++mi) MF_HOLD(fa[kk][mi]);                         \
        MF_HOLD(fb[kk][0]);                                                                           \
        if ((NJ_) > 1) MF_HOLD(fb[kk][1]);                                                            \
      }                                                                                               \
    }                                                                                                 \
    mf::raw_barrier();                                                                                \
    __builtin_amdgcn_s_setprio(1);                                                                    \
    _Pragma("unroll") for (int q = 0; q < 16; ++q) {                                                  \
      const int kk = q >> 3, mi = q & 3, nj = (q >> 2) & 1;                                           \
      if (nj < (NJ_)) acc[mi][nj] = mf::mfma_bf16_32x32x16(fa[kk][mi], fb[kk][nj], acc[mi][nj]);      \
    }                                                                                                 \
    __builtin_amdgcn_s_setprio(0);                                                                    \
    mf::raw_barrier();                                                                                \
  }
#define MF_PP_RW(i0_, i1_) if (more1) MF_PP_REQ_W(sw ^ 1, i0_, i1_)
#define MF_PP_RA(i0_, i1_) if (more2) MF_PP_REQ_A(sa2, i0_, i1_)
#define MF_PP_LOOP(NJ_)                                                                               \
  for (int t = 0; t < T; ++t) {                                                                       \
    const int sw = t & 1;                                                                             \
    const bool more1 = t + 1 < T && !(a.dbg & 1), more2 = t + 2 < T && !(a.dbg & 1);                  \
    if (a.dbg & 2) { kg = kgw = 8 * chunk; tc = kg; tx = ty = tz = 0; }                               \
    MF_PP_PHASE(NJ_, 0, MF_PP_RW, )                                                                   \
    MF_PP_PHASE(NJ_, 1, MF_PP_RA, if (more2) mf::wait_dma<4>(); else mf::wait_dma<0>();)              \
    sa = sa == 2 ? 0 : sa + 1;                                                                        \
    sa2 = sa2 == 2 ? 0 : sa2 + 1;                                                                     \
  }
  MF_PP_REQ_A(0, 0, 4) MF_PP_REQ_W(0, 0, 4)
  if (T > 1 && !(a.dbg & 1)) {
    MF_PP_REQ_A(1, 0, 4)
    mf::wait_dma<4>();
  } else {
    mf::wait_dma<0>();
  }
  mf::raw_barrier();
  int sa = 0, sa2 = 2;
  if (wm == 1 && !(a.dbg & 4)) mf::raw_barrier();
  if (ncols > 32) {
    MF_PP_LOOP(2)
  } else if (ncols > 0) {
    MF_PP_LOOP(1)
  } else {
    MF_PP_LOOP(0)
  }
  if (wm == 0 && !(a.dbg & 4)) mf::raw_barrier();
#undef MF_PP_LOOP
#undef MF_PP_RW
#undef MF_PP_RA
#undef MF_PP_READS
#undef MF_PP_PHASE
#undef MF_PP_REQ_W
#undef MF_PP_REQ_A

  constexpr int kEp = kBNb + 4;
  float *s_out = reinterpret_cast<float *>(s_raw);
  const float *bias = a.bias && a.S == 1 && !nt_split(MODE) ? a.bias + grp * a.b_gs : nullptr;
  const bool relu = a.relu && a.S == 1 && !nt_split(MODE), out_f32 = a.out_f32 || a.S > 1;
  const int ldo = a.S > 1 ? a.N : a.ldo;
  void *const outp = a.S > 1 ? (void *)(a.slab + (int64_t)split * a.M * a.N) : a.out;
#pragma unroll
  for (int pass = 0; pass < 4; ++pass) {
    if (wm == (pass >> 1)) {
#pragma unroll
      for (int mh = 0; mh < 2; ++mh)
#pragma unroll
        for (int ni = 0; ni < 2; ++ni) {
          const int nl = wn * 64 + ni * 32 + lrow;
          const float bn = (bias && n0 + nl < a.N) ? bias[n0 + nl] : 0.0f;
          const mf_f32x16 &c = (pass & 1) ? acc[2 + mh][ni] : acc[mh][ni];
#pragma unroll
          for (int e = 0; e < 16; ++e) {
            const int ml = mh * 32 + (e & 3) + 8 * (e >> 2) + 4 * lhalf;
            float v = c[e] + bn;
            if (relu) v = v > 0.0f ? v : 0.0f;
            s_out[ml * kEp + nl] = v;
          }
        }
    }
    __syncthreads();
    for (int i = tid; i < 64 * (kBNb / 8); i += 512) {
      const int ml = i / (kBNb / 8), c8 = i - ml * (kBNb / 8);
      const int m = m0 + 128 * (pass >> 1) + 64 * (pass & 1) + ml, n = n0 + 8 * c8;
      if (m >= a.M || n >= a.N) continue;
      int64_t orow = m;
      if (MODE == kConvDgrad) {
        const int h = m & ((1 << (3 * dol)) - 1), p = (m >> (3 * dol)) & 7, b = m >> (3 * dol + 3);
        const int x = 2 * (h >> (2 * dol)) + (p & 1), y = 2 * ((h >> dol) & (Do - 1)) + ((p >> 1) & 1),
                  z = 2 * (h & (Do - 1)) + (p >> 2);
        orow = (((int64_t)b * a.D + x) * a.D + y) * a.D + z;
      }
      const float4 v0 = *reinterpret_cast<const float4 *>(s_out + ml * kEp + 8 * c8);
      const float4 v1 = *reinterpret_cast<const float4 *>(s_out + ml * kEp + 8 * c8 + 4);
      float v[8] = {v0.x, v0.y, v0.z, v0.w, v1.x, v1.y, v1.z, v1.w};
      if (nt_split(MODE) && a.S == 1) {
        conv2_store8(a, m, n, v);
        continue;
      }
      const int nv = a.N - n < 8 ? a.N - n : 8;
      if (out_f32) {
        float *o = reinterpret_cast<float *>(outp) + grp * a.o_gs + orow * ldo + n;
        if (nv == 8 && (ldo & 3) == 0 && ((uintptr_t)o & 15) == 0) {
          float4 *o4 = reinterpret_cast<float4 *>(o);
          if (a.accumulate && a.S == 1) {
            const float4 p0 = o4[0], p1 = o4[1];
            v[0] += p0.x; v[1] += p0.y; v[2] += p0.z; v[3] += p0.w;
            v[4] += p1.x; v[5] += p1.y; v[6] += p1.z; v[7] += p1.w;
          }
          o4[0] = make_float4(v[0], v[1], v[2], v[3]);
          o4[1] = make_float4(v[4], v[5], v[6], v[7]);
        } else {
          for (int j = 0; j < nv; ++j) o[j] = a.accumulate && a.S == 1 ? o[j] + v[j] : v[j];
        }
      } else {
        uint16_t *o = reinterpret_cast<uint16_t *>(outp) + grp * a.o_gs + orow * ldo + n;
        if (nv == 8 && (ldo & 7) == 0 && ((uintptr_t)o & 15) == 0) {
          *reinterpret_cast<uint4 *>(o) = make_uint4(mf::pack_bf16x2(v[0], v[1]), mf::pack_bf16x2(v[2], v[3]),
                                                     mf::pack_bf16x2(v[4], v[5]), mf::pack_bf16x2(v[6], v[7]));
        } else {
          for (int j = 0; j < nv; ++j) o[j] = (uint16_t)mf::bf16_bits(v[j]);
        }
      }
    }
    __syncthreads();
  }
}

}
```

Measured before the change: 1985 objects/sec.

## Route heads2 and occupancy conv3 through split-bf16 MFMA GEMM path

Adds a grouped split-bf16 linear entry point. heads1 now writes its output directly in hi/lo bf16 split form per group, so heads2 can run as a grouped split-bf16 MFMA GEMM instead of the f32 linear path. Separately, the occupancy conv can emit a split-bf16 h2 that feeds the split k4s2 conv3_occ kernel without split-K, but that path is gated behind a class flag that defaults off. The aim is to replace the f32 GEMM and the intermediate f32 buffers with tensor-core work. The cost is extra hi/lo packing work and more bf16 rounding risk.

```diff
diff --git a/include/mfhip.h b/include/mfhip.h
--- a/include/mfhip.h
+++ b/include/mfhip.h
@@ -169,6 +169,9 @@
                                            int64_t los, mfStream_t stream);
 int mf_occupancy_convs_fwd(const float *grid, const float *w1, const float *b1, const float *w2,
                            const float *b2, float *h1, float *h2, int32_t B, int32_t D, mfStream_t stream);
+int mf_occupancy_convs_split_fwd(const float *grid, const float *w1, const float *b1, const float *w2,
+                                 const float *b2, float *h1, float *h2, void *h2s, int32_t B, int32_t D,
+                                 mfStream_t stream);
 
 int mf_linear_fwd(const float *A, int64_t a_group_stride, int32_t lda, const float *W, int64_t w_group_stride,
                   int32_t ldw, const float *bias, int64_t b_group_stride, float *out, int64_t o_group_stride,
@@ -226,6 +229,10 @@
 int mf_linear_split_fwd(const void *As, int32_t lda, const void *wp, const float *bias, int32_t relu, float *out32,
                         int32_t ldo32, void *outs, int32_t ldos, int32_t los, void *ws, int64_t ws_bytes, int32_t M,
                         int32_t N, int32_t Kp, mfStream_t stream);
+int mf_linear_split_grouped_fwd(const void *As, int64_t a_gs, int32_t lda, const void *wp, int64_t w_gs, const float *bias,
+                                int64_t b_gs, int32_t relu, float *out32, int64_t o_gs, int32_t ldo32, void *outs,
+                                int64_t os_gs, int32_t ldos, int32_t los, int32_t gw, void *ws, int64_t ws_bytes, int32_t M,
+                                int32_t N, int32_t Kp, int32_t groups, mfStream_t stream);
 int64_t mf_conv3d_k3_narrow_bf16_pack_elems(int32_t CI);
 int mf_conv3d_k3_narrow_bf16_pack(const float *W, int32_t Cout, int32_t Cin, int32_t w_cin, int32_t c_off,
                                   int32_t transpose, void *wp, mfStream_t stream);
diff --git a/morefusion_amd/_lib.py b/morefusion_amd/_lib.py
--- a/morefusion_amd/_lib.py
+++ b/morefusion_amd/_lib.py
@@ -106,6 +106,7 @@
     "mf_sparse_conv3d_k4s2_points_cl_fwd": ([_p, _i64, _p, _p, _i64, _f, _f, _f, _f, _p, _p, _p, _p, _p] + [_i] * 6 + [_p], _i),
     "mf_interpolate_voxel_grid_cl_fwd": ([_p, _p, _p, _i64, _i, _i, _i, _i, _i, _p, _i64, _p], _i),
     "mf_occupancy_convs_fwd": ([_p] * 7 + [_i] * 2 + [_p], _i),
+    "mf_occupancy_convs_split_fwd": ([_p] * 8 + [_i] * 2 + [_p], _i),
     "mf_linear_fwd": ([_p, _i64, _i, _p, _i64, _i, _p, _i64, _p, _i64] + [_i] * 7 + [_p], _i),
     "mf_cast_rows_bf16": ([_p, _i64, _p, _i64, _i64, _i, _p], _i),
     "mf_relu_mask_bf16": ([_p, _p, _p, _p, _i64, _p], _i),
@@ -130,6 +131,8 @@
     "mf_linear_split_pack": ([_p, _i64] + [_i] * 6 + [_p, _p], _i),
     "mf_linear_split_workspace_bytes": ([_i64, _i, _i], _i64),
     "mf_linear_split_fwd": ([_p, _i, _p, _p, _i, _p, _i, _p, _i, _i, _p, _i64] + [_i] * 3 + [_p], _i),
+    "mf_linear_split_grouped_fwd": ([_p, _i64, _i, _p, _i64, _p, _i64, _i, _p, _i64, _i, _p, _i64, _i, _i, _i, _p, _i64]
+                                   + [_i] * 4 + [_p], _i),
     "mf_sparse_conv3d_k4s2_points_cl_split_fwd": ([_p, _i64, _p, _p, _i64, _f, _f, _f, _f, _p, _p, _p, _p, _p, _p] + [_i] * 6 + [_p], _i),
     "mf_interpolate_voxel_grid_cl_split_fwd": ([_p, _p, _p, _i64, _i, _i, _i, _i, _i, _p, _i64, _i64, _p], _i),
     "mf_conv3d_k3_narrow_bf16_pack_elems": ([_i], _i64),
diff --git a/morefusion_amd/contrib/singleview_3d/models/volumetric_cl.py b/morefusion_amd/contrib/singleview_3d/models/volumetric_cl.py
--- a/morefusion_amd/contrib/singleview_3d/models/volumetric_cl.py
+++ b/morefusion_amd/contrib/singleview_3d/models/volumetric_cl.py
@@ -7,12 +7,13 @@
 
 F_COLS, F_LD = 984, 992
 
-SPLIT_MIN_BATCH = {"conv4": 4, "heads1": 4}
+SPLIT_MIN_BATCH = {"conv4": 4, "heads1": 4, "conv3_occ": 4, "heads2": 4}
 
 
 class ChannelsLastVolumetric:
 
     split_bf16 = True
+    split_conv3_occ = False
 
     def __init__(self, model):
         self.m = model
@@ -82,7 +83,7 @@
         return (self.split_bf16 and self.mfma_linear and not torch.is_autocast_enabled()
                 and not torch.is_grad_enabled() and B >= SPLIT_MIN_BATCH[layer])
 
-    def conv_k4s2_split(self, name, conv, xs_cl, B, D, cin, c_off=0, relu=True, bias=True, out_split=None):
+    def conv_k4s2_split(self, name, conv, xs_cl, B, D, cin, c_off=0, relu=True, bias=True, out_split=None, splitk=True):
         L = _lib.lib()
 
         def build():
@@ -93,12 +94,12 @@
             return wp, (conv.bias.detach().float().contiguous() if conv.bias is not None else None)
         wp, b = self._pack(name + "_split", [conv.weight] + ([conv.bias] if conv.bias is not None else []), build)
         cout = wp.shape[0]
-        nbytes = L.mf_conv3d_k4s2_split_workspace_bytes(B, cin, cout, D)
+        nbytes = L.mf_conv3d_k4s2_split_workspace_bytes(B, cin, cout, D) if splitk else 0
         ws = self._scratch(name + "_split_ws", (max(nbytes, 16),), xs_cl.device, torch.uint8)
         out = torch.empty((B, (D // 2) ** 3, cout), dtype=torch.float32, device=xs_cl.device)
         _lib.check(L.mf_conv3d_k4s2_split_fwd(xs_cl.data_ptr(), wp.data_ptr(), _lib.ptr(b if bias else None), int(relu),
-                                              out.data_ptr(), cout, _lib.ptr(out_split), 2 * cout, cout, ws.data_ptr(),
-                                              nbytes, B, cin, cout, D, _lib.stream_ptr()), "mf_conv3d_k4s2_split_fwd")
+                                              out.data_ptr(), cout, _lib.ptr(out_split), 2 * cout, cout,
+                                              ws.data_ptr() if nbytes else None, nbytes, B, cin, cout, D, _lib.stream_ptr()), "mf_conv3d_k4s2_split_fwd")
         return out
 
     def sample_split(self, vox_cl, D, pts, batch_indices, fs_block, ldos, los):
@@ -112,7 +113,7 @@
         _lib.check(_lib.lib().mf_split_bf16(feat[:, c0:].data_ptr(), 0, 1, 0, feat.stride(0), 1, c1 - c0, 1, n,
                                             fs[:, c0:].data_ptr(), 2 * F_LD, F_LD, _lib.stream_ptr()), "mf_split_bf16")
 
-    def heads1_split(self, fs, h1):
+    def heads1_split(self, fs, h1, h1s=None):
         m, L = self.m, _lib.lib()
         names = ("rot", "trans", "conf")
 
@@ -127,15 +128,46 @@
         n, N = fs.shape[0], wp.shape[0]
         nbytes = L.mf_linear_split_workspace_bytes(n, N, F_LD)
         ws = self._scratch("heads1_split_ws", (max(nbytes, 16),), fs.device, torch.uint8)
+        if h1s is not None:
+            _lib.check(L.mf_linear_split_grouped_fwd(fs.data_ptr(), 0, 2 * F_LD, wp.data_ptr(), 0, b.data_ptr(), 0, 1,
+                                                     None, 0, 0, h1s.data_ptr(), 0, h1s.stride(0), 0, N // 3,
+                                                     ws.data_ptr(), nbytes, n, N, F_LD, 1, _lib.stream_ptr()),
+                       "mf_linear_split_grouped_fwd")
+            return
         _lib.check(L.mf_linear_split_fwd(fs.data_ptr(), 2 * F_LD, wp.data_ptr(), b.data_ptr(), 1, h1.data_ptr(),
                                          h1.stride(0), None, 0, 0, ws.data_ptr(), nbytes, n, N, F_LD,
                                          _lib.stream_ptr()), "mf_linear_split_fwd")
 
-    def occupancy(self, grid):
+    def heads2_split(self, h1s, h2):
+        m, L = self.m, _lib.lib()
+        convs = [getattr(m, f"conv2_{k}") for k in ("rot", "trans", "conf")]
+        N, K = convs[0].weight.shape[0], convs[0].weight.shape[1]
+        Np = -(-N // 128) * 128
+
+        def build():
+            w = torch.stack([c.weight.detach().float().squeeze(-1) for c in convs]).contiguous()
+            wp = torch.empty((len(convs), Np, 3 * K), dtype=torch.bfloat16, device=w.device)
+            _lib.check(L.mf_linear_split_pack(w.data_ptr(), N * K, K, N, K, Np, K, len(convs), wp.data_ptr(),
+                                              _lib.stream_ptr()), "mf_linear_split_pack")
+            return wp, torch.stack([c.bias.detach().float() for c in convs]).contiguous()
+        wp, b = self._pack("gemm_heads2_split", [t for c in convs for t in (c.weight, c.bias)], build)
+        G = len(convs)
+        _lib.check(L.mf_linear_split_grouped_fwd(h1s.data_ptr(), 2 * K, h1s.stride(0), wp.data_ptr(), Np * 3 * K,
+                                                 b.data_ptr(), N, 1, h2.data_ptr(), N, h2.stride(0), None, 0, 0, 0, 0,
+                                                 None, 0, h1s.shape[0], N, K, G, _lib.stream_ptr()),
+                   "mf_linear_split_grouped_fwd")
+
+    def occupancy(self, grid, split=False):
         B, D = grid.shape[0], grid.shape[1]
         g = _lib.f32c(grid)
         w1, b1, w2, b2 = self._occ_pack()
         h1 = self._scratch("occ_h1", (B, D ** 3, 8), g.device)
+        if split:
+            h2s = self._scratch("occ_h2_split", (B, D ** 3, 32), g.device, torch.bfloat16)
+            _lib.check(_lib.lib().mf_occupancy_convs_split_fwd(g.data_ptr(), w1.data_ptr(), b1.data_ptr(), w2.data_ptr(),
+                                                               b2.data_ptr(), h1.data_ptr(), None, h2s.data_ptr(), B, D,
+                                                               _lib.stream_ptr()), "mf_occupancy_convs_split_fwd")
+            return h2s
         h2 = torch.empty((B, D ** 3, 16), dtype=torch.float32, device=g.device)
         _lib.check(_lib.lib().mf_occupancy_convs_fwd(g.data_ptr(), w1.data_ptr(), b1.data_ptr(), w2.data_ptr(),
                                                      b2.data_ptr(), h1.data_ptr(), h2.data_ptr(), B, D,
@@ -197,8 +229,13 @@
 
         dense = None
         if m._with_occupancy:
-            h_occ = self.occupancy(grid_nontarget_empty)
-            dense = self.conv_k4s2("conv3_occ", m.conv3, h_occ, B, D, cin=16, c_off=144, relu=False, bias=False)
+            if self.split_conv3_occ and self._split_path("conv3_occ", B):
+                h_occ = self.occupancy(grid_nontarget_empty, split=True)
+                dense = self.conv_k4s2_split("conv3_occ", m.conv3, h_occ, B, D, cin=16, c_off=144, relu=False, bias=False,
+                                             splitk=False)
+            else:
+                h_occ = self.occupancy(grid_nontarget_empty)
+                dense = self.conv_k4s2("conv3_occ", m.conv3, h_occ, B, D, cin=16, c_off=144, relu=False, bias=False)
         h3s = self._scratch("h3_split", (B, (D // 2) ** 3, 2 * m.conv3.out_channels), dev, torch.bfloat16) if split4 else None
         h3 = self._sparse.from_points_cl(feat[:, 72:216], F_LD, pts, batch_indices, B, dense, D, out_split=h3s)
         pts2 = pts * 0.5
@@ -253,7 +290,6 @@
                 return wp.contiguous()[None], b.contiguous()[None]
             w1, b1 = self._pack("gemm_heads1", [t for k in names for t in (getattr(m, f"conv1_{k}").weight,
                                                                             getattr(m, f"conv1_{k}").bias)], build1)
-            h1 = self._scratch("heads_h1", (n, 1920), dev)
             h2 = self._scratch("heads_h2", (n, 768), dev)
             h3 = self._scratch("heads_h3", (n, 384), dev)
             np4 = -(-(nf * 4) // 128) * 128
@@ -264,13 +300,20 @@
             if fs is None and self._split_path("heads1", B):
                 fs = self._scratch("feat_split", (n, 2 * F_LD), dev, torch.bfloat16, zero=True)
                 self._split_cols(feat, 0, F_COLS, fs)
-            if fs is not None:
-                self.heads1_split(fs, h1)
+            split2 = fs is not None and self._split_path("heads2", B)
+            if split2:
+                h1s = self._scratch("heads_h1_split", (n, 2 * 1920), dev, torch.bfloat16)
+                self.heads1_split(fs, None, h1s)
+                self.heads2_split(h1s, h2)
             else:
-                _lib.check(L.mf_linear_fwd(feat.data_ptr(), 0, F_LD, w1.data_ptr(), 0, F_LD, b1.data_ptr(), 0,
-                                           h1.data_ptr(), 0, 1920, n, 1920, 1920, F_LD, 1, 1, _lib.stream_ptr()),
-                           "mf_linear_fwd")
-            self._linear("heads2", [getattr(m, f"conv2_{k}") for k in names], h1, 1920, h2, 768, True, a_gs=640, o_gs=256)
+                h1 = self._scratch("heads_h1", (n, 1920), dev)
+                if fs is not None:
+                    self.heads1_split(fs, h1)
+                else:
+                    _lib.check(L.mf_linear_fwd(feat.data_ptr(), 0, F_LD, w1.data_ptr(), 0, F_LD, b1.data_ptr(), 0,
+                                               h1.data_ptr(), 0, 1920, n, 1920, 1920, F_LD, 1, 1, _lib.stream_ptr()),
+                               "mf_linear_fwd")
+                self._linear("heads2", [getattr(m, f"conv2_{k}") for k in names], h1, 1920, h2, 768, True, a_gs=640, o_gs=256)
             self._linear("heads3", [getattr(m, f"conv3_{k}") for k in names], h2, 768, h3, 384, True, a_gs=256, o_gs=128)
             w4, b4 = self._pack("gemm_heads4", [t for k in names for t in (getattr(m, f"conv4_{k}").weight,
                                                                            getattr(m, f"conv4_{k}").bias)],
diff --git a/morefusion_amd/csrc/conv3d.hip b/morefusion_amd/csrc/conv3d.hip
--- a/morefusion_amd/csrc/conv3d.hip
+++ b/morefusion_amd/csrc/conv3d.hip
@@ -206,10 +206,10 @@
     if (v0 + j < V && c0 + tx < C) dst[((int64_t)b * V + v0 + j) * C + c0 + tx] = tile[tx][j];
 }
 
-template <int CI, int CO, int DIL>
+template <int CI, int CO, int DIL, bool SPLIT = false>
 __global__ __launch_bounds__(256) void k_occ_conv3(const float *__restrict__ x, const float *__restrict__ w,
                                                    const float *__restrict__ bias, float *__restrict__ out,
-                                                   int B, int D) {
+                                                   int B, int D, uint16_t *__restrict__ outs = nullptr) {
   const int64_t total = (int64_t)B * D * D * D;
   const int64_t i = (int64_t)blockIdx.x * blockDim.x + threadIdx.x;
   if (i >= total) return;
@@ -250,12 +250,29 @@
       }
     }
   }
-  float *dst = out + i * CO;
-#pragma unroll
-  for (int q = 0; q < CO / 4; ++q)
-    reinterpret_cast<float4 *>(dst)[q] =
-        make_float4(fmaxf(acc[4 * q], 0.0f), fmaxf(acc[4 * q + 1], 0.0f), fmaxf(acc[4 * q + 2], 0.0f),
-                    fmaxf(acc[4 * q + 3], 0.0f));
+  if (!SPLIT || out) {
+    float *dst = out + i * CO;
+#pragma unroll
+    for (int q = 0; q < CO / 4; ++q)
+      reinterpret_cast<float4 *>(dst)[q] =
+          make_float4(fmaxf(acc[4 * q], 0.0f), fmaxf(acc[4 * q + 1], 0.0f), fmaxf(acc[4 * q + 2], 0.0f),
+                      fmaxf(acc[4 * q + 3], 0.0f));
+  }
+  if constexpr (SPLIT && CO % 8 == 0) {
+    uint16_t *os = outs + i * (2 * CO);
+#pragma unroll
+    for (int q = 0; q < CO / 8; ++q) {
+      uint32_t h[8], l[8];
+#pragma unroll
+      for (int j = 0; j < 8; ++j) {
+        const float v = fmaxf(acc[8 * q + j], 0.0f);
+        h[j] = mf::bf16_bits(v);
+        l[j] = mf::bf16_bits(v - mf::bf16_lo(h[j]));
+      }
+      reinterpret_cast<uint4 *>(os)[q] = make_uint4(h[0] | h[1] << 16, h[2] | h[3] << 16, h[4] | h[5] << 16, h[6] | h[7] << 16);
+      reinterpret_cast<uint4 *>(os + CO)[q] = make_uint4(l[0] | l[1] << 16, l[2] | l[3] << 16, l[4] | l[5] << 16, l[6] | l[7] << 16);
+    }
+  }
 }
 
 int ilog2(int x) {
@@ -329,18 +346,44 @@
   return mf::check_launch("mf_to_channels_last");
 }
 
+namespace {
+int occupancy_convs(const float *grid, const float *w1, const float *b1, const float *w2, const float *b2, float *h1,
+                    float *h2, uint16_t *h2s, int32_t B, int32_t D, hipStream_t stream, const char *what) {
+  if (B <= 0) return 0;
+  const int64_t total = (int64_t)B * D * D * D;
+  if (total * (h2s ? 32 : 16) >= (1ll << 31) || (!h2 && !h2s) || ((uintptr_t)h2s & 15)) {
+    mf::set_last_error(hipErrorInvalidValue,
+                       "occupancy_convs: an output (the split one 16-byte aligned), B * D^3 * 16 (split: 32) below 2^31");
+    return -(int)hipErrorInvalidValue;
+  }
+  const unsigned nb = (unsigned)((total + 255) / 256);
+  hipLaunchKernelGGL((k_occ_conv3<1, 8, 1>), dim3(nb), dim3(256), 0, stream, grid, w1, b1, h1, B, D, (uint16_t *)nullptr);
+  if (h2s)
+    hipLaunchKernelGGL((k_occ_conv3<8, 16, 2, true>), dim3(nb), dim3(256), 0, stream, (const float *)h1, w2, b2, h2, B, D, h2s);
+  else
+    hipLaunchKernelGGL((k_occ_conv3<8, 16, 2>), dim3(nb), dim3(256), 0, stream, (const float *)h1, w2, b2, h2, B, D,
+                       (uint16_t *)nullptr);
+  return mf::check_launch(what);
+}
+}
+
 extern "C" int mf_occupancy_convs_fwd(const float *grid, const float *w1, const float *b1, const float *w2,
                                       const float *b2, float *h1, float *h2, int32_t B, int32_t D,
                                       mfStream_t stream_) {
-  hipStream_t stream = (hipStream_t)stream_;
-  if (B <= 0) return 0;
-  const int64_t total = (int64_t)B * D * D * D;
-  if (total * 16 >= (1ll << 31)) {
-    mf::set_last_error(hipErrorInvalidValue, "occupancy_convs: B * D^3 * 16 must stay below 2^31");
+  if (B > 0 && !h2) {
+    mf::set_last_error(hipErrorInvalidValue, "occupancy_convs: h2 is null");
     return -(int)hipErrorInvalidValue;
   }
-  const unsigned nb = (unsigned)((total + 255) / 256);
-  hipLaunchKernelGGL((k_occ_conv3<1, 8, 1>), dim3(nb), dim3(256), 0, stream, grid, w1, b1, h1, B, D);
-  hipLaunchKernelGGL((k_occ_conv3<8, 16, 2>), dim3(nb), dim3(256), 0, stream, (const float *)h1, w2, b2, h2, B, D);
-  return mf::check_launch("mf_occupancy_convs_fwd");
-}
+  return occupancy_convs(grid, w1, b1, w2, b2, h1, h2, nullptr, B, D, (hipStream_t)stream_, "mf_occupancy_convs_fwd");
+}
+
+extern "C" int mf_occupancy_convs_split_fwd(const float *grid, const float *w1, const float *b1, const float *w2,
+                                            const float *b2, float *h1, float *h2, void *h2s, int32_t B, int32_t D,
+                                            mfStream_t stream_) {
+  if (B > 0 && !h2s) {
+    mf::set_last_error(hipErrorInvalidValue, "occupancy_convs_split: h2s is null");
+    return -(int)hipErrorInvalidValue;
+  }
+  return occupancy_convs(grid, w1, b1, w2, b2, h1, h2, (uint16_t *)h2s, B, D, (hipStream_t)stream_,
+                         "mf_occupancy_convs_split_fwd");
+}
diff --git a/morefusion_amd/csrc/gemm_bf16.hip b/morefusion_amd/csrc/gemm_bf16.hip
--- a/morefusion_amd/csrc/gemm_bf16.hip
+++ b/morefusion_amd/csrc/gemm_bf16.hip
@@ -209,7 +209,7 @@
 int launch_nt_split(NtArgs a, int xc, int act, float *out32, int ldo32, void *outs, int ldos, int los, void *ws,
                     int64_t ws_bytes, mfStream_t stream, const char *what, const float *res = nullptr, int ldr = 0,
                     const float *slope = nullptr) {
-  const NtPlan p = nt_plan({MODE, a.M, a.N, a.K, 1, false, 0, true, ws ? ws_bytes : 0}, read_knobs());
+  const NtPlan p = nt_plan({MODE, a.M, a.N, a.K, a.groups, false, 0, a.groups == 1, ws ? ws_bytes : 0}, read_knobs());
   a.xc = xc; a.act = act; a.ldo32 = ldo32; a.ldos = ldos; a.los = los; a.out32 = out32; a.outs = (uint16_t *)outs;
   a.res = res; a.ldr = ldr; a.slope = slope;
   a.S = p.S; a.slab = p.S > 1 ? (float *)ws : nullptr; a.dbg = p.dbg;
@@ -590,3 +590,27 @@
   return launch_nt_split<kRowsS>(a, 2 * Kp, relu ? 1 : 0, out32, ldo32, outs, ldos, los, ws, ws_bytes, stream_,
                                  "mf_linear_split_fwd");
 }
+
+extern "C" int mf_linear_split_grouped_fwd(const void *As, int64_t a_gs, int32_t lda, const void *wp, int64_t w_gs,
+                                           const float *bias, int64_t b_gs, int32_t relu, float *out32, int64_t o_gs,
+                                           int32_t ldo32, void *outs, int64_t os_gs, int32_t ldos, int32_t los, int32_t gw,
+                                           void *ws, int64_t ws_bytes, int32_t M, int32_t N, int32_t Kp, int32_t groups,
+                                           mfStream_t stream_) {
+  if (M <= 0 || N <= 0 || groups <= 0) return 0;
+  if (Kp <= 0 || Kp % 8 || lda % 8 || lda < 2 * Kp || (((uintptr_t)As | (uintptr_t)wp | (uintptr_t)ws) & 15))
+    return bad("linear_split_grouped_fwd: Kp, lda % 8 == 0, lda >= 2 Kp, 16-byte aligned operands");
+  if ((int64_t)M * lda >= kMaxBf16Elems || (int64_t)N * 3 * Kp >= kMaxBf16Elems)
+    return bad("linear_split_grouped_fwd: an operand of one group spans >= 2^31 bytes");
+  if (groups > 1 && (a_gs % 8 || w_gs % 8 || b_gs % 4 || o_gs % 4 || os_gs % 8 || a_gs < 0 || w_gs < 0 || b_gs < 0 ||
+                     o_gs < 0 || os_gs < 0))
+    return bad("linear_split_grouped_fwd: group strides keep every group 16-byte aligned");
+  if (gw < 0 || gw % 8 || (gw && outs && (N % gw || ldos < 2 * N)))
+    return bad("linear_split_grouped_fwd: gw % 8 == 0, N % gw == 0, ldos >= 2 N");
+  if (int e = split_out_check("linear_split_grouped_fwd: an output; N % 8 == 0; pitches >= N, multiples of 8; lo plane inside the row; 16-byte aligned",
+                              bias, out32, ldo32, outs, ldos, gw ? N : los, N))
+    return e;
+  NtArgs a = nt_operands(As, lda, a_gs, wp, 3 * Kp, w_gs, bias, b_gs, M, N, 3 * Kp, groups);
+  a.o_gs = o_gs; a.os_gs = os_gs; a.gw = outs ? gw : 0;
+  return launch_nt_split<kRowsS>(a, 2 * Kp, relu ? 1 : 0, out32, ldo32, outs, ldos, los, ws, ws_bytes, stream_,
+                                 "mf_linear_split_grouped_fwd");
+}
diff --git a/morefusion_amd/csrc/gemm_bf16_nt.h b/morefusion_amd/csrc/gemm_bf16_nt.h
--- a/morefusion_amd/csrc/gemm_bf16_nt.h
+++ b/morefusion_amd/csrc/gemm_bf16_nt.h
@@ -29,16 +29,18 @@
   int B, D, Do, olog, Cin, Cout, ks, stride, pad, dil;
   int S;
   float *slab;
-  int xc, act, ldr, ldo32, ldos, los;
+  int xc, act, ldr, ldo32, ldos, los, gw;
+  int64_t os_gs;
   const float *res, *slope;
   float *out32;
   uint16_t *outs;
   int dbg;
 };
 
-__device__ __forceinline__ void conv2_store8(const NtArgs &a, int64_t m, int n, float *v) {
+__device__ __forceinline__ void conv2_store8(const NtArgs &a, int64_t m, int n, float *v, int grp = 0) {
   if (a.bias) {
-    const float4 b0 = *reinterpret_cast<const float4 *>(a.bias + n), b1 = *reinterpret_cast<const float4 *>(a.bias + n + 4);
+    const float *bias = a.bias + grp * a.b_gs;
+    const float4 b0 = *reinterpret_cast<const float4 *>(bias + n), b1 = *reinterpret_cast<const float4 *>(bias + n + 4);
     v[0] += b0.x; v[1] += b0.y; v[2] += b0.z; v[3] += b0.w; v[4] += b1.x; v[5] += b1.y; v[6] += b1.z; v[7] += b1.w;
   }
   if (a.res) {
@@ -52,7 +54,7 @@
     for (int j = 0; j < 8; ++j) v[j] = v[j] > 0.0f ? v[j] : s * v[j];
   }
   if (a.out32) {
-    float4 *o = reinterpret_cast<float4 *>(a.out32 + m * a.ldo32 + n);
+    float4 *o = reinterpret_cast<float4 *>(a.out32 + grp * a.o_gs + m * a.ldo32 + n);
     o[0] = make_float4(v[0], v[1], v[2], v[3]);
     o[1] = make_float4(v[4], v[5], v[6], v[7]);
   }
@@ -63,9 +65,10 @@
       h[j] = mf::bf16_bits(v[j]);
       l[j] = mf::bf16_bits(v[j] - mf::bf16_lo(h[j]));
     }
-    uint16_t *o = a.outs + m * a.ldos + n;
+    const int blk = a.gw ? n / a.gw : 0;
+    uint16_t *o = a.outs + grp * a.os_gs + m * a.ldos + (a.gw ? n + blk * a.gw : n);
     *reinterpret_cast<uint4 *>(o) = make_uint4(h[0] | h[1] << 16, h[2] | h[3] << 16, h[4] | h[5] << 16, h[6] | h[7] << 16);
-    *reinterpret_cast<uint4 *>(o + a.los) =
+    *reinterpret_cast<uint4 *>(o + (a.gw ? a.gw : a.los)) =
         make_uint4(l[0] | l[1] << 16, l[2] | l[3] << 16, l[4] | l[5] << 16, l[6] | l[7] << 16);
   }
 }
@@ -332,7 +335,7 @@
     const float4 v1 = *reinterpret_cast<const float4 *>(s_out + ml * kEp + 8 * c8 + 4);
     float v[8] = {v0.x, v0.y, v0.z, v0.w, v1.x, v1.y, v1.z, v1.w};
     if (nt_split(MODE)) {
-      conv2_store8(a, m, n, v);
+      conv2_store8(a, m, n, v, grp);
       continue;
     }
     const int nv = a.N - n < 8 ? a.N - n : 8;
@@ -640,7 +643,7 @@
       const float4 v1 = *reinterpret_cast<const float4 *>(s_out + ml * kEp + 8 * c8 + 4);
       float v[8] = {v0.x, v0.y, v0.z, v0.w, v1.x, v1.y, v1.z, v1.w};
       if (nt_split(MODE) && a.S == 1) {
-        conv2_store8(a, m, n, v);
+        conv2_store8(a, m, n, v, grp);
         continue;
       }
       const int nv = a.N - n < 8 ? a.N - n : 8;
```

Measured after the change: 2000 objects/sec, median of 6. No clear change (+0.8%).
